# AnthonyDickson/HIVE

Hardware: AMD Instinct MI355X
Metric: frames/sec (depth+TSDF integrate) @640x480, 512^3 vol (higher is better)
Workload: dtype bf16; 1 GPU; synthetic 640x480x150 RGB (seeded room trajectory), host-resident uint8 frames uploaded in the timed region, DPT-Hybrid depth (seeded random weights: depth 1-7 m, bf16, hip engine) + 512x512x512 TSDF integrate, 107 frames/step; frames_total=4066, volume=512x512x512, tsdf_overlap=True, scaling_mode=weak

## Files before the change

hive_amd/csrc/conv.hip:

```cpp
#include "hive_internal.hpp"
#include "mfma_pipe.hpp"

#include <algorithm>

#ifndef HIVE_CONV_AHEAD_GN2
#define HIVE_CONV_AHEAD_GN2 4
#endif
#ifndef HIVE_CONV_ABLATE
#define HIVE_CONV_ABLATE 0
#endif
#ifndef HIVE_CONV_AHEAD
#define HIVE_CONV_AHEAD 4
#endif

using hive_mfma::f32x4;
using hive_mfma::vec;

namespace {

template <typename T>
struct ConvParams {
    const T *x;
    const T *w;
    const T *bias;
    const T *res1;
    const T *res2;
    T *out;
    T *out_relu;
    const T *zeros;
    int H, W, Cin, Cout, relu;
    int Ho, Wo;
    int S, taps;
    int stride, pad_t, pad_l;
    int M;
    float *gn_partial;
    int stats_only;
    const float *gn_stats;
    const T *gn_gamma, *gn_beta;
    int gn_G, gn_cpg;
    int split_k;
    hive_mfma::f32x4 *sk_ws;
    unsigned *sk_count;
};

__device__ __forceinline__ float gn_affine_exact(float x, float rstd, float gamma, float beta, float mean) {
#pragma clang fp contract(off)
    const float a = rstd * gamma;
    const float b = beta - mean * a;
    return x * a + b;
}

template <typename T, int MT, int GN, int NRES = 1>
__device__ __forceinline__ void conv_epilogue(const ConvParams<T> &p, f32x4 (&acc)[4][MT], int m_base, int n_base, unsigned char *stage, int lane,
                                              int boundary) {
    asm volatile("" : "+v"(lane));
    const int n = n_base + (lane & 7) * 8;
    float b[8] = {0.f, 0.f, 0.f, 0.f, 0.f, 0.f, 0.f, 0.f};
    if (p.bias) {
        const vec<T, 8> bv = *reinterpret_cast<const vec<T, 8> *>(p.bias + n);
#pragma unroll
        for (int j = 0; j < 8; ++j) b[j] = (float)bv[j];
    }
    float ggam[8], gbet[8], gmean[2] = {0.f, 0.f}, grstd[2] = {0.f, 0.f};
    if (GN == 2) {
        const vec<T, 8> gv = *reinterpret_cast<const vec<T, 8> *>(p.gn_gamma + n), bv = *reinterpret_cast<const vec<T, 8> *>(p.gn_beta + n);
#pragma unroll
        for (int j = 0; j < 8; ++j) ggam[j] = (float)gv[j], gbet[j] = (float)bv[j];
        const int hw = p.Ho * p.Wo, img0 = boundary / hw - 1, n_img = p.M / hw, g = n / p.gn_cpg;
        const float *st = p.gn_stats + ((size_t)img0 * p.gn_G + g) * 2;
        gmean[0] = st[0], grstd[0] = st[1];
        if (img0 + 1 < n_img) gmean[1] = st[2 * p.gn_G], grstd[1] = st[2 * p.gn_G + 1];
    }
    constexpr int AHEAD = GN == 2 ? HIVE_CONV_AHEAD_GN2 : (NRES == 2 ? HIVE_CONV_AHEAD / 2 : HIVE_CONV_AHEAD);
    vec<T, 8> rs1[AHEAD + 1][2], rs2[NRES == 2 ? AHEAD + 1 : 1][2];
    const int row_in_frag = lane >> 3;
    auto pre = [&](int mt, int j) {
        const int m = min(m_base + mt * 16 + 8 * j + row_in_frag, p.M - 1);
        const size_t off = (size_t)m * p.Cout + n;
        if (GN != 1 && p.res1) rs1[mt % (AHEAD + 1)][j] = *reinterpret_cast<const vec<T, 8> *>(p.res1 + off);
        if (GN == 0 && NRES == 2) rs2[mt % (AHEAD + 1)][j] = *reinterpret_cast<const vec<T, 8> *>(p.res2 + off);
    };
    hive_mfma::staged_rows<MT, AHEAD>(stage, acc, lane, pre, [&](int r, int, const f32x4 &lo, const f32x4 &hi, int mt, int jrow) {
        const int m = m_base + r;
        if (m >= p.M) return;
        const size_t o_off = (size_t)m * p.Cout + n;
        float o[8];
#pragma unroll
        for (int j = 0; j < 4; ++j) o[j] = lo[j] + b[j], o[4 + j] = hi[j] + b[4 + j];
        if (GN == 0 && p.res1) {
            const vec<T, 8> rs = rs1[mt % (AHEAD + 1)][jrow];
#pragma unroll
            for (int j = 0; j < 8; ++j) o[j] += (float)rs[j];
        }
        if (GN == 0 && NRES == 2) {
            const vec<T, 8> rs = rs2[mt % (AHEAD + 1)][jrow];
#pragma unroll
            for (int j = 0; j < 8; ++j) o[j] += (float)rs[j];
        }
        if (GN == 0 && p.relu) {
#pragma unroll
            for (int j = 0; j < 8; ++j) o[j] = fmaxf(o[j], 0.0f);
        }
        vec<T, 8> ov;
#pragma unroll
        for (int j = 0; j < 8; ++j) ov[j] = (T)o[j];
        if (GN == 2) {
            const bool second = m >= boundary;
            const float mean = second ? gmean[1] : gmean[0], rstd = second ? grstd[1] : grstd[0];
#pragma unroll
            for (int j = 0; j < 8; ++j) o[j] = gn_affine_exact((float)ov[j], rstd, ggam[j], gbet[j], mean);
            if (p.res1) {
                const vec<T, 8> rs = rs1[mt % (AHEAD + 1)][jrow];
#pragma unroll
                for (int j = 0; j < 8; ++j) o[j] = (float)(T)o[j] + (float)rs[j];
            }
            if (p.relu) {
#pragma unroll
                for (int j = 0; j < 8; ++j) o[j] = fmaxf(o[j], 0.0f);
            }
#pragma unroll
            for (int j = 0; j < 8; ++j) ov[j] = (T)o[j];
            *reinterpret_cast<vec<T, 8> *>(p.out + o_off) = ov;
            return;
        }
        if (GN != 1 || !p.stats_only) *reinterpret_cast<vec<T, 8> *>(p.out + o_off) = ov;
        if (GN == 0 && p.out_relu) {
#pragma unroll
            for (int j = 0; j < 8; ++j) ov[j] = (T)fmaxf(o[j], 0.0f);
            *reinterpret_cast<vec<T, 8> *>(p.out_relu + o_off) = ov;
        }
    });
}

__device__ __forceinline__ float dot2acc(vec<__bf16, 2> a, vec<__bf16, 2> b, float c) { return __builtin_amdgcn_fdot2_f32_bf16(a, b, c, false); }
__device__ __forceinline__ float dot2acc(vec<_Float16, 2> a, vec<_Float16, 2> b, float c) { return __builtin_amdgcn_fdot2(a, b, c, false); }
__device__ __forceinline__ float dpp_row_total(float v) {
#define HIVE_ROR_ADD(ctrl) v += __builtin_bit_cast(float, __builtin_amdgcn_update_dpp(0, __builtin_bit_cast(int, v), ctrl, 0xf, 0xf, false))
    HIVE_ROR_ADD(0x128);
    HIVE_ROR_ADD(0x124);
    HIVE_ROR_ADD(0x122);
    HIVE_ROR_ADD(0x121);
#undef HIVE_ROR_ADD
    return v;
}
template <typename T, int MT>
__device__ __forceinline__ void gn_sums_from_acc(const ConvParams<T> &p, const f32x4 (&acc)[4][MT], int m_base, int n_base, int lane, int boundary,
                                                 float *wsum) {
    asm volatile("" : "+v"(lane));
    const int fr = lane & 15, fq = lane >> 4;
    const int m_end = m_base + MT * 16;
    const bool one_image = m_end <= p.M && (m_end <= boundary || m_base >= boundary);
    const bool second = m_base >= boundary;
    vec<T, 2> ones;
    ones[0] = ones[1] = (T)1.0f;
#pragma unroll
    for (int nt = 0; nt < 4; ++nt) {
        f32x4 bias = f32x4{0.f, 0.f, 0.f, 0.f};
        if (p.bias) {
            const vec<T, 4> bv = *reinterpret_cast<const vec<T, 4> *>(p.bias + n_base + nt * 16 + fq * 4);
#pragma unroll
            for (int e = 0; e < 4; ++e) bias[e] = (float)bv[e];
        }
        f32x4 sv[2], qv[2];
        sv[0] = sv[1] = qv[0] = qv[1] = f32x4{0.f, 0.f, 0.f, 0.f};
        if (one_image) {
            f32x4 ts = f32x4{0.f, 0.f, 0.f, 0.f}, tq = ts;
#pragma unroll
            for (int mt = 0; mt < MT; mt += 2) {
                const f32x4 a0 = acc[nt][mt] + bias, a1 = acc[nt][mt + 1] + bias;
#pragma unroll
                for (int e = 0; e < 4; ++e) {
                    vec<T, 2> y;
                    y[0] = (T)a0[e], y[1] = (T)a1[e];
                    ts[e] = dot2acc(y, ones, ts[e]);
                    tq[e] = dot2acc(y, y, tq[e]);
                }
            }
            const f32x4 zero4 = f32x4{0.f, 0.f, 0.f, 0.f};
            sv[0] = second ? zero4 : ts;
            sv[1] = second ? ts : zero4;
            qv[0] = second ? zero4 : tq;
            qv[1] = second ? tq : zero4;
        } else {
#pragma unroll
            for (int mt = 0; mt < MT; mt += 2) {
                const int m0 = m_base + mt * 16 + fr, m1 = m0 + 16;
                const bool v0 = m0 < p.M, v1 = m1 < p.M, s0 = m0 >= boundary, s1 = m1 >= boundary;
                const f32x4 a0 = acc[nt][mt] + bias, a1 = acc[nt][mt + 1] + bias;
#pragma unroll
                for (int e = 0; e < 4; ++e) {
                    vec<T, 2> y, z;
                    y[0] = (T)(v0 && !s0 ? a0[e] : 0.f), y[1] = (T)(v1 && !s1 ? a1[e] : 0.f);
                    z[0] = (T)(v0 && s0 ? a0[e] : 0.f), z[1] = (T)(v1 && s1 ? a1[e] : 0.f);
                    sv[0][e] = dot2acc(y, ones, sv[0][e]);
                    qv[0][e] = dot2acc(y, y, qv[0][e]);
                    sv[1][e] = dot2acc(z, ones, sv[1][e]);
                    qv[1][e] = dot2acc(z, z, qv[1][e]);
                }
            }
        }
#pragma unroll
        for (int h = 0; h < 2; ++h) {
            f32x4 st = f32x4{0.f, 0.f, 0.f, 0.f}, qt = f32x4{0.f, 0.f, 0.f, 0.f};
            if (h == 0 || m_end > boundary) {
#pragma unroll
                for (int e = 0; e < 4; ++e) {
                    st[e] = dpp_row_total(sv[h][e]);
                    qt[e] = dpp_row_total(qv[h][e]);
                }
            }
            if (fr == 0) {
                *reinterpret_cast<f32x4 *>(wsum + (h * 2 + 0) * 64 + nt * 16 + fq * 4) = st;
                *reinterpret_cast<f32x4 *>(wsum + (h * 2 + 1) * 64 + nt * 16 + fq * 4) = qt;
            }
        }
    }
}

constexpr int BK = 64;


template <typename T, int TM, int TN, int GN>
__global__ __launch_bounds__(512, 1) void conv_kernel(ConvParams<T> p) {
    extern __shared__ __attribute__((aligned(16))) unsigned char lds[];
    constexpr int A_GROUPS = TM / 8, A_PW = A_GROUPS / 8;
    constexpr int W_GROUPS = TN / 8, GROUPS = A_GROUPS + W_GROUPS, PER_WAVE = GROUPS / 8;
    constexpr int STAGE_BYTES = GROUPS * 1024;
    constexpr int WN = TN / 64, WM = 8 / WN, RW = TM / WM, MT = RW / 16;
    const int tid = threadIdx.x;
    int lane = tid & 63;
    const int wave = __builtin_amdgcn_readfirstlane(tid >> 6);
    const int wr = wave / WN, wc = wave % WN;
    const int tiles_n = p.Cout / TN, n_tiles = ((p.M + TM - 1) / TM) * tiles_n;
    const int xcd = blockIdx.x & 7, per_xcd = gridDim.x >> 3, tq = n_tiles >> 3, tr = n_tiles & 7;
    const int run0 = xcd < tr ? xcd * (tq + 1) : tr * (tq + 1) + (xcd - tr) * tq, run_n = tq + (xcd < tr ? 1 : 0);
    int tl = blockIdx.x >> 3;
    if (tl >= run_n) return;
    const int K = p.taps * p.Cin, CPT = p.Cin / BK;

    struct Tile {
        int m0, n0;
        int py[A_PW], px[A_PW];
        const T *pbase[A_PW];
    };
    int a_chunk[A_PW];
    auto lane_constants = [&]() {
#pragma unroll
        for (int j = 0; j < A_PW; ++j) {
            const int row = (wave + 8 * j) * 8 + (lane >> 3);
            a_chunk[j] = ((lane & 7) ^ ((row >> 1) & 7)) * 8;
        }
    };
    lane_constants();
    auto setup = [&](int t, Tile &tile) {
        tile.m0 = (t / tiles_n) * TM;
        tile.n0 = (t % tiles_n) * TN;
#pragma unroll
        for (int j = 0; j < A_PW; ++j) {
            const int row = (wave + 8 * j) * 8 + (lane >> 3);
            const int m = min(tile.m0 + row, p.M - 1);
            const int img = m / (p.Ho * p.Wo), rem = m - img * (p.Ho * p.Wo);
            const int oy = rem / p.Wo, ox = rem - oy * p.Wo;
            tile.py[j] = oy * p.stride - p.pad_t;
            tile.px[j] = ox * p.stride - p.pad_l;
            tile.pbase[j] = p.x + (((long long)img * p.H + tile.py[j]) * p.W + tile.px[j]) * p.Cin + a_chunk[j];
        }
    };

    auto issue_piece = [&](const Tile &tile, int stage, int tap, int cc, int j) {
        unsigned char *st = lds + stage * STAGE_BYTES;
        if (HIVE_CONV_ABLATE & 4) return;
        if (j < A_PW) {
            const int dy = tap / p.S, dx = tap - dy * p.S;
            const long long shift = ((long long)dy * p.W + dx) * p.Cin + cc * BK;
            const bool inside = (unsigned)(tile.py[j] + dy) < (unsigned)p.H && (unsigned)(tile.px[j] + dx) < (unsigned)p.W;
            const T *g = inside ? tile.pbase[j] + shift : p.zeros + a_chunk[j];
            __builtin_amdgcn_global_load_lds((const void *)g, (__attribute__((address_space(3))) void *)(st + (wave + 8 * j) * 1024), 16, 0, 0);
        } else {
            const int grp = wave + 8 * (j - A_PW);
            const int row = grp * 8 + (lane >> 3);
            const int chunk = (lane & 7) ^ ((row >> 1) & 7);
            const T *g = p.w + (size_t)(tile.n0 + row) * K + tap * p.Cin + cc * BK + chunk * 8;
            __builtin_amdgcn_global_load_lds((const void *)g, (__attribute__((address_space(3))) void *)(st + (A_GROUPS + grp) * 1024), 16, 0, 0);
        }
    };

    const int KT = p.taps * CPT, last_tap = p.taps - 1;
    Tile tile;
    setup(run0 + tl, tile);
#pragma unroll
    for (int j = 0; j < PER_WAVE; ++j) issue_piece(tile, 0, 0, 0, j);
    int buf = 0;
    for (;;) {
        asm volatile("" : "+v"(lane));
        lane_constants();
        const int fr = lane & 15, fq = lane >> 4;
        const bool has_next = tl + per_xcd < run_n;
        const int em0 = tile.m0, en0 = tile.n0;
        f32x4 acc[4][MT];
#pragma unroll
        for (int i = 0; i < 4; ++i)
#pragma unroll
            for (int j = 0; j < MT; ++j) acc[i][j] = f32x4{0.f, 0.f, 0.f, 0.f};
        int nx_tap = 1, nx_cc = 0;
        if (nx_tap == p.taps) nx_tap = 0, nx_cc = 1;
        for (int kt = 0; kt < KT; ++kt) {
            asm volatile("s_waitcnt vmcnt(0)" ::: "memory");
            __builtin_amdgcn_s_barrier();
            int is_tap = nx_tap, is_cc = nx_cc;
            if (kt + 1 == KT) {
                if (has_next) {
                    setup(run0 + tl + per_xcd, tile);
                    is_tap = 0, is_cc = 0;
                } else {
                    is_tap = last_tap, is_cc = CPT - 1;
                }
            }
            if (++nx_tap == p.taps) nx_tap = 0, ++nx_cc;
            const unsigned char *a_t = lds + buf * STAGE_BYTES, *w_t = a_t + A_GROUPS * 1024;
            if (HIVE_CONV_ABLATE & 2) {
                for (int j = 0; j < PER_WAVE; ++j) issue_piece(tile, buf ^ 1, is_tap, is_cc, j);
            } else {
                hive_mfma::kstep64<T, MT, false>(a_t, w_t, wr * RW, wc * 64, fr, fq, acc, PER_WAVE, [&](int j) { issue_piece(tile, buf ^ 1, is_tap, is_cc, j); });
            }
            buf ^= 1;
        }
        unsigned char *stage = lds + 2 * STAGE_BYTES + wave * 4096;
        const int hw = p.Ho * p.Wo, boundary = (em0 / hw + 1) * hw;
        if (!(HIVE_CONV_ABLATE & 1) && !(GN == 1 && p.stats_only)) {
            if (GN == 0 && p.res2)
                conv_epilogue<T, MT, GN, 2>(p, acc, em0 + wr * RW, en0 + wc * 64, stage, lane, boundary);
            else
                conv_epilogue<T, MT, GN, 1>(p, acc, em0 + wr * RW, en0 + wc * 64, stage, lane, boundary);
        }
        if (GN == 1 && !(HIVE_CONV_ABLATE & 8)) {
            __builtin_amdgcn_wave_barrier();
            gn_sums_from_acc<T, MT>(p, acc, em0 + wr * RW, en0 + wc * 64, lane, boundary, reinterpret_cast<float *>(stage));
            __syncthreads();
            const int tile_m = em0 / TM;
            for (int t = tid; t < 4 * TN; t += 512) {
                const int hq = t / TN, ch = t - hq * TN, cw = ch >> 6, c = ch & 63;
                float a = 0.f;
#pragma unroll
                for (int w = 0; w < WM; ++w) a += reinterpret_cast<const float *>(lds + 2 * STAGE_BYTES + (w * WN + cw) * 4096)[hq * 64 + c];
                p.gn_partial[((size_t)tile_m * 4 + hq) * p.Cout + en0 + ch] = a;
            }
        }
        if (!has_next) break;
        tl += per_xcd;
    }
    asm volatile("s_waitcnt vmcnt(0)" ::: "memory");
}

template <typename T, int TN, int GN, int NST>
__global__ __launch_bounds__(512, 1) void conv_deep_kernel(ConvParams<T> p) {
    extern __shared__ __attribute__((aligned(16))) unsigned char lds[];
    constexpr int TM = 128, AHEAD = NST - 1;
    constexpr int A_GROUPS = TM / 8, A_PW = A_GROUPS / 8;
    constexpr int W_GROUPS = TN / 8, GROUPS = A_GROUPS + W_GROUPS, PER_WAVE = GROUPS / 8;
    constexpr int STAGE_BYTES = GROUPS * 1024;
    constexpr int WN = TN / 64, WM = 8 / WN, RW = TM / WM, MT = RW / 16;
    static_assert(AHEAD * PER_WAVE < 64, "vmcnt is a 6-bit counter");
    const int tid = threadIdx.x;
    int lane = tid & 63;
    const int wave = __builtin_amdgcn_readfirstlane(tid >> 6);
    const int wr = wave / WN, wc = wave % WN;
    const int S = p.split_k, KT = p.taps * (p.Cin / BK);
    const int tiles_n = p.Cout / TN, n_items = ((p.M + TM - 1) / TM) * tiles_n * S;
    const int xcd = blockIdx.x & 7, per_xcd = gridDim.x >> 3, tq = n_items >> 3, tr = n_items & 7;
    const int run0 = xcd < tr ? xcd * (tq + 1) : tr * (tq + 1) + (xcd - tr) * tq, run_n = tq + (xcd < tr ? 1 : 0);
    int tl = blockIdx.x >> 3;
    if (tl >= run_n) return;

    struct Tile {
        int m0, n0, kt, k1, tl;
        int py[A_PW], px[A_PW];
        const T *pbase[A_PW];
    };
    int a_chunk[A_PW];
    auto lane_constants = [&]() {
#pragma unroll
        for (int j = 0; j < A_PW; ++j) {
            const int row = (wave + 8 * j) * 8 + (lane >> 3);
            a_chunk[j] = ((lane & 7) ^ ((row >> 1) & 7)) * 8;
        }
    };
    lane_constants();
    auto coords = [&](int item, int &m0, int &n0, int &k0, int &k1) {
        const int t = item / S, s = item - t * S;
        m0 = (t / tiles_n) * TM;
        n0 = (t % tiles_n) * TN;
        k0 = s * KT / S;
        k1 = (s + 1) * KT / S;
    };
    auto setup = [&](Tile &tile) {
        coords(run0 + tile.tl, tile.m0, tile.n0, tile.kt, tile.k1);
#pragma unroll
        for (int j = 0; j < A_PW; ++j) {
            const int row = (wave + 8 * j) * 8 + (lane >> 3);
            const int m = min(tile.m0 + row, p.M - 1);
            const int img = m / (p.Ho * p.Wo), rem = m - img * (p.Ho * p.Wo);
            const int oy = rem / p.Wo, ox = rem - oy * p.Wo;
            tile.py[j] = oy * p.stride - p.pad_t;
            tile.px[j] = ox * p.stride - p.pad_l;
            tile.pbase[j] = p.x + (((long long)img * p.H + tile.py[j]) * p.W + tile.px[j]) * p.Cin + a_chunk[j];
        }
    };
    auto issue_piece = [&](const Tile &tile, int stage, int j) {
        unsigned char *st = lds + stage * STAGE_BYTES;
        const int cc = tile.kt / p.taps, tap = tile.kt - cc * p.taps;
        if (j < A_PW) {
            const int dy = tap / p.S, dx = tap - dy * p.S;
            const long long shift = ((long long)dy * p.W + dx) * p.Cin + cc * BK;
            const bool inside = (unsigned)(tile.py[j] + dy) < (unsigned)p.H && (unsigned)(tile.px[j] + dx) < (unsigned)p.W;
            const T *g = inside ? tile.pbase[j] + shift : p.zeros + a_chunk[j];
            hive_mfma::lds_dma16_untracked((const void *)g, __builtin_amdgcn_readfirstlane(hive_mfma::lds_address(st + (wave + 8 * j) * 1024)));
        } else {
            const int grp = wave + 8 * (j - A_PW);
            const int row = grp * 8 + (lane >> 3);
            const int chunk = (lane & 7) ^ ((row >> 1) & 7);
            const T *g = p.w + (size_t)(tile.n0 + row) * (p.taps * p.Cin) + tap * p.Cin + cc * BK + chunk * 8;
            hive_mfma::lds_dma16_untracked((const void *)g, __builtin_amdgcn_readfirstlane(hive_mfma::lds_address(st + (A_GROUPS + grp) * 1024)));
        }
    };
    auto advance = [&](Tile &tile) {
        if (tile.kt + 1 < tile.k1) {
            ++tile.kt;
        } else if (tile.tl + per_xcd < run_n) {
            tile.tl += per_xcd;
            setup(tile);
        }
    };
    Tile is;
    is.tl = tl;
    setup(is);
#pragma unroll
    for (int a = 0; a < AHEAD; ++a) {
#pragma unroll
        for (int j = 0; j < PER_WAVE; ++j) issue_piece(is, a, j);
        advance(is);
    }
    int buf = 0;
    for (;;) {
        asm volatile("" : "+v"(lane));
        lane_constants();
        const int fr = lane & 15, fq = lane >> 4;
        const bool has_next = tl + per_xcd < run_n;
        int em0, en0, k0, k1;
        coords(run0 + tl, em0, en0, k0, k1);
        f32x4 acc[4][MT];
#pragma unroll
        for (int i = 0; i < 4; ++i)
#pragma unroll
            for (int j = 0; j < MT; ++j) acc[i][j] = f32x4{0.f, 0.f, 0.f, 0.f};
        for (int kt = k0; kt < k1; ++kt) {
            asm volatile("s_waitcnt vmcnt(%0)" ::"n"((AHEAD - 1) * PER_WAVE) : "memory");
            __builtin_amdgcn_s_barrier();
            const int ib = buf + AHEAD >= NST ? buf + AHEAD - NST : buf + AHEAD;
            const unsigned char *a_t = lds + buf * STAGE_BYTES, *w_t = a_t + A_GROUPS * 1024;
            hive_mfma::kstep64<T, MT, false>(a_t, w_t, wr * RW, wc * 64, fr, fq, acc, PER_WAVE, [&](int j) { issue_piece(is, ib, j); });
            advance(is);
            buf = buf + 1 == NST ? 0 : buf + 1;
        }
        unsigned char *epi = lds + NST * STAGE_BYTES;
        bool store = true;
        if (S > 1) store = hive_mfma::splitk_combine<512>(S, p.sk_ws, p.sk_count, run0 + tl, acc, tid, reinterpret_cast<int *>(epi));
        if (store) {
            unsigned char *stage = epi + wave * 4096;
            const int hw = p.Ho * p.Wo, boundary = (em0 / hw + 1) * hw;
            if (!(GN == 1 && p.stats_only)) {
                if (GN == 0 && p.res2)
                    conv_epilogue<T, MT, GN, 2>(p, acc, em0 + wr * RW, en0 + wc * 64, stage, lane, boundary);
                else
                    conv_epilogue<T, MT, GN, 1>(p, acc, em0 + wr * RW, en0 + wc * 64, stage, lane, boundary);
            }
            if (GN == 1) {
                __builtin_amdgcn_wave_barrier();
                gn_sums_from_acc<T, MT>(p, acc, em0 + wr * RW, en0 + wc * 64, lane, boundary, reinterpret_cast<float *>(stage));
                __syncthreads();
                const int tile_m = em0 / TM;
                for (int t = tid; t < 4 * TN; t += 512) {
                    const int hq = t / TN, ch = t - hq * TN, cw = ch >> 6, c = ch & 63;
                    float a = 0.f;
#pragma unroll
                    for (int w = 0; w < WM; ++w) a += reinterpret_cast<const float *>(epi + (w * WN + cw) * 4096)[hq * 64 + c];
                    p.gn_partial[((size_t)tile_m * 4 + hq) * p.Cout + en0 + ch] = a;
                }
            }
        }
        if (!has_next) break;
        __builtin_amdgcn_s_waitcnt(0x0F70);
        __syncthreads();
        tl += per_xcd;
    }
    asm volatile("s_waitcnt vmcnt(0)" ::: "memory");
}

constexpr int conv_lds(int tm, int tn, int nst = 2) { return nst * (tm / 8 + tn / 8) * 1024 + hive_mfma::STAGED_ROWS_LDS; }

constexpr int CONV_DEEP_NST = 4;

template <typename T>
int ensure_conv_attrs(hive_ctx *ctx) {
    static bool set[64] = {};
    if (ctx->device < 64 && set[ctx->device]) return HIVE_OK;
#define HIVE_CONV_ATTR(TM_, TN_, GN_) \
    HIVE_CHECK_HIP(ctx, hipFuncSetAttribute((const void *)conv_kernel<T, TM_, TN_, GN_>, hipFuncAttributeMaxDynamicSharedMemorySize, conv_lds(TM_, TN_)))
    HIVE_CONV_ATTR(256, 256, 0);
    HIVE_CONV_ATTR(256, 256, 1);
    HIVE_CONV_ATTR(256, 128, 0);
    HIVE_CONV_ATTR(256, 128, 1);
    HIVE_CONV_ATTR(256, 64, 0);
    HIVE_CONV_ATTR(256, 64, 1);
    HIVE_CONV_ATTR(128, 256, 0);
    HIVE_CONV_ATTR(128, 256, 1);
    HIVE_CONV_ATTR(128, 128, 0);
    HIVE_CONV_ATTR(128, 128, 1);
    HIVE_CONV_ATTR(256, 256, 2);
    HIVE_CONV_ATTR(128, 256, 2);
#undef HIVE_CONV_ATTR
    HIVE_CHECK_HIP(ctx, hipFuncSetAttribute((const void *)conv_deep_kernel<T, 128, 0, CONV_DEEP_NST>, hipFuncAttributeMaxDynamicSharedMemorySize, conv_lds(128, 128, CONV_DEEP_NST)));
    HIVE_CHECK_HIP(ctx, hipFuncSetAttribute((const void *)conv_deep_kernel<T, 128, 1, CONV_DEEP_NST>, hipFuncAttributeMaxDynamicSharedMemorySize, conv_lds(128, 128, CONV_DEEP_NST)));
    if (ctx->device < 64) set[ctx->device] = true;
    return HIVE_OK;
}

struct GnMode {
    int stats_only = 0;
    const float *gn_stats = nullptr;
    const void *gn_gamma = nullptr, *gn_beta = nullptr;
    int gn_G = 0, gn_cpg = 0;
};

template <typename T>
int launch_conv_t(hive_ctx *ctx, const char *what, const void *d_x, int N, int H, int W, int C_in, int C_out, int R, int stride, int pad_t,
                  int pad_l, int Ho, int Wo, const void *d_w, const void *d_bias, int relu, const void *d_residual, const void *d_residual2,
                  void *d_out, void *d_out_relu, void *d_gn_partial, long long gn_partial_floats, int *gn_tile_rows, const GnMode *gn_mode) {
    HIVE_REQUIRE(ctx, d_x && d_w && d_out, "%s: NULL argument", what);
    if (gn_tile_rows) *gn_tile_rows = 0;
    HIVE_REQUIRE(ctx, N > 0 && H > 0 && W > 0 && Ho > 0 && Wo > 0 && (long long)N * H * W < (1ll << 31) && (long long)N * Ho * Wo < (1ll << 31),
                 "%s: bad sizes %d x %d x %d -> %d x %d", what, N, H, W, Ho, Wo);
    HIVE_REQUIRE(ctx, (R == 1 || R == 3) && (stride == 1 || stride == 2) && pad_t >= 0 && pad_t < R && pad_l >= 0 && pad_l < R,
                 "%s: kernel %d, stride %d, padding (%d, %d)", what, R, stride, pad_t, pad_l);
    HIVE_REQUIRE(ctx, (long long)(Ho - 1) * stride - pad_t < H && (long long)(Wo - 1) * stride - pad_l < W, "%s: output %d x %d reaches outside the %d x %d input", what, Ho,
                 Wo, H, W);
    HIVE_REQUIRE(ctx, C_in > 0 && C_in % 64 == 0 && C_out > 0 && C_out % 64 == 0, "%s: need C_in %% 64 == 0 and C_out %% 64 == 0, got %d -> %d", what, C_in, C_out);
    HIVE_REQUIRE(ctx, (R == 1 && stride == 1) || (d_out != d_x && d_out_relu != d_x), "%s: the output must not alias the input", what);
    ConvParams<T> p{};
    p.x = (const T *)d_x;
    p.w = (const T *)d_w;
    p.bias = (const T *)d_bias;
    p.res1 = (const T *)d_residual;
    p.res2 = (const T *)d_residual2;
    p.out = (T *)d_out;
    p.out_relu = (T *)d_out_relu;
    p.zeros = (const T *)ctx->d_zeros;
    p.H = H;
    p.W = W;
    p.Cin = C_in;
    p.Cout = C_out;
    p.relu = relu;
    p.Ho = Ho;
    p.Wo = Wo;
    p.S = R;
    p.taps = R * R;
    p.stride = stride;
    p.pad_t = pad_t;
    p.pad_l = pad_l;
    p.M = N * Ho * Wo;
    int rc = ensure_conv_attrs<T>(ctx);
    if (rc) return rc;
    const int tn = C_out % 256 == 0 ? 256 : (C_out % 128 == 0 ? 128 : 64);
    int tm = 256;
    if (tn >= 128) {
        const long long per = C_out / tn, t256 = (long long)((p.M + 255) / 256) * per, t128 = (long long)((p.M + 127) / 128) * per;
        const long long r256 = (t256 + ctx->num_cus - 1) / ctx->num_cus, r128 = (t128 + ctx->num_cus - 1) / ctx->num_cus;
        if (t256 < ctx->num_cus || r128 * 128 * 100 < r256 * 256 * 85) tm = 128;
    }
    if (gn_mode) {
        p.stats_only = gn_mode->stats_only;
        p.gn_stats = gn_mode->gn_stats;
        p.gn_gamma = (const T *)gn_mode->gn_gamma;
        p.gn_beta = (const T *)gn_mode->gn_beta;
        p.gn_G = gn_mode->gn_G;
        p.gn_cpg = gn_mode->gn_cpg;
    }
    if (d_gn_partial && gn_tile_rows && (long long)Ho * Wo >= tm && !relu && !d_residual && !d_residual2 && !d_out_relu) {
        HIVE_REQUIRE(ctx, (long long)((p.M + tm - 1) / tm) * 4 * C_out <= gn_partial_floats, "%s: gn_partial holds %lld floats, %lld needed", what,
                     gn_partial_floats, (long long)((p.M + tm - 1) / tm) * 4 * C_out);
        p.gn_partial = (float *)d_gn_partial;
        *gn_tile_rows = tm;
    }
    {
        const long long tiles128 = (long long)((p.M + 127) / 128) * (C_out / 128);
        const char *deep_env = getenv("HIVE_CONV_DEEP");
        const bool allowed = !(deep_env && deep_env[0] == '0');
        if (allowed && !p.gn_stats && C_out % 128 == 0 && tiles128 <= ctx->num_cus && tiles128 <= HIVE_SPLITK_TILES) {
            const int KT = p.taps * (C_in / BK);
            const char *sk_env = getenv("HIVE_SPLITK");
            p.split_k = sk_env ? std::max(1, std::min(atoi(sk_env), KT)) : hive_mfma::splitk_ways(tiles128, KT, ctx->num_cus);
            p.split_k = (int)std::max<long long>(1, std::min<long long>(p.split_k, ctx->num_cus / tiles128));
            if (ctx->deterministic) p.split_k = 1;
            ++ctx->n_deep_ring_launches;
            if (p.split_k > 1) {
                ++ctx->n_splitk_launches;
                void *ws = nullptr;
                rc = hive_splitk_workspace(ctx, (size_t)tiles128 * p.split_k * 128 * 128 * sizeof(float), &ws, &p.sk_count);
                if (rc) return rc;
                p.sk_ws = reinterpret_cast<hive_mfma::f32x4 *>(ws);
            }
            const bool stats = d_gn_partial && gn_tile_rows && (long long)Ho * Wo >= 128 && !relu && !d_residual && !d_residual2 && !d_out_relu;
            if (stats) {
                HIVE_REQUIRE(ctx, (long long)((p.M + 127) / 128) * 4 * C_out <= gn_partial_floats, "%s: gn_partial holds %lld floats, %lld needed", what,
                             gn_partial_floats, (long long)((p.M + 127) / 128) * 4 * C_out);
                p.gn_partial = (float *)d_gn_partial;
                *gn_tile_rows = 128;
            }
            const long long items = tiles128 * p.split_k;
            const dim3 dgrid((unsigned)std::min<long long>((items + 7) / 8 * 8, (long long)ctx->num_cus / 8 * 8));
            if (stats)
                hipLaunchKernelGGL((conv_deep_kernel<T, 128, 1, CONV_DEEP_NST>), dgrid, dim3(512), (size_t)conv_lds(128, 128, CONV_DEEP_NST), ctx->stream, p);
            else
                hipLaunchKernelGGL((conv_deep_kernel<T, 128, 0, CONV_DEEP_NST>), dgrid, dim3(512), (size_t)conv_lds(128, 128, CONV_DEEP_NST), ctx->stream, p);
            HIVE_CHECK_HIP(ctx, hipGetLastError());
            return HIVE_OK;
        }
    }
    const long long tiles = (long long)((p.M + tm - 1) / tm) * (C_out / tn);
    const dim3 grid((unsigned)std::min<long long>((tiles + 7) / 8 * 8, (long long)ctx->num_cus / 8 * 8));
    const size_t lds = (size_t)conv_lds(tm, tn);
#define HIVE_CONV_LAUNCH(TM_, TN_)                                                                                   \
    do {                                                                                                             \
        if (p.gn_partial)                                                                                            \
            hipLaunchKernelGGL((conv_kernel<T, TM_, TN_, 1>), grid, dim3(512), lds, ctx->stream, p);                    \
        else                                                                                                         \
            hipLaunchKernelGGL((conv_kernel<T, TM_, TN_, 0>), grid, dim3(512), lds, ctx->stream, p);                    \
    } while (0)
    if (p.gn_stats) {
        if (tm == 256)
            hipLaunchKernelGGL((conv_kernel<T, 256, 256, 2>), grid, dim3(512), lds, ctx->stream, p);
        else
            hipLaunchKernelGGL((conv_kernel<T, 128, 256, 2>), grid, dim3(512), lds, ctx->stream, p);
    } else if (tm == 256 && tn == 256)
        HIVE_CONV_LAUNCH(256, 256);
    else if (tm == 256 && tn == 128)
        HIVE_CONV_LAUNCH(256, 128);
    else if (tm == 256)
        HIVE_CONV_LAUNCH(256, 64);
    else if (tn == 256)
        HIVE_CONV_LAUNCH(128, 256);
    else
        HIVE_CONV_LAUNCH(128, 128);
#undef HIVE_CONV_LAUNCH
    HIVE_CHECK_HIP(ctx, hipGetLastError());
    return HIVE_OK;
}

int launch_conv(hive_ctx *ctx, const char *what, const void *d_x, int dtype, int N, int H, int W, int C_in, int C_out, int R, int stride, int pad_t,
                int pad_l, int Ho, int Wo, const void *d_w, const void *d_bias, int relu, const void *d_residual, const void *d_residual2,
                void *d_out, void *d_out_relu, void *d_gn_partial = nullptr, long long gn_partial_floats = 0, int *gn_tile_rows = nullptr,
                const GnMode *gn_mode = nullptr) {
    if (dtype == HIVE_BF16)
        return launch_conv_t<__bf16>(ctx, what, d_x, N, H, W, C_in, C_out, R, stride, pad_t, pad_l, Ho, Wo, d_w, d_bias, relu, d_residual, d_residual2, d_out, d_out_relu,
                                     d_gn_partial, gn_partial_floats, gn_tile_rows, gn_mode);
    if (dtype == HIVE_F16)
        return launch_conv_t<_Float16>(ctx, what, d_x, N, H, W, C_in, C_out, R, stride, pad_t, pad_l, Ho, Wo, d_w, d_bias, relu, d_residual, d_residual2, d_out,
                                       d_out_relu, d_gn_partial, gn_partial_floats, gn_tile_rows, gn_mode);
    if (gn_tile_rows) *gn_tile_rows = 0;
    return hive_fail(ctx, HIVE_ERR_INVALID, "%s: dtype must be HIVE_F16 or HIVE_BF16", what);
}

}

extern "C" int hive_nhwc_conv3x3(hive_ctx *ctx, const void *d_x, int dtype, int N, int H, int W, int C_in, int C_out, const void *d_w,
                                 const void *d_bias, int relu, const void *d_residual, const void *d_residual2, void *d_out,
                                 void *d_out_relu) {
    HIVE_ENTER(ctx);
    if (!ctx) return hive_fail(nullptr, HIVE_ERR_INVALID, "ctx is NULL");
    HIVE_REQUIRE(ctx, C_out % 128 == 0, "nhwc_conv3x3: need C_out %% 128 == 0, got %d", C_out);
    HIVE_REQUIRE(ctx, d_out != d_x && d_out_relu != d_x, "nhwc_conv3x3: the output must not alias the input (3 x 3 halo)");
    return launch_conv(ctx, "nhwc_conv3x3", d_x, dtype, N, H, W, C_in, C_out, 3, 1, 1, 1, H, W, d_w, d_bias, relu, d_residual, d_residual2, d_out, d_out_relu);
}

extern "C" int64_t hive_nhwc_conv_gn_partial_floats(int64_t n_px, int C_out) { return (n_px / 128 + 1) * 4 * (int64_t)C_out; }

extern "C" int hive_nhwc_conv_gn(hive_ctx *ctx, const void *d_x, int dtype, int N, int H, int W, int C_in, int C_out, int kernel, int stride, int pad_top,
                                 int pad_left, int H_out, int W_out, const void *d_w, const void *d_bias, int relu, const void *d_residual,
                                 const void *d_residual2, void *d_out, void *d_out_relu, void *d_gn_partial, int64_t gn_partial_floats, int *gn_tile_rows) {
    HIVE_ENTER(ctx);
    if (!ctx) return hive_fail(nullptr, HIVE_ERR_INVALID, "ctx is NULL");
    HIVE_REQUIRE(ctx, d_gn_partial && gn_tile_rows, "nhwc_conv_gn: NULL argument");
    return launch_conv(ctx, "nhwc_conv_gn", d_x, dtype, N, H, W, C_in, C_out, kernel, stride, pad_top, pad_left, H_out, W_out, d_w, d_bias, relu, d_residual,
                       d_residual2, d_out, d_out_relu, d_gn_partial, gn_partial_floats, gn_tile_rows);
}

extern "C" int hive_nhwc_conv_gn_apply(hive_ctx *ctx, const void *d_x, int dtype, int N, int H, int W, int C_in, int C_out, int kernel, int stride,
                                       int pad_top, int pad_left, int H_out, int W_out, const void *d_w, int G, const void *d_gamma, const void *d_beta,
                                       float eps, const void *d_residual, int relu, void *d_out, void *d_scratch, int64_t scratch_floats, int *fused) {
    HIVE_ENTER(ctx);
    if (!ctx) return hive_fail(nullptr, HIVE_ERR_INVALID, "ctx is NULL");
    HIVE_REQUIRE(ctx, d_gamma && d_beta && d_scratch && fused, "nhwc_conv_gn_apply: NULL argument");
    *fused = 0;
    const long long hw = (long long)H_out * W_out;
    if (G <= 0 || C_out % 256 != 0 || C_out % G != 0 || (C_out / G) % 8 != 0 || hw < 256) return HIVE_OK;
    const int64_t partial_floats = hive_nhwc_conv_gn_partial_floats((int64_t)N * hw, C_out);
    HIVE_REQUIRE(ctx, scratch_floats >= partial_floats + 2ll * N * G, "nhwc_conv_gn_apply: scratch holds %lld floats, %lld needed", (long long)scratch_floats,
                 (long long)(partial_floats + 2ll * N * G));
    float *partial = (float *)d_scratch, *stats = partial + partial_floats;
    GnMode mode;
    mode.stats_only = 1;
    int tile_rows = 0;
    int rc = launch_conv(ctx, "nhwc_conv_gn_apply", d_x, dtype, N, H, W, C_in, C_out, kernel, stride, pad_top, pad_left, H_out, W_out, d_w, nullptr, 0, nullptr,
                         nullptr, d_out, nullptr, partial, partial_floats, &tile_rows, &mode);
    if (rc) return rc;
    HIVE_REQUIRE(ctx, tile_rows > 0, "nhwc_conv_gn_apply: no statistics from a %lld-pixel map", hw);
    rc = hive_gn_finalize_tiles(ctx, partial, N, (int)hw, C_out, G, tile_rows, eps, stats);
    if (rc) return rc;
    mode.stats_only = 0;
    mode.gn_stats = stats;
    mode.gn_gamma = d_gamma;
    mode.gn_beta = d_beta;
    mode.gn_G = G;
    mode.gn_cpg = C_out / G;
    rc = launch_conv(ctx, "nhwc_conv_gn_apply", d_x, dtype, N, H, W, C_in, C_out, kernel, stride, pad_top, pad_left, H_out, W_out, d_w, nullptr, relu, d_residual,
                     nullptr, d_out, nullptr, nullptr, 0, nullptr, &mode);
    if (rc) return rc;
    *fused = 1;
    return HIVE_OK;
}

extern "C" int hive_nhwc_conv_gn_apply_gram(hive_ctx *ctx, const void *d_x, int dtype, int N, int H, int W, int C_in, int C_out, int stride, int H_out, int W_out,
                                            const void *d_w, const float *d_tables, int G, const void *d_gamma, const void *d_beta, float eps, const void *d_residual,
                                            int relu, void *d_out, void *d_scratch, int64_t scratch_floats, int *fused) {
    HIVE_ENTER(ctx);
    if (!ctx) return hive_fail(nullptr, HIVE_ERR_INVALID, "ctx is NULL");
    HIVE_REQUIRE(ctx, d_gamma && d_beta && d_scratch && d_tables && fused, "nhwc_conv_gn_apply_gram: NULL argument");
    *fused = 0;
    const long long hw = (long long)H_out * W_out;
    if (G < 4 || 256 % G != 0 || G > 64 || C_out % 256 != 0 || C_out % G != 0 || (C_out / G) % 8 != 0 || hw < 256 || !(C_in == 64 || C_in == 128 || C_in == 256)) return HIVE_OK;
    HIVE_REQUIRE(ctx, scratch_floats >= 2ll * N * G, "nhwc_conv_gn_apply_gram: scratch holds %lld floats, %lld needed", (long long)scratch_floats, 2ll * N * G);
    HIVE_REQUIRE(ctx, (long long)(H_out - 1) * stride < H && (long long)(W_out - 1) * stride < W, "nhwc_conv_gn_apply_gram: output %d x %d reaches outside the %d x %d input", H_out,
                 W_out, H, W);
    float *stats = (float *)d_scratch;
    int rc = hive_gram_gn_stats(ctx, d_x, dtype, N, H, W, C_in, C_out, stride, H_out, W_out, G, d_tables, eps, stats, nullptr, nullptr);
    if (rc) return rc;
    GnMode mode;
    mode.gn_stats = stats;
    mode.gn_gamma = d_gamma;
    mode.gn_beta = d_beta;
    mode.gn_G = G;
    mode.gn_cpg = C_out / G;
    rc = launch_conv(ctx, "nhwc_conv_gn_apply_gram", d_x, dtype, N, H, W, C_in, C_out, 1, stride, 0, 0, H_out, W_out, d_w, nullptr, relu, d_residual, nullptr, d_out, nullptr,
                     nullptr, 0, nullptr, &mode);
    if (rc) return rc;
    *fused = 1;
    return HIVE_OK;
}

extern "C" int hive_nhwc_conv(hive_ctx *ctx, const void *d_x, int dtype, int N, int H, int W, int C_in, int C_out, int kernel, int stride, int pad_top,
                              int pad_left, int H_out, int W_out, const void *d_w, const void *d_bias, int relu, const void *d_residual,
                              const void *d_residual2, void *d_out, void *d_out_relu) {
    HIVE_ENTER(ctx);
    if (!ctx) return hive_fail(nullptr, HIVE_ERR_INVALID, "ctx is NULL");
    return launch_conv(ctx, "nhwc_conv", d_x, dtype, N, H, W, C_in, C_out, kernel, stride, pad_top, pad_left, H_out, W_out, d_w, d_bias, relu, d_residual,
                       d_residual2, d_out, d_out_relu);
}
```

hive_amd/csrc/dpt_net.hip:

```cpp
#include "hive_internal.hpp"

#include <algorithm>
#include <map>
#include <string>
#include <vector>

typedef unsigned short half_t;

namespace {

template <typename T>
__global__ __launch_bounds__(256) void assemble_tokens_kernel(const T *__restrict__ patch, const T *__restrict__ cls, const T *__restrict__ pos,
                                                              T *__restrict__ tokens, int B, int n_patch, int D) {
    const int dv = D / 8;
    const long long total = (long long)B * (n_patch + 1) * dv;
    for (long long i = (long long)blockIdx.x * 256 + threadIdx.x; i < total; i += (long long)gridDim.x * 256) {
        const int c = (int)(i % dv) * 8;
        const long long row = i / dv;
        const int t = (int)(row % (n_patch + 1)), b = (int)(row / (n_patch + 1));
        const T *src = t == 0 ? cls + c : patch + ((size_t)b * n_patch + (t - 1)) * D + c;
        const uint4 ra = *reinterpret_cast<const uint4 *>(src), rp = *reinterpret_cast<const uint4 *>(pos + (size_t)t * D + c);
        const T *a = reinterpret_cast<const T *>(&ra), *p = reinterpret_cast<const T *>(&rp);
        T o[8];
#pragma unroll
        for (int j = 0; j < 8; ++j) o[j] = (T)((float)a[j] + (float)p[j]);
        *reinterpret_cast<uint4 *>(tokens + (size_t)row * D + c) = *reinterpret_cast<const uint4 *>(o);
    }
}

__global__ __launch_bounds__(256) void readout_concat_kernel(const half_t *__restrict__ tokens, half_t *__restrict__ out, int B, int n_patch, int D) {
    const int dv = D / 8;
    const long long total = (long long)B * n_patch * 2 * dv;
    for (long long i = (long long)blockIdx.x * 256 + threadIdx.x; i < total; i += (long long)gridDim.x * 256) {
        const int c = (int)(i % (2 * dv));
        const long long row = i / (2 * dv);
        const int b = (int)(row / n_patch), t = (int)(row % n_patch);
        const half_t *src = c < dv ? tokens + ((size_t)b * (n_patch + 1) + 1 + t) * D + c * 8 : tokens + (size_t)b * (n_patch + 1) * D + (c - dv) * 8;
        *reinterpret_cast<uint4 *>(out + (size_t)row * 2 * D + c * 8) = *reinterpret_cast<const uint4 *>(src);
    }
}

void launch_assemble_tokens(hive_ctx *ctx, int dtype, int blocks, const void *patch, const void *cls, const void *pos, void *tokens, int B, int n_patch, int D) {
    if (dtype == HIVE_BF16)
        hipLaunchKernelGGL(assemble_tokens_kernel<__bf16>, dim3(blocks), dim3(256), 0, ctx->stream, (const __bf16 *)patch, (const __bf16 *)cls, (const __bf16 *)pos,
                           (__bf16 *)tokens, B, n_patch, D);
    else
        hipLaunchKernelGGL(assemble_tokens_kernel<_Float16>, dim3(blocks), dim3(256), 0, ctx->stream, (const _Float16 *)patch, (const _Float16 *)cls,
                           (const _Float16 *)pos, (_Float16 *)tokens, B, n_patch, D);
}

}

struct hive_dpt {
    hive_ctx *ctx = nullptr;
    hive_dpt_config cfg{};
    std::map<std::string, const void *> w;
    hive_vit *vit = nullptr;
    std::map<std::string, float *> gram_tables;
    void *arena = nullptr;
    size_t arena_bytes = 0, arena_used = 0;

    const void *get(const std::string &name) const {
        auto it = w.find(name);
        return it == w.end() ? nullptr : it->second;
    }
    struct Block {
        size_t off, bytes;
    };
    std::vector<Block> free_blocks;
    std::map<const void *, Block> live;
    char *base() const { return arena ? (char *)arena : (char *)(uintptr_t)4096; }
    void reset_arena() {
        free_blocks.clear();
        live.clear();
        arena_used = 0;
    }
    half_t *alloc(size_t elems) {
        const size_t bytes = (elems * sizeof(half_t) + 255) & ~(size_t)255;
        size_t off = arena_used;
        bool found = false;
        for (size_t i = 0; i < free_blocks.size(); ++i)
            if (free_blocks[i].bytes >= bytes) {
                off = free_blocks[i].off;
                if (free_blocks[i].bytes == bytes)
                    free_blocks.erase(free_blocks.begin() + i);
                else
                    free_blocks[i] = Block{off + bytes, free_blocks[i].bytes - bytes};
                found = true;
                break;
            }
        if (!found) {
            if (!free_blocks.empty() && free_blocks.back().off + free_blocks.back().bytes == arena_used) {
                off = free_blocks.back().off;
                free_blocks.pop_back();
            }
            arena_used = off + bytes;
        }
        half_t *p = (half_t *)(base() + off);
        live[p] = Block{off, bytes};
        return p;
    }
    void release(const void *p) {
        if (!p) return;
        auto it = live.find(p);
        if (it == live.end()) return;
        Block b = it->second;
        live.erase(it);
        size_t i = 0;
        while (i < free_blocks.size() && free_blocks[i].off < b.off) ++i;
        free_blocks.insert(free_blocks.begin() + i, b);
        if (i + 1 < free_blocks.size() && free_blocks[i].off + free_blocks[i].bytes == free_blocks[i + 1].off) {
            free_blocks[i].bytes += free_blocks[i + 1].bytes;
            free_blocks.erase(free_blocks.begin() + i + 1);
        }
        if (i > 0 && free_blocks[i - 1].off + free_blocks[i - 1].bytes == free_blocks[i].off) {
            free_blocks[i - 1].bytes += free_blocks[i].bytes;
            free_blocks.erase(free_blocks.begin() + i);
        }
    }
};

namespace {

struct Map {
    half_t *p;
    int H, W, C;
    float *gn = nullptr;
    int gn_tm = 0;
};

#define DPT_TRY(expr)              \
    do {                           \
        int _rc = (expr);          \
        if (_rc) return _rc;       \
    } while (0)

int run_forward(hive_dpt *d, bool dry, const uint8_t *d_rgb, int B, int FH, int FW, int H, int W, const void *d_pos, float *d_depth, float max_depth,
                uint16_t *d_mm, float *d_m) {
    hive_ctx *ctx = d->ctx;
    const bool resized = FH != H || FW != W;
    auto preprocess = [&](half_t *xin) -> int {
        if (resized) return hive_dpt_resize_preprocess(ctx, d_rgb, B, FH, FW, H, W, 0.5f, 0.5f, d->cfg.dtype, xin);
        return hive_dpt_preprocess(ctx, d_rgb, (int64_t)B * H * W * 3, 0.5f, 0.5f, d->cfg.dtype, xin);
    };
    const int dt = d->cfg.dtype;
    const std::string bb = "pretrained.model.patch_embed.backbone.";
    auto need = [&](const std::string &n, const void **out) -> int {
        *out = d->get(n);
        if (!*out) return hive_fail(ctx, HIVE_ERR_INVALID, "hive_dpt: tensor '%s' missing from the table", n.c_str());
        return HIVE_OK;
    };
    auto same_out = [](int i, int s) { return (i + s - 1) / s; };
    auto drop = [&](Map &m) {
        d->release(m.p);
        d->release(m.gn);
        m.p = nullptr;
        m.gn = nullptr;
    };
    auto conv = [&](const Map &x, const std::string &wname, const char *bias_name, int cout, int k, int stride, bool same_pad, int relu, const half_t *res1,
                    const half_t *res2, bool want_relu_copy, Map *out, Map *out_relu, bool gn_stats = false) -> int {
        int pt, pl, oh, ow;
        if (same_pad) {
            oh = same_out(x.H, stride);
            ow = same_out(x.W, stride);
            pt = std::max((oh - 1) * stride + k - x.H, 0) / 2;
            pl = std::max((ow - 1) * stride + k - x.W, 0) / 2;
        } else {
            pt = pl = k / 2;
            oh = (x.H + 2 * pt - k) / stride + 1;
            ow = (x.W + 2 * pl - k) / stride + 1;
        }
        *out = Map{d->alloc((size_t)B * oh * ow * cout), oh, ow, cout};
        if (out_relu) *out_relu = Map{want_relu_copy ? d->alloc((size_t)B * oh * ow * cout) : nullptr, oh, ow, cout};
        const int64_t gn_floats = gn_stats ? hive_nhwc_conv_gn_partial_floats((int64_t)B * oh * ow, cout) : 0;
        if (gn_stats) out->gn = (float *)d->alloc((size_t)gn_floats * 2);
        if (dry) return HIVE_OK;
        const void *wp, *bp = nullptr;
        DPT_TRY(need(wname, &wp));
        if (bias_name) DPT_TRY(need(bias_name, &bp));
        if (gn_stats)
            return hive_nhwc_conv_gn(ctx, x.p, dt, B, x.H, x.W, x.C, cout, k, stride, pt, pl, oh, ow, wp, bp, relu, res1, res2, out->p,
                                     out_relu ? out_relu->p : nullptr, out->gn, gn_floats, &out->gn_tm);
        return hive_nhwc_conv(ctx, x.p, dt, B, x.H, x.W, x.C, cout, k, stride, pt, pl, oh, ow, wp, bp, relu, res1, res2, out->p,
                              out_relu ? out_relu->p : nullptr);
    };
    auto conv_norm = [&](const Map &x, const std::string &wname, const std::string &norm_prefix, int cout, int stride, const half_t *residual, int relu,
                         Map *out) -> int {
        const int oh = same_out(x.H, stride), ow = same_out(x.W, stride);
        const int64_t scratch_floats = hive_nhwc_conv_gn_partial_floats((int64_t)B * oh * ow, cout) + 2ll * B * 32;
        float *scratch = (float *)d->alloc((size_t)scratch_floats * 2);
        *out = Map{d->alloc((size_t)B * oh * ow * cout), oh, ow, cout};
        const bool eligible = cout % 256 == 0 && (cout / 32) % 8 == 0 && (long long)oh * ow >= 256;
        Map t{eligible ? nullptr : d->alloc((size_t)B * oh * ow * cout), oh, ow, cout};
        auto done = [&](int rc) {
            d->release(scratch);
            d->release(t.p);
            return rc;
        };
        if (dry) return done(HIVE_OK);
        const void *wp, *g, *b;
        DPT_TRY(need(wname, &wp));
        DPT_TRY(need(norm_prefix + ".weight", &g));
        DPT_TRY(need(norm_prefix + ".bias", &b));
        int fused = 0;
        const char *gram_env = getenv("HIVE_GN_GRAM");
        const long long out_elems = (long long)B * oh * ow * cout;
        const bool gram = !(gram_env && gram_env[0] == '0') && !ctx->deterministic && eligible &&
                          (((x.C == 64 || x.C == 128) && out_elems >= 150000000ll) || (x.C == 256 && stride == 2 && out_elems >= 250000000ll));
        if (gram) {
            float *&tables = d->gram_tables[wname];
            if (!tables) {
                HIVE_CHECK_HIP(ctx, hipMalloc((void **)&tables, (size_t)hive_gn_gram_table_floats(x.C, 32) * sizeof(float)));
                DPT_TRY(hive_gn_gram_prepare(ctx, wp, dt, x.C, cout, 32, tables));
            }
            DPT_TRY(hive_nhwc_conv_gn_apply_gram(ctx, x.p, dt, B, x.H, x.W, x.C, cout, stride, oh, ow, wp, tables, 32, g, b, d->cfg.gn_eps, residual, relu, out->p, scratch,
                                                 scratch_floats, &fused));
            if (fused) return done(HIVE_OK);
        }
        DPT_TRY(hive_nhwc_conv_gn_apply(ctx, x.p, dt, B, x.H, x.W, x.C, cout, 1, stride, 0, 0, oh, ow, wp, 32, g, b, d->cfg.gn_eps, residual, relu, out->p,
                                        scratch, scratch_floats, &fused));
        if (fused) return done(HIVE_OK);
        if (eligible) return hive_fail(ctx, HIVE_ERR_INVALID, "hive_dpt: conv + GroupNorm of '%s' was not fused", wname.c_str());
        DPT_TRY(hive_nhwc_conv_gn(ctx, x.p, dt, B, x.H, x.W, x.C, cout, 1, stride, 0, 0, oh, ow, wp, nullptr, 0, nullptr, nullptr, t.p, nullptr, scratch,
                                  scratch_floats, &t.gn_tm));
        return done(hive_nhwc_group_norm_stats(ctx, t.p, dt, B, oh * ow, cout, 32, g, b, d->cfg.gn_eps, residual, relu, out->p, scratch, t.gn_tm));
    };
    auto group_norm = [&](const Map &x, const std::string &prefix, const half_t *residual, int relu, Map *out) -> int {
        *out = Map{d->alloc((size_t)B * x.H * x.W * x.C), x.H, x.W, x.C};
        if (dry) return HIVE_OK;
        const void *g, *b;
        DPT_TRY(need(prefix + ".weight", &g));
        DPT_TRY(need(prefix + ".bias", &b));
        return hive_nhwc_group_norm_stats(ctx, x.p, dt, B, x.H * x.W, x.C, 32, g, b, d->cfg.gn_eps, residual, relu, out->p, x.gn, x.gn_tm);
    };

    Map layer_1, layer_2, layer_3, layer_4;
    auto hybrid_backbone = [&]() -> int {
        half_t *xin = d->alloc((size_t)B * H * W * 3);
        Map s0{d->alloc((size_t)B * same_out(H, 2) * same_out(W, 2) * 64), same_out(H, 2), same_out(W, 2), 64};
        const int64_t stem_floats = hive_nhwc_conv_gn_partial_floats((int64_t)B * s0.H * s0.W, 64);
        s0.gn = (float *)d->alloc((size_t)stem_floats * 2);
        if (!dry) {
            DPT_TRY(preprocess(xin));
            const void *sw;
            DPT_TRY(need(bb + "stem.conv.weight", &sw));
            DPT_TRY(hive_resnet_stem_conv_gn(ctx, xin, dt, B, H, W, sw, s0.p, s0.gn, stem_floats, &s0.gn_tm));
        }
        d->release(xin);
        Map feat{d->alloc((size_t)B * same_out(s0.H, 2) * same_out(s0.W, 2) * 64), same_out(s0.H, 2), same_out(s0.W, 2), 64};
        if (!dry) {
            const void *g, *b;
            DPT_TRY(need(bb + "stem.norm.weight", &g));
            DPT_TRY(need(bb + "stem.norm.bias", &b));
            DPT_TRY(hive_nhwc_group_norm_relu_maxpool(ctx, s0.p, dt, B, s0.H, s0.W, 64, 32, g, b, d->cfg.gn_eps, feat.p, s0.gn_tm ? s0.gn : nullptr, s0.gn_tm));
        }
        drop(s0);
        const int depths[3] = {3, 4, 9}, chans[3] = {256, 512, 1024};
        Map hook[2] = {Map{nullptr, 0, 0, 0}, Map{nullptr, 0, 0, 0}};
        for (int s = 0; s < 3; ++s) {
            for (int blk = 0; blk < depths[s]; ++blk) {
                const std::string pre = bb + "stages." + std::to_string(s) + ".blocks." + std::to_string(blk) + ".";
                const int cout = chans[s], mid = cout / 4, stride = (blk == 0 && s > 0) ? 2 : 1;
                Map in = feat, shortcut = feat, t, u, t2, u2;
                if (blk == 0) DPT_TRY(conv_norm(in, pre + "downsample.conv.weight", pre + "downsample.norm", cout, stride, nullptr, 0, &shortcut));
                DPT_TRY(conv(in, pre + "conv1.weight", nullptr, mid, 1, 1, true, 0, nullptr, nullptr, false, &t, nullptr, true));
                int bneck = 0;
                if (mid == 64 && stride == 1 && (long long)t.H * t.W >= 256) {
                    t2 = Map{d->alloc((size_t)B * t.H * t.W * 64), t.H, t.W, 64};
                    const int64_t floats = hive_nhwc_conv_gn_partial_floats((int64_t)B * t.H * t.W, 64);
                    t2.gn = (float *)d->alloc((size_t)floats * 2);
                    if (dry) {
                        bneck = 1;
                    } else {
                        const void *g, *b, *w2;
                        DPT_TRY(need(pre + "norm1.weight", &g));
                        DPT_TRY(need(pre + "norm1.bias", &b));
                        DPT_TRY(need(pre + "conv2.weight", &w2));
                        DPT_TRY(hive_bneck_gn_conv3x3(ctx, t.p, dt, B, t.H, t.W, 64, t.gn, t.gn_tm, g, b, d->cfg.gn_eps, w2, t2.p, t2.gn, floats, &t2.gn_tm, &bneck));
                        if (!bneck) return hive_fail(ctx, HIVE_ERR_INVALID, "hive_dpt: the 64-channel bottleneck convolution of '%s' was not fused", pre.c_str());
                    }
                    drop(t);
                }
                if (!bneck) {
                    DPT_TRY(group_norm(t, pre + "norm1", nullptr, 1, &u));
                    drop(t);
                    DPT_TRY(conv(u, pre + "conv2.weight", nullptr, mid, 3, stride, true, 0, nullptr, nullptr, false, &t2, nullptr, true));
                    drop(u);
                }
                DPT_TRY(group_norm(t2, pre + "norm2", nullptr, 1, &u2));
                drop(t2);
                DPT_TRY(conv_norm(u2, pre + "conv3.weight", pre + "norm3", cout, 1, shortcut.p, 1, &feat));
                drop(u2);
                if (blk == 0) drop(shortcut);
                if (in.p != hook[0].p && in.p != hook[1].p) drop(in);
            }
            if (s < 2) hook[s] = feat;
        }
        layer_1 = hook[0];
        layer_2 = hook[1];

        const int gh = feat.H, gw = feat.W, n_patch = gh * gw, N = n_patch + 1, D = 768;
        Map pe;
        DPT_TRY(conv(feat, "pretrained.model.patch_embed.proj.weight", "pretrained.model.patch_embed.proj.bias", D, 1, 1, false, 0, nullptr, nullptr, false, &pe,
                     nullptr));
        half_t *tokens = d->alloc((size_t)B * N * D), *tap3 = d->alloc((size_t)B * N * D), *tap4 = d->alloc((size_t)B * N * D);
        half_t *cat = d->alloc((size_t)B * n_patch * 2 * D);
        Map map3{d->alloc((size_t)B * n_patch * D), gh, gw, D}, map4{d->alloc((size_t)B * n_patch * D), gh, gw, D};
        if (!dry) {
            const void *cls;
            DPT_TRY(need("pretrained.model.cls_token", &cls));
            const int blocks = (int)std::min<long long>(((long long)B * N * D / 8 + 255) / 256, (long long)ctx->num_cus * 16);
            launch_assemble_tokens(ctx, dt, blocks, pe.p, cls, d_pos, tokens, B, n_patch, D);
            HIVE_CHECK_HIP(ctx, hipGetLastError());
            const int taps[2] = {8, 11};
            void *tap_out[2] = {tap3, tap4};
            DPT_TRY(hive_vit_forward(d->vit, tokens, B, N, taps, 2, tap_out));
            const half_t *tap[2] = {tap3, tap4};
            Map *maps[2] = {&map3, &map4};
            for (int r = 0; r < 2; ++r) {
                hipLaunchKernelGGL(readout_concat_kernel, dim3(blocks), dim3(256), 0, ctx->stream, tap[r], cat, B, n_patch, D);
                HIVE_CHECK_HIP(ctx, hipGetLastError());
                const std::string pre = std::string("pretrained.act_postprocess") + (r == 0 ? "3" : "4") + ".0.project.0.";
                const void *rw, *rb;
                DPT_TRY(need(pre + "weight", &rw));
                DPT_TRY(need(pre + "bias", &rb));
                DPT_TRY(hive_vit_linear(ctx, cat, dt, rw, (const float *)rb, nullptr, maps[r]->p, B * n_patch, D, 2 * D, 1 ));
            }
        }
        drop(feat);
        drop(pe);
        d->release(tokens);
        d->release(tap3);
        d->release(tap4);
        d->release(cat);
        Map t4;
        DPT_TRY(conv(map3, "pretrained.act_postprocess3.3.weight", "pretrained.act_postprocess3.3.bias", D, 1, 1, false, 0, nullptr, nullptr, false, &layer_3, nullptr));
        drop(map3);
        DPT_TRY(conv(map4, "pretrained.act_postprocess4.3.weight", "pretrained.act_postprocess4.3.bias", D, 1, 1, false, 0, nullptr, nullptr, false, &t4, nullptr));
        drop(map4);
        DPT_TRY(conv(t4, "pretrained.act_postprocess4.4.weight", "pretrained.act_postprocess4.4.bias", D, 3, 2, false, 0, nullptr, nullptr, false, &layer_4, nullptr));
        drop(t4);
        return HIVE_OK;
    };
    auto large_backbone = [&]() -> int {
        const int D = 1024, gh = H / 16, gw = W / 16, n_patch = gh * gw, N = n_patch + 1;
        half_t *xin = d->alloc((size_t)B * H * W * 3), *cols = d->alloc((size_t)B * n_patch * 768), *pe = d->alloc((size_t)B * n_patch * D);
        half_t *tokens = d->alloc((size_t)B * N * D), *cat = d->alloc((size_t)B * n_patch * 2 * D);
        half_t *tapb[4];
        Map maps[4];
        for (int r = 0; r < 4; ++r) {
            tapb[r] = d->alloc((size_t)B * N * D);
            maps[r] = Map{d->alloc((size_t)B * n_patch * D), gh, gw, D};
        }
        if (!dry) {
            DPT_TRY(preprocess(xin));
            DPT_TRY(hive_patch_rows(ctx, xin, dt, B, H, W, 3, 16, cols));
            const void *pw, *pb, *cls;
            DPT_TRY(need("pretrained.model.patch_embed.proj.weight", &pw));
            DPT_TRY(need("pretrained.model.patch_embed.proj.bias.f32", &pb));
            DPT_TRY(need("pretrained.model.cls_token", &cls));
            DPT_TRY(hive_vit_linear(ctx, cols, dt, pw, (const float *)pb, nullptr, pe, B * n_patch, D, 768, 0));
            const int blocks = (int)std::min<long long>(((long long)B * N * D / 8 + 255) / 256, (long long)ctx->num_cus * 16);
            launch_assemble_tokens(ctx, dt, blocks, pe, cls, d_pos, tokens, B, n_patch, D);
            HIVE_CHECK_HIP(ctx, hipGetLastError());
            const int taps[4] = {5, 11, 17, 23};
            void *tap_out[4] = {tapb[0], tapb[1], tapb[2], tapb[3]};
            DPT_TRY(hive_vit_forward(d->vit, tokens, B, N, taps, 4, tap_out));
            for (int r = 0; r < 4; ++r) {
                hipLaunchKernelGGL(readout_concat_kernel, dim3(blocks), dim3(256), 0, ctx->stream, (const half_t *)tapb[r], cat, B, n_patch, D);
                HIVE_CHECK_HIP(ctx, hipGetLastError());
                const std::string pre = "pretrained.act_postprocess" + std::to_string(r + 1) + ".0.project.0.";
                const void *rw, *rb;
                DPT_TRY(need(pre + "weight", &rw));
                DPT_TRY(need(pre + "bias", &rb));
                DPT_TRY(hive_vit_linear(ctx, cat, dt, rw, (const float *)rb, nullptr, maps[r].p, B * n_patch, D, 2 * D, 1 ));
            }
        }
        d->release(xin);
        d->release(cols);
        d->release(pe);
        d->release(tokens);
        d->release(cat);
        for (int r = 0; r < 4; ++r) d->release(tapb[r]);
        auto conv_transpose = [&](const Map &x, const std::string &prefix, int s_, Map *out) -> int {
            Map tmp{d->alloc((size_t)B * x.H * x.W * s_ * s_ * x.C), x.H, x.W, s_ * s_ * x.C};
            *out = Map{d->alloc((size_t)B * x.H * x.W * s_ * s_ * x.C), s_ * x.H, s_ * x.W, x.C};
            if (dry) {
                drop(tmp);
                return HIVE_OK;
            }
            const void *wr, *bias;
            DPT_TRY(need(prefix + ".weight.rows", &wr));
            DPT_TRY(need(prefix + ".bias", &bias));
            DPT_TRY(hive_nhwc_conv(ctx, x.p, dt, B, x.H, x.W, x.C, s_ * s_ * x.C, 1, 1, 0, 0, x.H, x.W, wr, nullptr, 0, nullptr, nullptr, tmp.p, nullptr));
            const int rc = hive_nhwc_pixel_shuffle_bias(ctx, tmp.p, bias, dt, B, x.H, x.W, x.C, s_, out->p);
            drop(tmp);
            return rc;
        };
        const std::string pp = "pretrained.act_postprocess";
        Map t;
        DPT_TRY(conv(maps[0], pp + "1.3.weight", (pp + "1.3.bias").c_str(), 256, 1, 1, false, 0, nullptr, nullptr, false, &t, nullptr));
        drop(maps[0]);
        DPT_TRY(conv_transpose(t, pp + "1.4", 4, &layer_1));
        drop(t);
        DPT_TRY(conv(maps[1], pp + "2.3.weight", (pp + "2.3.bias").c_str(), 512, 1, 1, false, 0, nullptr, nullptr, false, &t, nullptr));
        drop(maps[1]);
        DPT_TRY(conv_transpose(t, pp + "2.4", 2, &layer_2));
        drop(t);
        DPT_TRY(conv(maps[2], pp + "3.3.weight", (pp + "3.3.bias").c_str(), 1024, 1, 1, false, 0, nullptr, nullptr, false, &layer_3, nullptr));
        drop(maps[2]);
        DPT_TRY(conv(maps[3], pp + "4.3.weight", (pp + "4.3.bias").c_str(), 1024, 1, 1, false, 0, nullptr, nullptr, false, &t, nullptr));
        drop(maps[3]);
        DPT_TRY(conv(t, pp + "4.4.weight", (pp + "4.4.bias").c_str(), 1024, 3, 2, false, 0, nullptr, nullptr, false, &layer_4, nullptr));
        drop(t);
        return HIVE_OK;
    };

    DPT_TRY(d->cfg.backbone == 0 ? hybrid_backbone() : large_backbone());

    auto refinenet = [&](int n, const Map *path, const Map &lrn, const Map &lrn_relu, Map *out) -> int {
        const std::string pre = "scratch.refinenet" + std::to_string(n) + ".";
        Map o = lrn, o_relu = lrn_relu, t;
        if (path) {
            DPT_TRY(conv(lrn_relu, pre + "resConfUnit1.conv1.weight", (pre + "resConfUnit1.conv1.bias").c_str(), 256, 3, 1, false, 1, nullptr, nullptr, false, &t,
                         nullptr));
            DPT_TRY(conv(t, pre + "resConfUnit1.conv2.weight", (pre + "resConfUnit1.conv2.bias").c_str(), 256, 3, 1, false, 0, lrn.p, path->p, true, &o, &o_relu));
            drop(t);
        }
        Map u, low, t2;
        DPT_TRY(conv(o_relu, pre + "resConfUnit2.conv1.weight", (pre + "resConfUnit2.conv1.bias").c_str(), 256, 3, 1, false, 1, nullptr, nullptr, false, &t2, nullptr));
        DPT_TRY(conv(t2, pre + "resConfUnit2.conv2.weight", (pre + "resConfUnit2.conv2.bias").c_str(), 256, 3, 1, false, 0, o.p, nullptr, false, &u, nullptr));
        drop(t2);
        if (o.p != lrn.p) drop(o);
        if (o_relu.p != lrn_relu.p) drop(o_relu);
        DPT_TRY(conv(u, pre + "out_conv.weight", nullptr, 256, 1, 1, false, 0, nullptr, nullptr, false, &low, nullptr));
        drop(u);
        *out = Map{d->alloc((size_t)B * 4 * low.H * low.W * 256), 2 * low.H, 2 * low.W, 256};
        int rc = HIVE_OK;
        if (!dry) {
            const void *ob;
            DPT_TRY(need(pre + "out_conv.bias", &ob));
            rc = hive_nhwc_upsample2x(ctx, low.p, ob, dt, B, low.H, low.W, 256, out->p);
        }
        drop(low);
        return rc;
    };
    const Map *layers[4] = {&layer_1, &layer_2, &layer_3, &layer_4};
    Map path{}, prev{};
    for (int n = 4; n >= 1; --n) {
        Map lrn, lrn_relu;
        DPT_TRY(conv(*layers[n - 1], "scratch.layer" + std::to_string(n) + "_rn.weight", nullptr, 256, 3, 1, false, 0, nullptr, nullptr, true, &lrn, &lrn_relu));
        d->release(layers[n - 1]->p);
        DPT_TRY(refinenet(n, n == 4 ? nullptr : &prev, lrn, lrn_relu, &path));
        drop(lrn);
        drop(lrn_relu);
        if (n != 4) drop(prev);
        prev = path;
    }

    Map lo;
    DPT_TRY(conv(path, "scratch.output_conv.0.weight", "scratch.output_conv.0.bias", 128, 3, 1, false, 0, nullptr, nullptr, false, &lo, nullptr));
    drop(path);
    float *net_depth = resized ? (float *)d->alloc((size_t)B * H * W * 2) : nullptr;
    if (dry) return HIVE_OK;
    const void *w3;
    DPT_TRY(need("scratch.output_conv.2.weight", &w3));
    HIVE_REQUIRE(ctx, 2 * lo.H == H && 2 * lo.W == W, "hive_dpt: network size %d x %d must be a multiple of 32", H, W);
    if (!resized)
        return hive_dpt_head_fused(ctx, lo.p, nullptr, dt, B, lo.H, lo.W, 128, 32, w3, d->cfg.head_b3, d->cfg.head_w1, d->cfg.head_b1,
                                   d->cfg.non_negative, d->cfg.invert, d->cfg.scale, d->cfg.shift, d_depth, 1.0f / 1000.0f, max_depth, d_mm, d_m);
    DPT_TRY(hive_dpt_head_fused(ctx, lo.p, nullptr, dt, B, lo.H, lo.W, 128, 32, w3, d->cfg.head_b3, d->cfg.head_w1, d->cfg.head_b1, d->cfg.non_negative, d->cfg.invert,
                                d->cfg.scale, d->cfg.shift, net_depth, 1.0f / 1000.0f, max_depth, nullptr, nullptr));
    return hive_depth_resize_nearest(ctx, net_depth, B, H, W, FH, FW, 1.0f / 1000.0f, max_depth, d_depth, d_mm, d_m);
}

}

extern "C" {

int hive_dpt_create(hive_ctx *ctx, const hive_dpt_config *config, const hive_dpt_tensor *tensors, int n_tensors, hive_dpt **out) {
    HIVE_ENTER(ctx);
    if (!ctx) return hive_fail(nullptr, HIVE_ERR_INVALID, "ctx is NULL");
    HIVE_REQUIRE(ctx, config && tensors && n_tensors > 0 && out, "hive_dpt_create: NULL argument");
    HIVE_REQUIRE(ctx, config->backbone == 0 || config->backbone == 1, "hive_dpt_create: backbone %d (0 = vitb_rn50_384, 1 = vitl16_384)", config->backbone);
    HIVE_REQUIRE(ctx, config->dtype == HIVE_BF16 || config->dtype == HIVE_F16, "hive_dpt_create: dtype %d (HIVE_F16 = %d or HIVE_BF16 = %d)", config->dtype, (int)HIVE_F16,
                 (int)HIVE_BF16);
    const int vit_depth = config->backbone == 0 ? 12 : 24, vit_dim = config->backbone == 0 ? 768 : 1024, vit_heads = vit_dim / 64;
    *out = nullptr;
    hive_dpt *d = new hive_dpt();
    d->ctx = ctx;
    d->cfg = *config;
    for (int i = 0; i < n_tensors; ++i)
        if (tensors[i].name && tensors[i].data) d->w[tensors[i].name] = tensors[i].data;
    std::vector<hive_vit_block_weights> blocks(vit_depth);
    const char *fields[12] = {"norm1.weight", "norm1.bias", "attn.qkv.weight", "attn.qkv.bias", "attn.proj.weight", "attn.proj.bias",
                              "norm2.weight", "norm2.bias", "mlp.fc1.weight", "mlp.fc1.bias", "mlp.fc2.weight", "mlp.fc2.bias"};
    for (int i = 0; i < vit_depth; ++i) {
        const void **dst = reinterpret_cast<const void **>(&blocks[i]);
        for (int f = 0; f < 12; ++f) {
            const std::string name = "pretrained.model.blocks." + std::to_string(i) + "." + fields[f];
            dst[f] = d->get(name);
            if (!dst[f]) {
                int rc = hive_fail(ctx, HIVE_ERR_INVALID, "hive_dpt_create: tensor '%s' missing from the table", name.c_str());
                delete d;
                return rc;
            }
        }
    }
    int rc = hive_vit_create(ctx, config->dtype, vit_depth, vit_dim, vit_heads, 4 * vit_dim, config->ln_eps, blocks.data(), &d->vit);
    if (rc) {
        hive_dpt_destroy(d);
        return rc;
    }
    *out = d;
    return HIVE_OK;
}

int hive_dpt_forward_frames(hive_dpt *d, const uint8_t *d_rgb, int B, int frame_h, int frame_w, int net_h, int net_w, const void *d_pos_embed, float *d_depth,
                            float max_depth, uint16_t *d_out_mm, float *d_out_m) {
    HIVE_ENTER(d ? d->ctx : nullptr);
    if (!d) return hive_fail(nullptr, HIVE_ERR_INVALID, "dpt is NULL");
    hive_ctx *ctx = d->ctx;
    const int H = net_h, W = net_w;
    HIVE_REQUIRE(ctx, d_rgb && d_pos_embed && (d_depth || d_out_mm || d_out_m), "hive_dpt_forward: NULL argument");
    HIVE_REQUIRE(ctx, B > 0 && frame_h > 0 && frame_w > 0, "hive_dpt_forward: bad frame batch %d x %d x %d", B, frame_h, frame_w);
    HIVE_REQUIRE(ctx, H >= 32 && W >= 32 && H % 32 == 0 && W % 32 == 0, "hive_dpt_forward: the network's input size must be a multiple of 32 (%d x %d)", H, W);
    void *arena = d->arena;
    d->arena = nullptr;
    d->reset_arena();
    int rc = run_forward(d, true, d_rgb, B, frame_h, frame_w, H, W, d_pos_embed, d_depth, max_depth, d_out_mm, d_out_m);
    d->arena = arena;
    if (rc) return rc;
    const size_t need = d->arena_used;
    if ((rc = hive_reserve_device(ctx, &d->arena, &d->arena_bytes, need))) return rc;
    d->reset_arena();
    return run_forward(d, false, d_rgb, B, frame_h, frame_w, H, W, d_pos_embed, d_depth, max_depth, d_out_mm, d_out_m);
}

int hive_dpt_forward(hive_dpt *d, const uint8_t *d_rgb, int B, int H, int W, const void *d_pos_embed, float *d_depth, float max_depth,
                     uint16_t *d_out_mm, float *d_out_m) {
    return hive_dpt_forward_frames(d, d_rgb, B, H, W, H, W, d_pos_embed, d_depth, max_depth, d_out_mm, d_out_m);
}

int hive_dpt_weights_modified(hive_dpt *d) {
    HIVE_ENTER(d ? d->ctx : nullptr);
    if (!d) return hive_fail(nullptr, HIVE_ERR_INVALID, "dpt is NULL");
    HIVE_CHECK_HIP(d->ctx, hipStreamSynchronize(d->ctx->stream));
    for (auto &kv : d->gram_tables)
        if (kv.second) (void)hipFree(kv.second);
    d->gram_tables.clear();
    return hive_vit_weights_modified(d->vit);
}

int hive_dpt_arena_bytes(hive_dpt *d, int64_t *bytes) {
    if (!d || !bytes) return hive_fail(d ? d->ctx : nullptr, HIVE_ERR_INVALID, "hive_dpt_arena_bytes: NULL argument");
    *bytes = (int64_t)d->arena_bytes;
    return HIVE_OK;
}

int hive_dpt_destroy(hive_dpt *d) {
    if (!d) return HIVE_OK;
    {
        HIVE_ENTER(d->ctx);
        (void)hipStreamSynchronize(d->ctx->stream);
        if (d->vit) hive_vit_destroy(d->vit);
        if (d->arena) (void)hipFree(d->arena);
        for (auto &kv : d->gram_tables)
            if (kv.second) (void)hipFree(kv.second);
    }
    delete d;
    return HIVE_OK;
}

}
```

hive_amd/csrc/hive_internal.hpp:

```cpp
#pragma once
#include <hip/hip_runtime.h>

#include <cstdarg>
#include <cstdint>
#include <cstdio>
#include <cstring>
#include <string>
#include <vector>

#include "../../include/hive_mi355x.h"

#define HIVE_WAVE 64

struct hive_staging_slot {
    void *pinned = nullptr;
    size_t bytes = 0;
    hipEvent_t done = nullptr;
    bool in_flight = false;
};

struct hive_ctx {
    int device = 0;
    int num_cus = 256;
    hipStream_t stream = nullptr;
    bool owns_stream = false;
    int round_mode = HIVE_ROUND_HALF_EVEN;
    std::string last_error;

    static constexpr int kSlots = 4;
    hive_staging_slot slots[kSlots];
    int next_slot = 0;

    void *d_scratch = nullptr;
    size_t scratch_bytes = 0;
    void *d_frame = nullptr;
    size_t frame_bytes = 0;
    void *d_batch = nullptr;
    size_t batch_bytes = 0;
    void *d_in = nullptr;
    size_t in_bytes = 0;
    int tsdf_scalars = 0;
    int tsdf_multi_scalars = 0;
    unsigned *d_scalars = nullptr;
    void *h_pinned_small = nullptr;
    void *d_zeros = nullptr;
    void *d_splitk = nullptr;
    size_t splitk_bytes = 0;
    unsigned *d_splitk_count = nullptr;
    void *d_gram = nullptr;
    size_t gram_bytes = 0;

    bool deterministic = false;
    int64_t n_splitk_launches = 0, n_deep_ring_launches = 0;

    bool timing = false;
    std::vector<hipEvent_t> ev_pool;
    size_t ev_used = 0;
    hipEvent_t last_start = nullptr, last_stop = nullptr;
};

int hive_fail(hive_ctx *ctx, int code, const char *fmt, ...);

struct hive_device_guard {
    int prev = -1;
    bool switched = false;
    explicit hive_device_guard(const hive_ctx *ctx) {
        if (!ctx) return;
        if (hipGetDevice(&prev) == hipSuccess && prev != ctx->device) switched = hipSetDevice(ctx->device) == hipSuccess;
    }
    ~hive_device_guard() {
        if (switched) (void)hipSetDevice(prev);
    }
    hive_device_guard(const hive_device_guard &) = delete;
    hive_device_guard &operator=(const hive_device_guard &) = delete;
};
#define HIVE_ENTER(ctx) hive_device_guard _hive_device_guard(ctx)
void hive_set_global_error(const char *msg);

#define HIVE_CHECK_HIP(ctx, expr)                                                                        \
    do {                                                                                                 \
        hipError_t _e = (expr);                                                                          \
        if (_e != hipSuccess)                                                                            \
            return hive_fail((ctx), _e == hipErrorOutOfMemory ? HIVE_ERR_NOMEM : HIVE_ERR_DEVICE,        \
                             "%s failed: %s (%s:%d)", #expr, hipGetErrorString(_e), __FILE__, __LINE__); \
    } while (0)

#define HIVE_REQUIRE(ctx, cond, ...)                                   \
    do {                                                               \
        if (!(cond)) return hive_fail((ctx), HIVE_ERR_INVALID, __VA_ARGS__); \
    } while (0)

int hive_reserve_device(hive_ctx *ctx, void **ptr, size_t *cur, size_t bytes);
int hive_upload(hive_ctx *ctx, void *dst, const void *src, size_t bytes);
int hive_gn_finalize_tiles(hive_ctx *ctx, const float *d_partial, int N, int HW, int C, int G, int tile_rows, float eps, float *d_stats);
constexpr int HIVE_SPLITK_TILES = 4096;
int hive_splitk_workspace(hive_ctx *ctx, size_t bytes, void **ws, unsigned **count);
int hive_gram_gn_stats(hive_ctx *ctx, const void *d_x, int dtype, int N, int H, int W, int C_in, int C_out, int stride, int Ho, int Wo, int G, const float *d_tables,
                       float eps, float *d_stats, float *d_S_out, float *d_s_out);
__device__ __forceinline__ unsigned block_exclusive(unsigned c, unsigned *lds) {
    const int lane = threadIdx.x & 63, wave = threadIdx.x >> 6;
    unsigned inc = c;
    for (int off = 1; off < 64; off <<= 1) {
        const unsigned o = (unsigned)__shfl_up((int)inc, off);
        if (lane >= off) inc += o;
    }
    if (lane == 63) lds[wave] = inc;
    __syncthreads();
    unsigned before = 0;
    for (int w = 0; w < wave; ++w) before += lds[w];
    __syncthreads();
    return before + inc - c;
}
void hive_launch_scan_blocks2(hive_ctx *ctx, unsigned *a, unsigned *b, int nb, unsigned *totals, int *bbox);
struct hive_dec_job {
    const double *pos;
    const int32_t *faces;
    const unsigned *counts;
    long long vert_cap = 0, face_cap = 0;
    long long budget = 0;
    double max_error = 0.0;
    int32_t *out_faces = nullptr;
    long long out_face_cap = 0;
    int32_t *out_vertex_index = nullptr;
    unsigned *out_counts = nullptr;
};
size_t hive_decimate_scratch_bytes(long long vert_cap, long long face_cap);
int32_t *hive_decimate_vmap(void *scratch, long long vert_cap, long long face_cap);
int hive_decimate_run(hive_ctx *ctx, const hive_dec_job &job, void *scratch, int64_t stats[3]);
int hive_time_begin(hive_ctx *ctx);
int hive_time_end(hive_ctx *ctx);

struct hive_tsdf {
    hive_ctx *ctx = nullptr;
    int64_t dim[3] = {0, 0, 0};
    int64_t n = 0;
    int64_t x_off = 0;
    int64_t grid_dim0 = 0;
    double bnds[6] = {0, 0, 0, 0, 0, 0};
    float origin[3] = {0, 0, 0};
    float voxel_size = 0.f;
    float trunc = 0.f;
    float *d_tsdf = nullptr, *d_weight = nullptr, *d_color = nullptr;
    bool owns = false;
    int round_mode = HIVE_ROUND_HALF_EVEN;
    std::vector<int> last_groups;
    bool unit_weights = true;
    int64_t unit_frames = 0;
    int64_t frames_seen = 0, launches_seen = 0;
    const unsigned *last_n_items = nullptr;
    int64_t n_verts = -1, n_faces = -1;
    int64_t cap_verts = 0, cap_faces = 0;
    float *d_verts = nullptr, *d_norms = nullptr, *d_verts_vox = nullptr;
    int32_t *d_faces = nullptr;
    uint8_t *d_vcolors = nullptr;
    uint32_t *d_vbase = nullptr;
    size_t vbase_bytes = 0;
    uint32_t *d_blk = nullptr;
    size_t blk_bytes = 0;
};

void hive_tsdf_free_mesh(hive_tsdf *vol);

template <int RM>
__device__ __forceinline__ float hive_round(float x) {
    if (RM == 0) return rintf(x);
    return roundf(x);
}
```

hive_amd/csrc/vit.hip:

```cpp
#include "hive_internal.hpp"
#include "mfma_pipe.hpp"

#include <algorithm>
#include <cstdlib>
#include <cmath>

using hive_mfma::f32x4;
using hive_mfma::f32x16;
using hive_mfma::vec;

#ifndef HIVE_GEMM_AHEAD
#define HIVE_GEMM_AHEAD 3
#endif
enum { EPI_BIAS = 0, EPI_BIAS_GELU = 1, EPI_BIAS_RESIDUAL = 2, EPI_QKV = 3, EPI_QKV_ALL = 4 };

__device__ __forceinline__ int vt_slot(int tok) { return (tok & ~12) | ((tok & 4) << 1) | ((tok & 8) >> 1); }

using hive_mfma::swz;

template <typename T, int CH>
__global__ __launch_bounds__(256) void layernorm_kernel(const T *__restrict__ x, const float *__restrict__ gamma,
                                                        const float *__restrict__ beta, T *__restrict__ out, int M, float eps) {
    constexpr int D = 256 * CH;
    const int row = blockIdx.x * 4 + (threadIdx.x >> 6);
    const int lane = threadIdx.x & 63;
    if (row >= M) return;
    const T *xr = x + (size_t)row * D;
    float v[4 * CH];
    constexpr int n_chunks = CH;
    float sum = 0.f;
#pragma unroll
    for (int i = 0; i < n_chunks; ++i) {
        const vec<T, 4> t = *reinterpret_cast<const vec<T, 4> *>(xr + i * 256 + lane * 4);
        for (int j = 0; j < 4; ++j) {
            v[4 * i + j] = (float)t[j];
            sum += v[4 * i + j];
        }
    }
    for (int off = 32; off > 0; off >>= 1) sum += __shfl_xor(sum, off);
    const float mean = sum / (float)D;
    float var = 0.f;
#pragma unroll
    for (int i = 0; i < 4 * n_chunks; ++i) {
        const float d = v[i] - mean;
        var += d * d;
    }
    for (int off = 32; off > 0; off >>= 1) var += __shfl_xor(var, off);
    const float rstd = rsqrtf(var / (float)D + eps);
    T *orow = out + (size_t)row * D;
#pragma unroll
    for (int i = 0; i < n_chunks; ++i) {
        const int c = i * 256 + lane * 4;
        const float4 g = *reinterpret_cast<const float4 *>(gamma + c);
        const float4 b = *reinterpret_cast<const float4 *>(beta + c);
        vec<T, 4> o;
        o[0] = (T)((v[4 * i + 0] - mean) * rstd * g.x + b.x);
        o[1] = (T)((v[4 * i + 1] - mean) * rstd * g.y + b.y);
        o[2] = (T)((v[4 * i + 2] - mean) * rstd * g.z + b.z);
        o[3] = (T)((v[4 * i + 3] - mean) * rstd * g.w + b.w);
        *reinterpret_cast<vec<T, 4> *>(orow + c) = o;
    }
}

template <typename T>
struct GemmParams {
    const T *A;
    const T *W;
    const float *bias;
    const T *residual;
    T *C;
    T *vT;
    int M, N, K, ldc;
    int Np, H;
    int n_split;
    int q_cols;
    float q_scale;
    const float *ln_stats;
    const float *ln_c1;
    float *ln_partial;
    int split_k = 1;
    hive_mfma::f32x4 *sk_ws = nullptr;
    unsigned *sk_count = nullptr;
};

constexpr int BN = 128, BK = 64;

#ifndef HIVE_GEMM_ABLATE
#define HIVE_GEMM_ABLATE 0
#endif

typedef float f32x2 __attribute__((ext_vector_type(2)));

#ifndef HIVE_GELU_AS
#define HIVE_GELU_AS 0
#endif
#if HIVE_GELU_AS
__device__ __forceinline__ f32x2 gelu_exact2(f32x2 x) {
    const f32x2 ax = f32x2{fabsf(x.x), fabsf(x.y)};
    const f32x2 z = ax * 0.70710678118654752440f;
    const f32x2 d = 1.0f + 0.3275911f * z;
    const f32x2 t = f32x2{__builtin_amdgcn_rcpf(d.x), __builtin_amdgcn_rcpf(d.y)};
    const f32x2 poly = ((((1.061405429f * t - 1.453152027f) * t + 1.421413741f) * t - 0.284496736f) * t + 0.254829592f) * t;
    const f32x2 a = -z * z * 1.44269504088896340736f;
    const f32x2 e = f32x2{__builtin_amdgcn_exp2f(a.x), __builtin_amdgcn_exp2f(a.y)};
    const f32x2 erf_abs = 1.0f - poly * e;
    const f32x2 s = f32x2{copysignf(erf_abs.x, x.x), copysignf(erf_abs.y, x.y)};
    return 0.5f * x * (1.0f + s);
}
#else
__device__ __forceinline__ f32x2 gelu_exact2(f32x2 x) {
    const f32x2 ax = f32x2{fabsf(x.x), fabsf(x.y)};
    f32x2 q = 4.88117491e-04f * ax - 7.19880622e-03f;
    q = q * ax + 5.21468023e-02f;
    q = q * ax + 4.59595714e-01f;
    q = q * ax + 1.15100057e+00f;
    const f32x2 P = ax * q + 1.0f;
    const f32x2 e = f32x2{__builtin_amdgcn_exp2f(-P.x), __builtin_amdgcn_exp2f(-P.y)};
    return (x + ax) * 0.5f - ax * e;
}
#endif


template <typename T, bool UNTRACKED = false>
__device__ __forceinline__ void stage_group(const T *__restrict__ src, int ld, int row0, int row_max, int k0,
                                            unsigned char *tile, int grp, int lane) {
    const int row = grp * 8 + (lane >> 3);
    const int chunk = (lane & 7) ^ ((row >> 1) & 7);
    const int grow = min(row0 + row, row_max);
    const T *g = src + (size_t)grow * ld + k0 + chunk * 8;
    if constexpr (UNTRACKED)
        hive_mfma::lds_dma16_untracked((const void *)g, __builtin_amdgcn_readfirstlane(hive_mfma::lds_address(tile + grp * 1024)));
    else
        __builtin_amdgcn_global_load_lds((const void *)g, (__attribute__((address_space(3))) void *)(tile + grp * 1024), 16, 0, 0);
}

__device__ __forceinline__ float dpp_oct_total(float v) {
#define HIVE_DPP_ADD(ctrl) v += __builtin_bit_cast(float, __builtin_amdgcn_update_dpp(0, __builtin_bit_cast(int, v), ctrl, 0xf, 0xf, false))
    HIVE_DPP_ADD(0xB1);
    HIVE_DPP_ADD(0x4E);
    HIVE_DPP_ADD(0x141);
#undef HIVE_DPP_ADD
    return v;
}

template <typename T, int EPI, int MT>
__device__ __forceinline__ void gemm_store_rows(const GemmParams<T> &p, const f32x4 (&acc)[4][MT], int m_base, int n_base, unsigned char *stage, int lane) {
    const int n = n_base + (lane & 7) * 8, rr = lane >> 3;
    const float4 b0 = *reinterpret_cast<const float4 *>(p.bias + n), b1 = *reinterpret_cast<const float4 *>(p.bias + n + 4);
    const bool ln_in = EPI != EPI_BIAS_RESIDUAL && p.ln_stats != nullptr;
    const bool ln_out = EPI == EPI_BIAS_RESIDUAL && p.ln_partial != nullptr;
    float4 c0 = float4{0.f, 0.f, 0.f, 0.f}, c1 = c0;
    if (ln_in) {
        c0 = *reinterpret_cast<const float4 *>(p.ln_c1 + n);
        c1 = *reinterpret_cast<const float4 *>(p.ln_c1 + n + 4);
    }
    constexpr int AHEAD = HIVE_GEMM_AHEAD;
    vec<T, 8> rs[AHEAD + 1][2];
    float2 st_in[2] = {float2{0.f, 0.f}, float2{0.f, 0.f}}, st_out[2] = {float2{0.f, 0.f}, float2{0.f, 0.f}};
    const int pc = lane & 7;
    auto pair_row = [&](int q) { return m_base + (q >> 1) * 16 + 8 * (q & 1) + rr; };
    if (ln_in) {
        st_in[0] = *reinterpret_cast<const float2 *>(p.ln_stats + 2 * (size_t)min(pair_row(pc), p.M - 1));
        if (MT > 4) st_in[1] = *reinterpret_cast<const float2 *>(p.ln_stats + 2 * (size_t)min(pair_row(pc + 8), p.M - 1));
    }
    auto pre = [&](int mt, int j) {
        const int m = min(m_base + mt * 16 + 8 * j + rr, p.M - 1);
        if (EPI == EPI_BIAS_RESIDUAL) rs[mt % (AHEAD + 1)][j] = *reinterpret_cast<const vec<T, 8> *>(p.residual + (size_t)m * p.ldc + n);
    };
#define HIVE_BCAST8(v, k) __builtin_bit_cast(float, __builtin_amdgcn_ds_swizzle(__builtin_bit_cast(int, (v)), 0x18 | ((k) << 5)))
    hive_mfma::staged_rows<MT, AHEAD>(stage, acc, lane, pre, [&](int r, int, const f32x4 &lo, const f32x4 &hi, int mt, int j) {
        const int m = m_base + r;
        if (m >= p.M) return;
        float o[8];
        if (ln_in) {
            float2 st;
            {
                const int q = 2 * mt + j;
                const float2 src = st_in[q >> 3];
                switch (q & 7) {
                    case 0: st = float2{HIVE_BCAST8(src.x, 0), HIVE_BCAST8(src.y, 0)}; break;
                    case 1: st = float2{HIVE_BCAST8(src.x, 1), HIVE_BCAST8(src.y, 1)}; break;
                    case 2: st = float2{HIVE_BCAST8(src.x, 2), HIVE_BCAST8(src.y, 2)}; break;
                    case 3: st = float2{HIVE_BCAST8(src.x, 3), HIVE_BCAST8(src.y, 3)}; break;
                    case 4: st = float2{HIVE_BCAST8(src.x, 4), HIVE_BCAST8(src.y, 4)}; break;
                    case 5: st = float2{HIVE_BCAST8(src.x, 5), HIVE_BCAST8(src.y, 5)}; break;
                    case 6: st = float2{HIVE_BCAST8(src.x, 6), HIVE_BCAST8(src.y, 6)}; break;
                    default: st = float2{HIVE_BCAST8(src.x, 7), HIVE_BCAST8(src.y, 7)}; break;
                }
            }
            o[0] = st.y * (lo[0] - st.x * c0.x) + b0.x, o[1] = st.y * (lo[1] - st.x * c0.y) + b0.y;
            o[2] = st.y * (lo[2] - st.x * c0.z) + b0.z, o[3] = st.y * (lo[3] - st.x * c0.w) + b0.w;
            o[4] = st.y * (hi[0] - st.x * c1.x) + b1.x, o[5] = st.y * (hi[1] - st.x * c1.y) + b1.y;
            o[6] = st.y * (hi[2] - st.x * c1.z) + b1.z, o[7] = st.y * (hi[3] - st.x * c1.w) + b1.w;
        } else {
            o[0] = lo[0] + b0.x, o[1] = lo[1] + b0.y, o[2] = lo[2] + b0.z, o[3] = lo[3] + b0.w;
            o[4] = hi[0] + b1.x, o[5] = hi[1] + b1.y, o[6] = hi[2] + b1.z, o[7] = hi[3] + b1.w;
        }
        if (EPI == EPI_BIAS && n < p.q_cols) {
#pragma unroll
            for (int k = 0; k < 8; ++k) o[k] *= p.q_scale;
        }
        if (EPI == EPI_BIAS_GELU) {
#pragma unroll
            for (int k = 0; k < 8; k += 2) {
                const f32x2 g = gelu_exact2(f32x2{o[k], o[k + 1]});
                o[k] = g.x;
                o[k + 1] = g.y;
            }
        }
        if (EPI == EPI_BIAS_RESIDUAL) {
#pragma unroll
            for (int k = 0; k < 8; ++k) o[k] += (float)rs[mt % (AHEAD + 1)][j][k];
        }
        vec<T, 8> ov;
#pragma unroll
        for (int k = 0; k < 8; ++k) ov[k] = (T)o[k];
        if constexpr (HIVE_GEMM_ABLATE & 2)
            asm volatile("" ::"v"(ov));
        else
            *reinterpret_cast<vec<T, 8> *>(p.C + (size_t)m * p.ldc + n) = ov;
        if (ln_out) {
            float v[8], sum = 0.f;
#pragma unroll
            for (int k = 0; k < 8; ++k) {
                v[k] = (float)ov[k];
                sum += v[k];
            }
            sum = dpp_oct_total(sum);
            const float mean = sum * (1.0f / 64.0f);
            float m2 = 0.f;
#pragma unroll
            for (int k = 0; k < 8; ++k) m2 += (v[k] - mean) * (v[k] - mean);
            m2 = dpp_oct_total(m2);
            {
                const int q = 2 * mt + j;
                if (pc == (q & 7)) st_out[q >> 3] = float2{sum, m2};
            }
        }
    });
    if (ln_out) {
#pragma unroll
        for (int h = 0; h < (MT > 4 ? 2 : 1); ++h) {
            const int m = pair_row(pc + 8 * h);
            if (m < p.M) *reinterpret_cast<float2 *>(p.ln_partial + 2 * ((size_t)m * (p.N >> 6) + (n_base >> 6))) = st_out[h];
        }
    }
#undef HIVE_BCAST8
}

template <typename T, int CH>
__global__ __launch_bounds__(256) void ln_row_stats_kernel(const T *__restrict__ x, float *__restrict__ stats, int M, float eps) {
    constexpr int D = 256 * CH;
    const int row = blockIdx.x * 4 + (threadIdx.x >> 6);
    const int lane = threadIdx.x & 63;
    if (row >= M) return;
    const T *xr = x + (size_t)row * D;
    float v[4 * CH];
    float sum = 0.f;
#pragma unroll
    for (int i = 0; i < CH; ++i) {
        const vec<T, 4> t = *reinterpret_cast<const vec<T, 4> *>(xr + i * 256 + lane * 4);
        for (int j = 0; j < 4; ++j) {
            v[4 * i + j] = (float)t[j];
            sum += v[4 * i + j];
        }
    }
    for (int off = 32; off > 0; off >>= 1) sum += __shfl_xor(sum, off);
    const float mean = sum / (float)D;
    float var = 0.f;
#pragma unroll
    for (int i = 0; i < 4 * CH; ++i) {
        const float d = v[i] - mean;
        var += d * d;
    }
    for (int off = 32; off > 0; off >>= 1) var += __shfl_xor(var, off);
    if (lane == 0) *reinterpret_cast<float2 *>(stats + 2 * (size_t)row) = float2{mean, rsqrtf(var / (float)D + eps)};
}

__device__ __forceinline__ float dpp_row16_total(float v) {
#define HIVE_DPP_ADD(ctrl) v += __builtin_bit_cast(float, __builtin_amdgcn_update_dpp(0, __builtin_bit_cast(int, v), ctrl, 0xf, 0xf, false))
    HIVE_DPP_ADD(0x128);
    HIVE_DPP_ADD(0x124);
    HIVE_DPP_ADD(0x122);
    HIVE_DPP_ADD(0x121);
#undef HIVE_DPP_ADD
    return v;
}
__global__ __launch_bounds__(256) void ln_finalize_kernel(const float *__restrict__ partial, int M, int groups, float eps, float *__restrict__ stats) {
    const int row = blockIdx.x * 16 + (threadIdx.x >> 4), g = threadIdx.x & 15;
    float2 pg = float2{0.f, 0.f};
    if (row < M && g < groups) pg = reinterpret_cast<const float2 *>(partial)[(size_t)row * groups + g];
    const float mean = dpp_row16_total(pg.x) / (float)(64 * groups);
    const float d = pg.x * (1.0f / 64.0f) - mean;
    const float m2 = dpp_row16_total(g < groups ? pg.y + 64.0f * d * d : 0.f);
    if (row < M && g == 0) *reinterpret_cast<float2 *>(stats + 2 * (size_t)row) = float2{mean, rsqrtf(m2 / (float)(64 * groups) + eps)};
}

template <typename T>
__global__ __launch_bounds__(256) void ln_fold_weights_kernel(const T *__restrict__ W, const float *__restrict__ bias, const float *__restrict__ gamma,
                                                              const float *__restrict__ beta, int K, T *__restrict__ Wf, float *__restrict__ c1, float *__restrict__ c2) {
    __shared__ double red[2][256];
    const int n = blockIdx.x;
    double s1 = 0.0, s2 = 0.0;
    for (int k = threadIdx.x; k < K; k += 256) {
        const float w = (float)W[(size_t)n * K + k];
        const T wf = (T)(gamma[k] * w);
        Wf[(size_t)n * K + k] = wf;
        s1 += (double)(float)wf;
        s2 += (double)beta[k] * (double)w;
    }
    red[0][threadIdx.x] = s1;
    red[1][threadIdx.x] = s2;
    __syncthreads();
    for (int off = 128; off > 0; off >>= 1) {
        if ((int)threadIdx.x < off) {
            red[0][threadIdx.x] += red[0][threadIdx.x + off];
            red[1][threadIdx.x] += red[1][threadIdx.x + off];
        }
        __syncthreads();
    }
    if (threadIdx.x == 0) {
        c1[n] = (float)red[0][0];
        c2[n] = (float)(red[1][0] + (double)bias[n]);
    }
}

template <typename T, int EPI, int TM, int NST>
__global__ __launch_bounds__(TM * 2, 1) void gemm_kernel(GemmParams<T> p) {
    extern __shared__ __attribute__((aligned(16))) unsigned char lds[];
    constexpr int NWAVES = TM / 32;
    constexpr int A_GROUPS = TM / 8, GROUPS = A_GROUPS + 16, PER_WAVE = GROUPS / NWAVES;
    constexpr int STAGE_BYTES = GROUPS * 1024;
    constexpr bool VT = (EPI == EPI_QKV);
    constexpr bool ALL = (EPI == EPI_QKV_ALL);
    const int tid = threadIdx.x, lane = tid & 63;
    const int wave = __builtin_amdgcn_readfirstlane(tid >> 6);
    const int wr = wave >> 1, wc = wave & 1;
    const int S = p.split_k, KT = p.K / BK;
    const int tiles_n = p.N / BN, n_tiles = ((p.M + TM - 1) / TM) * tiles_n * S;
    const int xcd = blockIdx.x & 7, per_xcd = gridDim.x >> 3, tq = n_tiles >> 3, tr = n_tiles & 7;
    const int run0 = xcd < tr ? xcd * (tq + 1) : tr * (tq + 1) + (xcd - tr) * tq, run_n = tq + (xcd < tr ? 1 : 0);
    int tl = blockIdx.x >> 3;
    if (tl >= run_n) return;
    auto coords = [&](int item, int &m, int &n, int &ka, int &kb) {
        const int t = item / S, s = item - t * S;
        m = (t / tiles_n) * TM;
        n = (t % tiles_n) * BN;
        ka = s * KT / S;
        kb = (s + 1) * KT / S;
    };
    int m0, n0, k0, k1;
    coords(run0 + tl, m0, n0, k0, k1);

    auto issue_piece = [&](int tm0, int tn0, int kt, int buf, int j) {
        unsigned char *st = lds + buf * STAGE_BYTES;
        const int g = wave + j * NWAVES;
        if (g < A_GROUPS)
            stage_group<T, (NST > 2)>(p.A, p.K, tm0, p.M - 1, kt * BK, st, g, lane);
        else
            stage_group<T, (NST > 2)>(p.W, p.K, tn0, p.N - 1, kt * BK, st + A_GROUPS * 1024, g - A_GROUPS, lane);
    };
    constexpr int AHEAD = NST - 1;
    struct Cursor {
        int m0, n0, kt, k1, tl;
    } is = {m0, n0, k0, k1, tl};
    auto advance = [&](Cursor &c) {
        if (c.kt + 1 < c.k1) {
            ++c.kt;
        } else if (c.tl + per_xcd < run_n) {
            c.tl += per_xcd;
            coords(run0 + c.tl, c.m0, c.n0, c.kt, c.k1);
        }
    };
#pragma unroll
    for (int a = 0; a < AHEAD; ++a) {
#pragma unroll
        for (int j = 0; j < PER_WAVE; ++j) issue_piece(is.m0, is.n0, is.kt, a, j);
        advance(is);
    }
    const int fr = lane & 15, fq = lane >> 4;
    int buf = 0;
    for (;;) {
    const bool has_next = tl + per_xcd < run_n;
    f32x4 acc[4][4];
#pragma unroll
    for (int i = 0; i < 4; ++i)
#pragma unroll
        for (int j = 0; j < 4; ++j) acc[i][j] = f32x4{0.f, 0.f, 0.f, 0.f};
    for (int kt = k0; kt < k1; ++kt) {
        asm volatile("s_waitcnt vmcnt(%0)" ::"n"((AHEAD - 1) * PER_WAVE) : "memory");
        __builtin_amdgcn_s_barrier();
        const int ib = buf + AHEAD >= NST ? buf + AHEAD - NST : buf + AHEAD;
        const unsigned char *a_t = lds + buf * STAGE_BYTES, *w_t = a_t + A_GROUPS * 1024;
        if (ALL && n0 >= p.n_split)
            hive_mfma::kstep64<T, 4, true>(a_t, w_t, wr * 64, wc * 64, fr, fq, acc, PER_WAVE, [&](int j) { issue_piece(is.m0, is.n0, is.kt, ib, j); });
        else
            hive_mfma::kstep64<T, 4, VT>(a_t, w_t, wr * 64, wc * 64, fr, fq, acc, PER_WAVE, [&](int j) { issue_piece(is.m0, is.n0, is.kt, ib, j); });
        advance(is);
        buf = buf + 1 == NST ? 0 : buf + 1;
    }

    bool store = true;
    if (S > 1) store = hive_mfma::splitk_combine<TM * 2>(S, p.sk_ws, p.sk_count, run0 + tl, acc, tid, reinterpret_cast<int *>(lds + NST * STAGE_BYTES));
    if (store) {
    if (!VT && !(ALL && n0 >= p.n_split)) {
        if constexpr (!VT) gemm_store_rows<T, ALL ? EPI_BIAS : EPI, 4>(p, acc, m0 + wr * 64, n0 + wc * 64, lds + NST * STAGE_BYTES + wave * 4096, lane);
    } else if constexpr (VT || ALL) {
        unsigned char *ot = lds + NST * STAGE_BYTES + wave * 4096;
        const int mw = m0 + wr * 64;
        const int fqs = ((fq & 1) << 1) | (fq >> 1);
        float4 ls[4][2];
        if (p.ln_stats) {
#pragma unroll
            for (int mt = 0; mt < 4; ++mt) {
                const float *st = p.ln_stats + 2 * (size_t)min(mw + mt * 16 + fq * 4, p.M - 4);
                ls[mt][0] = *reinterpret_cast<const float4 *>(st), ls[mt][1] = *reinterpret_cast<const float4 *>(st + 4);
            }
        }
#pragma unroll
        for (int half = 0; half < 2; ++half) {
#pragma unroll
            for (int ntl = 0; ntl < 2; ++ntl) {
                const int nt = half * 2 + ntl, row = ntl * 16 + fr;
                const float b = p.bias[n0 + wc * 64 + nt * 16 + fr];
                const float c1v = p.ln_stats ? p.ln_c1[n0 + wc * 64 + nt * 16 + fr] : 0.f;
#pragma unroll
                for (int mt = 0; mt < 4; ++mt) {
                    vec<T, 4> ov;
                    if (p.ln_stats) {
                        const float4 s0 = ls[mt][0], s1 = ls[mt][1];
                        ov[0] = (T)(s0.y * (acc[mt][nt][0] - s0.x * c1v) + b);
                        ov[1] = (T)(s0.w * (acc[mt][nt][1] - s0.z * c1v) + b);
                        ov[2] = (T)(s1.y * (acc[mt][nt][2] - s1.x * c1v) + b);
                        ov[3] = (T)(s1.w * (acc[mt][nt][3] - s1.z * c1v) + b);
                    } else {
#pragma unroll
                        for (int j = 0; j < 4; ++j) ov[j] = (T)(acc[mt][nt][j] + b);
                    }
                    *reinterpret_cast<vec<T, 4> *>(ot + row * 128 + (((mt * 2 + (fqs >> 1)) ^ (row & 7)) << 4) + (fqs & 1) * 8) = ov;
                }
            }
            __builtin_amdgcn_fence(__ATOMIC_RELEASE, "wavefront");
            __builtin_amdgcn_wave_barrier();
            __builtin_amdgcn_fence(__ATOMIC_ACQUIRE, "wavefront");
            if (mw < p.M) {
                const int img = mw / p.Np, tok0 = mw - img * p.Np, head = (n0 - (ALL ? p.n_split : 0) + wc * 64) >> 6;
#pragma unroll
                for (int i = 0; i < 4; ++i) {
                    const int row = 8 * i + (lane >> 3), c = lane & 7;
                    const vec<T, 8> o8 = *reinterpret_cast<const vec<T, 8> *>(ot + row * 128 + ((c ^ (row & 7)) << 4));
                    *reinterpret_cast<vec<T, 8> *>(p.vT + (((size_t)img * p.H + head) * 64 + half * 32 + row) * p.Np + tok0 + 8 * c) = o8;
                }
            }
            __builtin_amdgcn_wave_barrier();
        }
    }
    }
    if (!has_next) break;
    if constexpr (NST > 2) __builtin_amdgcn_s_waitcnt(0x0F70);
    tl += per_xcd;
    coords(run0 + tl, m0, n0, k0, k1);
    }
    asm volatile("s_waitcnt vmcnt(0)" ::: "memory");
}

constexpr int T256 = 256, T256_STAGE = 2 * T256 / 8 * 1024;

#ifdef HIVE_GEMM_STAMPS
__device__ unsigned long long g_stamps[8 * 8192];
extern "C" int hive_debug_read_stamps(void *host, size_t bytes) {
    return hipMemcpyFromSymbol(host, HIP_SYMBOL(g_stamps), bytes, 0, hipMemcpyDeviceToHost) == hipSuccess ? 0 : 1;
}
#define HIVE_STAMP(i) do { if (tid == 0 && blockIdx.x < 8192) g_stamps[blockIdx.x * 8 + (i)] = clock64(); } while (0)
#define HIVE_STAMP_ADD(i, v) do { if (tid == 0 && blockIdx.x < 8192) g_stamps[blockIdx.x * 8 + (i)] = (v); } while (0)
#else
#define HIVE_STAMP(i) do { } while (0)
#define HIVE_STAMP_ADD(i, v) do { } while (0)
#endif

template <typename T, int EPI>
__global__ __launch_bounds__(512, 1) void gemm256_kernel(GemmParams<T> p) {
    extern __shared__ __attribute__((aligned(16))) unsigned char lds[];
    constexpr int A_GROUPS = T256 / 8, GROUPS = 2 * A_GROUPS, PER_WAVE = GROUPS / 8;
    static_assert(EPI != EPI_QKV, "the transposed v^T store stays with the 128-row kernel (N = 768)");
    const int tid = threadIdx.x, lane = tid & 63;
    const int wave = __builtin_amdgcn_readfirstlane(tid >> 6);
    const int wr = wave >> 2, wc = wave & 3;
    const int nwg = gridDim.x, xcd = blockIdx.x & 7, q = nwg >> 3, r = nwg & 7;
    const int tile = (xcd < r ? xcd * (q + 1) : r * (q + 1) + (xcd - r) * q) + (blockIdx.x >> 3);
    const int tiles_n = p.N / T256;
    const int m0 = (tile / tiles_n) * T256, n0 = (tile % tiles_n) * T256;

    unsigned piece_off[PER_WAVE];
#pragma unroll
    for (int j = 0; j < PER_WAVE; ++j) {
        const int g = wave + j * 8, row = (g & (A_GROUPS - 1)) * 8 + (lane >> 3), chunk = (lane & 7) ^ ((row >> 1) & 7);
        const int rel = j < PER_WAVE / 2 ? min(row, p.M - 1 - m0) : min(row, p.N - 1 - n0);
        piece_off[j] = (unsigned)rel * (unsigned)p.K * 2u + (unsigned)chunk * 16u;
    }
    const char *a_panel = reinterpret_cast<const char *>(p.A + (size_t)m0 * p.K), *w_panel = reinterpret_cast<const char *>(p.W + (size_t)n0 * p.K);
    auto issue_piece = [&](int kt, int stage, int j) {
        const char *g = (j < PER_WAVE / 2 ? a_panel : w_panel) + (size_t)kt * (BK * 2) + piece_off[j];
        __builtin_amdgcn_global_load_lds((const void *)g, (__attribute__((address_space(3))) void *)(lds + stage * T256_STAGE + (wave + j * 8) * 1024), 16, 0, 0);
    };

    f32x4 acc[4][8];
#pragma unroll
    for (int i = 0; i < 4; ++i)
#pragma unroll
        for (int j = 0; j < 8; ++j) acc[i][j] = f32x4{0.f, 0.f, 0.f, 0.f};

    const int KT = p.K / BK;
    HIVE_STAMP(0);
#pragma unroll
    for (int j = 0; j < PER_WAVE; ++j) issue_piece(0, 0, j);
    const int fr = lane & 15, fq = lane >> 4;
#ifdef HIVE_GEMM_STAMPS
    unsigned long long waited = 0, waited_vm = 0;
#endif
    hive_mfma::KPipe<T, 8, false> pipe;
    pipe.a_row0 = wr * 128, pipe.w_row0 = wc * 64, pipe.fr = fr, pipe.fq = fq;
    for (int kt = 0; kt < KT; ++kt) {
#ifdef HIVE_GEMM_STAMPS
        const unsigned long long w0 = clock64();
#endif
        asm volatile("s_waitcnt vmcnt(0) lgkmcnt(0)" ::: "memory");
#ifdef HIVE_GEMM_STAMPS
        const unsigned long long w1 = clock64();
#endif
        __builtin_amdgcn_s_barrier();
#ifdef HIVE_GEMM_STAMPS
        if (kt == 0) HIVE_STAMP(1); else waited += clock64() - w0, waited_vm += w1 - w0;
#endif
        const int nk = min(kt + 1, KT - 1);
        const unsigned char *a_t = lds + (kt & 1) * T256_STAGE, *w_t = a_t + A_GROUPS * 1024;
        pipe.begin(a_t, w_t);
        if (kt > 0) pipe.flush(acc);
        pipe.body(acc, PER_WAVE, [&](int j) { issue_piece(nk, (kt + 1) & 1, j); });
    }
    pipe.flush(acc);
    HIVE_STAMP(2);
    asm volatile("s_waitcnt vmcnt(0)" ::: "memory");
    HIVE_STAMP(3);
    HIVE_STAMP_ADD(6, waited);
    HIVE_STAMP_ADD(7, waited_vm);

    gemm_store_rows<T, EPI, 8>(p, acc, m0 + wr * 128, n0 + wc * 64, lds + 2 * T256_STAGE + wave * 4096, lane);
    HIVE_STAMP(4);
#ifdef HIVE_GEMM_STAMPS
    asm volatile("s_waitcnt vmcnt(0)" ::: "memory");
    HIVE_STAMP(5);
#endif
}

template <typename T, int EPI>
__global__ __launch_bounds__(512, 1) void gemm256p_kernel(GemmParams<T> p) {
    extern __shared__ __attribute__((aligned(16))) unsigned char lds[];
    constexpr int A_GROUPS = T256 / 8, GROUPS = 2 * A_GROUPS, PER_WAVE = GROUPS / 8;
    constexpr bool VT = (EPI == EPI_QKV);
    const int tid = threadIdx.x, lane = tid & 63;
    const int wave = __builtin_amdgcn_readfirstlane(tid >> 6);
    const int wr = wave >> 2, wc = wave & 3;
    const int tiles_n = p.N / T256, n_tiles = ((p.M + T256 - 1) / T256) * tiles_n;
    const int xcd = blockIdx.x & 7, per_xcd = gridDim.x >> 3, tq = n_tiles >> 3, tr = n_tiles & 7;
    const int run0 = xcd < tr ? xcd * (tq + 1) : tr * (tq + 1) + (xcd - tr) * tq, run_n = tq + (xcd < tr ? 1 : 0);
    int tl = blockIdx.x >> 3;
    if (tl >= run_n) return;
    int m0, n0;
    unsigned piece_off[PER_WAVE];
    const char *a_panel, *w_panel;
    auto setup = [&](int tile) {
        m0 = (tile / tiles_n) * T256;
        n0 = (tile % tiles_n) * T256;
#pragma unroll
        for (int j = 0; j < PER_WAVE; ++j) {
            const int g = wave + j * 8, row = (g & (A_GROUPS - 1)) * 8 + (lane >> 3), chunk = (lane & 7) ^ ((row >> 1) & 7);
            const int rel = j < PER_WAVE / 2 ? min(row, p.M - 1 - m0) : min(row, p.N - 1 - n0);
            piece_off[j] = (unsigned)rel * (unsigned)p.K * 2u + (unsigned)chunk * 16u;
        }
        a_panel = reinterpret_cast<const char *>(p.A + (size_t)m0 * p.K);
        w_panel = reinterpret_cast<const char *>(p.W + (size_t)n0 * p.K);
    };
    auto issue_piece = [&](int kt, int stage, int j) {
        const char *g = (j < PER_WAVE / 2 ? a_panel : w_panel) + (size_t)kt * (BK * 2) + piece_off[j];
        __builtin_amdgcn_global_load_lds((const void *)g, (__attribute__((address_space(3))) void *)(lds + stage * T256_STAGE + (wave + j * 8) * 1024), 16, 0, 0);
    };
    const int KT = p.K / BK;
    setup(run0 + tl);
#pragma unroll
    for (int j = 0; j < PER_WAVE; ++j) issue_piece(0, 0, j);
    hive_mfma::KPipe<T, 8, VT> pipe;
    pipe.a_row0 = wr * 128, pipe.w_row0 = wc * 64, pipe.fr = lane & 15, pipe.fq = lane >> 4;
    int buf = 0;
    for (;;) {
        const bool has_next = tl + per_xcd < run_n;
        const int em0 = m0, en0 = n0;
        f32x4 acc[VT ? 8 : 4][VT ? 4 : 8];
#pragma unroll
        for (int i = 0; i < (VT ? 8 : 4); ++i)
#pragma unroll
            for (int j = 0; j < (VT ? 4 : 8); ++j) acc[i][j] = f32x4{0.f, 0.f, 0.f, 0.f};
        for (int kt = 0; kt < KT; ++kt) {
            asm volatile("s_waitcnt vmcnt(0) lgkmcnt(0)" ::: "memory");
            __builtin_amdgcn_s_barrier();
            int nk = kt + 1;
            if (nk == KT) {
                if (has_next) {
                    setup(run0 + tl + per_xcd);
                    nk = 0;
                } else {
                    nk = KT - 1;
                }
            }
            const unsigned char *a_t = lds + buf * T256_STAGE, *w_t = a_t + A_GROUPS * 1024;
            pipe.begin(a_t, w_t);
            if (kt > 0) pipe.flush(acc);
            pipe.body(acc, PER_WAVE, [&](int j) { issue_piece(nk, buf ^ 1, j); });
            buf ^= 1;
        }
        pipe.flush(acc);
        if constexpr (HIVE_GEMM_ABLATE & 1) {
#pragma unroll
            for (int i = 0; i < (VT ? 8 : 4); ++i)
#pragma unroll
                for (int j = 0; j < (VT ? 4 : 8); ++j) asm volatile("" ::"v"(acc[i][j]));
        } else if constexpr (!VT) {
            gemm_store_rows<T, EPI, 8>(p, acc, em0 + wr * 128, en0 + wc * 64, lds + 2 * T256_STAGE + wave * 4096, lane);
        } else {
            unsigned char *ot = lds + 2 * T256_STAGE + wave * 4096;
            const int fr = lane & 15, fq = lane >> 4, fqs = ((fq & 1) << 1) | (fq >> 1);
#pragma unroll
            for (int blk = 0; blk < 2; ++blk) {
                const int mw = em0 + wr * 128 + blk * 64;
#pragma unroll
                for (int half = 0; half < 2; ++half) {
#pragma unroll
                    for (int ntl = 0; ntl < 2; ++ntl) {
                        const int nt = half * 2 + ntl, row = ntl * 16 + fr;
                        const float bv = p.bias[en0 + wc * 64 + nt * 16 + fr];
                        const float c1v = p.ln_stats ? p.ln_c1[en0 + wc * 64 + nt * 16 + fr] : 0.f;
#pragma unroll
                        for (int mtl = 0; mtl < 4; ++mtl) {
                            vec<T, 4> ov;
                            if (p.ln_stats) {
                                const float *st = p.ln_stats + 2 * (size_t)min(mw + mtl * 16 + fq * 4, p.M - 4);
                                const float4 s0 = *reinterpret_cast<const float4 *>(st), s1 = *reinterpret_cast<const float4 *>(st + 4);
                                ov[0] = (T)(s0.y * (acc[blk * 4 + mtl][nt][0] - s0.x * c1v) + bv);
                                ov[1] = (T)(s0.w * (acc[blk * 4 + mtl][nt][1] - s0.z * c1v) + bv);
                                ov[2] = (T)(s1.y * (acc[blk * 4 + mtl][nt][2] - s1.x * c1v) + bv);
                                ov[3] = (T)(s1.w * (acc[blk * 4 + mtl][nt][3] - s1.z * c1v) + bv);
                            } else
#pragma unroll
                            for (int j = 0; j < 4; ++j) ov[j] = (T)(acc[blk * 4 + mtl][nt][j] + bv);
                            *reinterpret_cast<vec<T, 4> *>(ot + row * 128 + (((mtl * 2 + (fqs >> 1)) ^ (row & 7)) << 4) + (fqs & 1) * 8) = ov;
                        }
                    }
                    __builtin_amdgcn_fence(__ATOMIC_RELEASE, "wavefront");
                    __builtin_amdgcn_wave_barrier();
                    __builtin_amdgcn_fence(__ATOMIC_ACQUIRE, "wavefront");
                    if (mw < p.M) {
                        const int img = mw / p.Np, tok0 = mw - img * p.Np, head = (en0 + wc * 64) >> 6;
#pragma unroll
                        for (int i = 0; i < 4; ++i) {
                            const int row = 8 * i + (lane >> 3), c = lane & 7;
                            const vec<T, 8> o8 = *reinterpret_cast<const vec<T, 8> *>(ot + row * 128 + ((c ^ (row & 7)) << 4));
                            *reinterpret_cast<vec<T, 8> *>(p.vT + (((size_t)img * p.H + head) * 64 + half * 32 + row) * p.Np + tok0 + 8 * c) = o8;
                        }
                    }
                    __builtin_amdgcn_wave_barrier();
                }
            }
        }
        if (!has_next) break;
        tl += per_xcd;
    }
    asm volatile("s_waitcnt vmcnt(0)" ::: "memory");
}

template <typename T>
struct AttnParams {
    const T *qk;
    const T *vT;
    T *out;
    int B, H, N, Np, D;
};

constexpr int ATT_KV = 64;
constexpr float ATT_DEFER = 8.0f;

__device__ __forceinline__ float max3_raw(float a, float b, float c) {
    float r;
    asm("v_max3_f32 %0, %1, %2, %3" : "=v"(r) : "v"(a), "v"(b), "v"(c));
    return r;
}

template <typename T, int KS>
__global__ __launch_bounds__(256 * KS) void attention_kernel(AttnParams<T> p) {
    __shared__ __attribute__((aligned(16))) unsigned char lds_all[KS * 2 * 2 * ATT_KV * 128];
    const int tid = threadIdx.x, lane = tid & 63;
    const int wave_all = __builtin_amdgcn_readfirstlane(tid >> 6);
    const int wave = wave_all & 3, kh = KS > 1 ? wave_all >> 2 : 0;
    unsigned char *lds = lds_all + kh * (2 * 2 * ATT_KV * 128);
    const int q_blocks = (p.Np + 127) / 128;
    const int qb = blockIdx.x % q_blocks;
    const int head = (blockIdx.x / q_blocks) % p.H;
    const int img = blockIdx.x / (q_blocks * p.H);
    const int lq = lane & 31, hh = lane >> 5;
    const int q_row = qb * 128 + wave * 32 + lq;
    const int q_tok = min(q_row, p.Np - 1);
    const size_t row0 = (size_t)img * p.Np;
    const int ld = 2 * p.D;

    vec<T, 8> qf[4];
    for (int ks = 0; ks < 4; ++ks)
        qf[ks] = *reinterpret_cast<const vec<T, 8> *>(p.qk + (row0 + q_tok) * ld + head * 64 + ks * 16 + hh * 8);

    const char *k_base = reinterpret_cast<const char *>(p.qk + row0 * ld + p.D + head * 64);
    const char *v_base = reinterpret_cast<const char *>(p.vT + ((size_t)img * p.H + head) * 64 * p.Np);
    unsigned k_off[2], v_off[2];
#pragma unroll
    for (int j = 0; j < 2; ++j) {
        const int row = (wave + 4 * j) * 8 + (lane >> 3), chunk = (lane & 7) ^ ((row >> 1) & 7);
        k_off[j] = (unsigned)row * (unsigned)ld * 2u + (unsigned)chunk * 16u;
        v_off[j] = (unsigned)row * (unsigned)p.Np * 2u + (unsigned)chunk * 16u;
    }
    auto issue_tile = [&](int t, int stage) {
        unsigned char *k_t = lds + stage * 2 * ATT_KV * 128 + wave * 1024, *v_t = k_t + ATT_KV * 128;
        const char *kp = k_base + (size_t)t * ((size_t)ATT_KV * ld * 2), *vp = v_base + (size_t)t * (ATT_KV * 2);
#pragma unroll
        for (int j = 0; j < 2; ++j)
            __builtin_amdgcn_global_load_lds((const void *)(kp + k_off[j]), (__attribute__((address_space(3))) void *)(k_t + j * 4096), 16, 0, 0);
#pragma unroll
        for (int j = 0; j < 2; ++j)
            __builtin_amdgcn_global_load_lds((const void *)(vp + v_off[j]), (__attribute__((address_space(3))) void *)(v_t + j * 4096), 16, 0, 0);
    };

    f32x16 oacc[2];
    for (int i = 0; i < 16; ++i) oacc[0][i] = oacc[1][i] = 0.f;
    float m_run = -INFINITY, l_run = 0.f;
    f32x16 neg_m;
    for (int i = 0; i < 16; ++i) neg_m[i] = 0.f;

    const int n_tiles = p.Np / ATT_KV;
    const int per_half = (n_tiles + KS - 1) / KS;
    const int t_begin = kh * per_half, t_end = min(n_tiles, t_begin + per_half);
    if (KS == 1 || t_begin < t_end) issue_tile(t_begin, 0);
    asm volatile("s_waitcnt vmcnt(0)" ::: "memory");
    __syncthreads();
    for (int it = 0; it < per_half; ++it) {
        const int t = t_begin + it;
        const int stage = it & 1;
        if (t + 1 < t_end) issue_tile(t + 1, stage ^ 1);
        if (KS == 1 || t < t_end) {
            const unsigned char *k_t = lds + stage * 2 * ATT_KV * 128, *v_t = k_t + ATT_KV * 128;
            const float m_used = it == 0 ? 0.f : m_run;
            f32x16 sacc[2];
#pragma unroll
            for (int ks = 0; ks < 4; ++ks)
#pragma unroll
                for (int kb = 0; kb < 2; ++kb) {
                    const vec<T, 8> kf = *reinterpret_cast<const vec<T, 8> *>(k_t + swz(kb * 32 + lq, ks * 2 + hh));
                    sacc[kb] = hive_mfma::mfma32(kf, qf[ks], ks == 0 ? neg_m : sacc[kb]);
                }
            if (t == n_tiles - 1) {
                asm volatile("; pad keys: last tile only" ::: "memory");
                const int key0 = t * ATT_KV + 4 * hh;
#pragma unroll
                for (int kb = 0; kb < 2; ++kb)
#pragma unroll
                    for (int i = 0; i < 16; ++i)
                        if (key0 + kb * 32 + (i & 3) + 8 * (i >> 2) >= p.N) sacc[kb][i] = -INFINITY;
            }
            float m_tile = max3_raw(sacc[0][0], sacc[1][0], sacc[0][1]);
            m_tile = max3_raw(m_tile, sacc[1][1], sacc[0][2]);
#pragma unroll
            for (int i = 2; i < 16; i += 2) {
                m_tile = max3_raw(m_tile, sacc[1][i], sacc[0][i + 1]);
                if (i + 2 < 16)
                    m_tile = max3_raw(m_tile, sacc[1][i + 1], sacc[0][i + 2]);
                else
                    m_tile = max3_raw(m_tile, sacc[1][i + 1], sacc[1][i + 1]);
            }
            m_tile = fmaxf(m_tile, __shfl_xor(m_tile, 32));
            if (it == 0 || __any(m_tile > ATT_DEFER)) {
                const float m_new = it == 0 ? m_tile : fmaxf(m_run, m_used + m_tile);
                const float delta = m_new - m_used;
                const float alpha = it == 0 ? 0.f : __builtin_amdgcn_exp2f(m_run - m_new);
                m_run = m_new;
                l_run *= alpha;
#pragma unroll
                for (int i = 0; i < 16; ++i) {
                    oacc[0][i] *= alpha;
                    oacc[1][i] *= alpha;
                    sacc[0][i] -= delta;
                    sacc[1][i] -= delta;
                    neg_m[i] = -m_new;
                }
            }
            vec<T, 8> pf[2][2];
            float l_tile = 0.f;
#pragma unroll
            for (int kb = 0; kb < 2; ++kb)
#pragma unroll
                for (int i = 0; i < 16; ++i) {
                    const float e = __builtin_amdgcn_exp2f(sacc[kb][i]);
                    l_tile += e;
                    pf[kb][i >> 3][i & 7] = (T)e;
                }
            l_run += l_tile;
#pragma unroll
            for (int kb = 0; kb < 2; ++kb)
#pragma unroll
                for (int s = 0; s < 2; ++s)
#pragma unroll
                    for (int db = 0; db < 2; ++db) {
                        const vec<T, 8> vf = *reinterpret_cast<const vec<T, 8> *>(v_t + swz(db * 32 + lq, 4 * kb + 2 * s + hh));
                        oacc[db] = hive_mfma::mfma32(vf, pf[kb][s], oacc[db]);
                    }
        }
        asm volatile("s_waitcnt vmcnt(0)" ::: "memory");
        __syncthreads();
    }
    float l_tot = l_run + __shfl_xor(l_run, 32);
    if constexpr (KS > 1) {
        float *xch = reinterpret_cast<float *>(lds_all + 4 * 4096) + wave * (34 * 64) + lane;
        if (kh == 1) {
#pragma unroll
            for (int i = 0; i < 16; ++i) {
                xch[i * 64] = oacc[0][i];
                xch[(16 + i) * 64] = oacc[1][i];
            }
            xch[32 * 64] = m_run;
            xch[33 * 64] = l_tot;
        }
        __syncthreads();
        if (kh == 1) return;
        const float m1 = xch[32 * 64], l1 = xch[33 * 64];
        const float m = fmaxf(m_run, m1);
        const float a0 = __builtin_amdgcn_exp2f(m_run - m), a1 = __builtin_amdgcn_exp2f(m1 - m);
        l_tot = l_tot * a0 + l1 * a1;
#pragma unroll
        for (int i = 0; i < 16; ++i) {
            oacc[0][i] = oacc[0][i] * a0 + xch[i * 64] * a1;
            oacc[1][i] = oacc[1][i] * a0 + xch[(16 + i) * 64] * a1;
        }
    }
    const float inv = 1.0f / l_tot;
    unsigned char *ot = lds_all + wave * 4096;
#pragma unroll
    for (int db = 0; db < 2; ++db)
#pragma unroll
        for (int g = 0; g < 4; ++g) {
            vec<T, 4> ov;
            for (int j = 0; j < 4; ++j) ov[j] = (T)(oacc[db][4 * g + j] * inv);
            *reinterpret_cast<vec<T, 4> *>(ot + lq * 128 + (((4 * db + g) ^ (lq & 7)) << 4) + 8 * hh) = ov;
        }
    __builtin_amdgcn_fence(__ATOMIC_RELEASE, "wavefront");
    __builtin_amdgcn_wave_barrier();
    __builtin_amdgcn_fence(__ATOMIC_ACQUIRE, "wavefront");
#pragma unroll
    for (int j = 0; j < 4; ++j) {
        const int r = 8 * j + (lane >> 3), c = lane & 7;
        const vec<T, 8> row = *reinterpret_cast<const vec<T, 8> *>(ot + r * 128 + ((c ^ (r & 7)) << 4));
        const int q = qb * 128 + wave * 32 + r;
        if (q < p.Np) *reinterpret_cast<vec<T, 8> *>(p.out + (row0 + q) * p.D + head * 64 + 8 * c) = row;
    }
}

typedef unsigned short half_bits;
__global__ __launch_bounds__(256) void pad_tokens_kernel(const half_bits *__restrict__ src, half_bits *__restrict__ dst, int B, int N, int Np,
                                                         int D, int to_padded) {
    const size_t chunks_per_row = D / 8;
    const size_t total = (size_t)B * Np * chunks_per_row;
    for (size_t i = (size_t)blockIdx.x * 256 + threadIdx.x; i < total; i += (size_t)gridDim.x * 256) {
        const size_t row = i / chunks_per_row, c = i % chunks_per_row;
        const int img = (int)(row / Np), tok = (int)(row % Np);
        if (to_padded) {
            uint4 v = make_uint4(0, 0, 0, 0);
            if (tok < N) v = *reinterpret_cast<const uint4 *>(src + ((size_t)img * N + tok) * D + c * 8);
            *reinterpret_cast<uint4 *>(dst + row * D + c * 8) = v;
        } else if (tok < N) {
            *reinterpret_cast<uint4 *>(dst + ((size_t)img * N + tok) * D + c * 8) = *reinterpret_cast<const uint4 *>(src + row * D + c * 8);
        }
    }
}

struct HeadTailParams {
    float w[64];
    float pre_bias[64];
    int pre_relu;
    float bias, scale, shift;
    int C, non_negative, invert;
    long long n_px;
    float depth_scale, max_depth;
};

template <typename T>
__global__ __launch_bounds__(256) void head_tail_kernel(const T *__restrict__ feat, HeadTailParams p, float *__restrict__ out_depth,
                                                        uint16_t *__restrict__ out_mm, float *__restrict__ out_m) {
    const long long i = (long long)blockIdx.x * 256 + threadIdx.x;
    if (i >= p.n_px) return;
    const T *f = feat + i * p.C;
    float acc = p.bias;
    for (int c = 0; c < p.C; c += 8) {
        const uint4 raw = *reinterpret_cast<const uint4 *>(f + c);
        const T *v = reinterpret_cast<const T *>(&raw);
#pragma unroll
        for (int j = 0; j < 8; ++j) {
            float x = (float)v[j] + p.pre_bias[c + j];
            if (p.pre_relu) x = fmaxf(x, 0.0f);
            acc += x * p.w[c + j];
        }
    }
    if (p.non_negative) acc = fmaxf(acc, 0.0f);
    float depth = acc;
    if (p.invert) depth = 1.0f / fmaxf(p.scale * acc + p.shift, 1e-8f);
    if (out_depth) out_depth[i] = depth;
    if (out_mm || out_m) {
        const uint16_t mm = (uint16_t)(int)fminf(fmaxf(depth * 1000.0f, 0.0f), 65535.0f);
        float m = p.depth_scale * (float)mm;
        if (m > p.max_depth) m = 0.0f;
        if (out_mm) out_mm[i] = mm;
        if (out_m) out_m[i] = m;
    }
}

struct PreprocessLut {
    float v[256];
};

template <typename T>
__global__ __launch_bounds__(256) void preprocess_kernel(const uint8_t *__restrict__ rgb, long long n, PreprocessLut lut,
                                                         T *__restrict__ out) {
    __shared__ float tab[256];
    tab[threadIdx.x] = lut.v[threadIdx.x];
    __syncthreads();
    const long long i = ((long long)blockIdx.x * 256 + threadIdx.x) * 4;
    if (i >= n) return;
    if (i + 4 <= n) {
        const uchar4 v = *reinterpret_cast<const uchar4 *>(rgb + i);
        T o[4] = {(T)tab[v.x], (T)tab[v.y], (T)tab[v.z], (T)tab[v.w]};
        *reinterpret_cast<uint2 *>(out + i) = *reinterpret_cast<const uint2 *>(o);
    } else {
        for (long long j = i; j < n; ++j) out[j] = (T)tab[rgb[j]];
    }
}

struct hive_vit {
    hive_ctx *ctx = nullptr;
    int dtype = HIVE_BF16;
    int depth = 0, dim = 0, heads = 0, mlp = 0;
    float eps = 1e-6f;
    std::vector<hive_vit_block_weights> blocks;
    void *ws = nullptr;
    size_t ws_bytes = 0;
    struct Folded {
        const void *qkv_w = nullptr, *fc1_w = nullptr;
        const float *qkv_c1 = nullptr, *qkv_c2 = nullptr, *fc1_c1 = nullptr, *fc1_c2 = nullptr;
    };
    std::vector<Folded> folded;
    void *fold_mem = nullptr;
};

template <typename T>
static int launch_layernorm(hive_ctx *ctx, const void *x, const float *g, const float *b, void *out, int M, int D, float eps) {
    const dim3 grid((M + 3) / 4), block(256);
    const T *xi = (const T *)x;
    T *xo = (T *)out;
    switch (D / 256) {
        case 1: hipLaunchKernelGGL((layernorm_kernel<T, 1>), grid, block, 0, ctx->stream, xi, g, b, xo, M, eps); break;
        case 2: hipLaunchKernelGGL((layernorm_kernel<T, 2>), grid, block, 0, ctx->stream, xi, g, b, xo, M, eps); break;
        case 3: hipLaunchKernelGGL((layernorm_kernel<T, 3>), grid, block, 0, ctx->stream, xi, g, b, xo, M, eps); break;
        case 4: hipLaunchKernelGGL((layernorm_kernel<T, 4>), grid, block, 0, ctx->stream, xi, g, b, xo, M, eps); break;
        default: return hive_fail(ctx, HIVE_ERR_INVALID, "layernorm: unsupported D %d", D);
    }
    HIVE_CHECK_HIP(ctx, hipGetLastError());
    return HIVE_OK;
}

constexpr int GEMM_TM = 128, GEMM_NST = 2, GEMM_NST_DEEP = 4;
constexpr size_t gemm_lds(int nst) { return (size_t)nst * (GEMM_TM / 8 + 16) * 1024 + (GEMM_TM / 32) * 4096; }
constexpr size_t GEMM_LDS = gemm_lds(GEMM_NST), GEMM_LDS_DEEP = gemm_lds(GEMM_NST_DEEP);
constexpr int GEMM256_LDS = 2 * T256_STAGE + hive_mfma::STAGED_ROWS_LDS;

template <typename T>
static int launch_gemm256(hive_ctx *ctx, int epi, const GemmParams<T> &p) {
    const dim3 grid((unsigned)(((p.M + T256 - 1) / T256) * (p.N / T256))), block(512);
    const size_t lds_bytes = GEMM256_LDS;
    static const char *persist = getenv("HIVE_GEMM_PERSIST");
    if (!(persist && persist[0] == '0')) {
        const dim3 pgrid((unsigned)std::min<long long>(((long long)grid.x + 7) / 8 * 8, (long long)ctx->num_cus / 8 * 8));
        switch (epi) {
            case EPI_BIAS: hipLaunchKernelGGL((gemm256p_kernel<T, EPI_BIAS>), pgrid, block, lds_bytes, ctx->stream, p); break;
            case EPI_BIAS_GELU: hipLaunchKernelGGL((gemm256p_kernel<T, EPI_BIAS_GELU>), pgrid, block, lds_bytes, ctx->stream, p); break;
            case EPI_BIAS_RESIDUAL: hipLaunchKernelGGL((gemm256p_kernel<T, EPI_BIAS_RESIDUAL>), pgrid, block, lds_bytes, ctx->stream, p); break;
            case EPI_QKV: hipLaunchKernelGGL((gemm256p_kernel<T, EPI_QKV>), pgrid, block, lds_bytes, ctx->stream, p); break;
            default: return hive_fail(ctx, HIVE_ERR_INVALID, "gemm: unknown epilogue %d", epi);
        }
        HIVE_CHECK_HIP(ctx, hipGetLastError());
        return HIVE_OK;
    }
    switch (epi) {
        case EPI_BIAS: hipLaunchKernelGGL((gemm256_kernel<T, EPI_BIAS>), grid, block, lds_bytes, ctx->stream, p); break;
        case EPI_BIAS_GELU: hipLaunchKernelGGL((gemm256_kernel<T, EPI_BIAS_GELU>), grid, block, lds_bytes, ctx->stream, p); break;
        case EPI_BIAS_RESIDUAL: hipLaunchKernelGGL((gemm256_kernel<T, EPI_BIAS_RESIDUAL>), grid, block, lds_bytes, ctx->stream, p); break;
        default: return hive_fail(ctx, HIVE_ERR_INVALID, "gemm: unknown epilogue %d", epi);
    }
    HIVE_CHECK_HIP(ctx, hipGetLastError());
    return HIVE_OK;
}

template <typename T>
static int launch_gemm(hive_ctx *ctx, int epi, const GemmParams<T> &p) {
    const char *force = getenv("HIVE_GEMM_TILE");
    const long long tiles256 = (long long)((p.M + T256 - 1) / T256) * (p.N / T256);
    const long long rounds = (tiles256 + ctx->num_cus - 1) / ctx->num_cus;
    const bool fills = tiles256 * 5 >= rounds * ctx->num_cus * 3;
    static const char *persist_env = getenv("HIVE_GEMM_PERSIST");
    const bool one_tile_kernel = persist_env && persist_env[0] == '0';
    if ((epi != EPI_QKV || !one_tile_kernel) && p.N % T256 == 0 && ((force && force[0] == '2') || (!force && fills))) return launch_gemm256<T>(ctx, epi, p);
    const long long tiles = (long long)((p.M + GEMM_TM - 1) / GEMM_TM) * (p.N / BN);
    GemmParams<T> q = p;
    const long long slots = (long long)(2 * ctx->num_cus) / 8 * 8;
    const char *sk_env = getenv("HIVE_SPLITK");
    q.split_k = sk_env ? std::max(1, std::min(atoi(sk_env), p.K / BK)) : hive_mfma::splitk_ways(tiles, p.K / BK, ctx->num_cus);
    if (tiles > HIVE_SPLITK_TILES || ctx->deterministic) q.split_k = 1;
    if (q.split_k > 1) {
        ++ctx->n_splitk_launches;
        void *ws = nullptr;
        int rc = hive_splitk_workspace(ctx, (size_t)tiles * q.split_k * GEMM_TM * BN * sizeof(float), &ws, &q.sk_count);
        if (rc) return rc;
        q.sk_ws = reinterpret_cast<hive_mfma::f32x4 *>(ws);
    }
    const long long items = tiles * q.split_k;
    const char *ring_env = getenv("HIVE_GEMM_RING");
    const bool deep = ring_env ? ring_env[0] == '4' : items <= ctx->num_cus;
    if (deep) ++ctx->n_deep_ring_launches;
    const dim3 grid((unsigned)std::min<long long>((items + 7) / 8 * 8, deep ? (long long)ctx->num_cus / 8 * 8 : slots)), block(GEMM_TM * 2);
#define HIVE_GEMM_CASE(EPI_)                                                                                                          \
    case EPI_:                                                                                                                        \
        if (deep)                                                                                                                     \
            hipLaunchKernelGGL((gemm_kernel<T, EPI_, GEMM_TM, GEMM_NST_DEEP>), grid, block, GEMM_LDS_DEEP, ctx->stream, q);            \
        else                                                                                                                          \
            hipLaunchKernelGGL((gemm_kernel<T, EPI_, GEMM_TM, GEMM_NST>), grid, block, GEMM_LDS, ctx->stream, q);                      \
        break
    switch (epi) {
        HIVE_GEMM_CASE(EPI_BIAS);
        HIVE_GEMM_CASE(EPI_BIAS_GELU);
        HIVE_GEMM_CASE(EPI_BIAS_RESIDUAL);
        HIVE_GEMM_CASE(EPI_QKV);
#undef HIVE_GEMM_CASE
        default: return hive_fail(ctx, HIVE_ERR_INVALID, "gemm: unknown epilogue %d", epi);
    }
    HIVE_CHECK_HIP(ctx, hipGetLastError());
    return HIVE_OK;
}

template <typename T>
static int ensure_gemm_attrs(hive_ctx *ctx) {
    static bool set[64] = {false};
    if (ctx->device < 64 && set[ctx->device]) return HIVE_OK;
#define HIVE_GEMM_ATTR(EPI_)                                                                                                                                  \
    HIVE_CHECK_HIP(ctx, hipFuncSetAttribute((const void *)gemm_kernel<T, EPI_, GEMM_TM, GEMM_NST>, hipFuncAttributeMaxDynamicSharedMemorySize, (int)GEMM_LDS)); \
    HIVE_CHECK_HIP(ctx, hipFuncSetAttribute((const void *)gemm_kernel<T, EPI_, GEMM_TM, GEMM_NST_DEEP>, hipFuncAttributeMaxDynamicSharedMemorySize, (int)GEMM_LDS_DEEP)); \
    HIVE_CHECK_HIP(ctx, hipFuncSetAttribute((const void *)gemm256p_kernel<T, EPI_>, hipFuncAttributeMaxDynamicSharedMemorySize, GEMM256_LDS))
    HIVE_GEMM_ATTR(EPI_BIAS);
    HIVE_GEMM_ATTR(EPI_BIAS_GELU);
    HIVE_GEMM_ATTR(EPI_BIAS_RESIDUAL);
    HIVE_GEMM_ATTR(EPI_QKV);
#undef HIVE_GEMM_ATTR
    HIVE_CHECK_HIP(ctx, hipFuncSetAttribute((const void *)gemm_kernel<T, EPI_QKV_ALL, GEMM_TM, GEMM_NST_DEEP>, hipFuncAttributeMaxDynamicSharedMemorySize, (int)GEMM_LDS_DEEP));
    HIVE_CHECK_HIP(ctx, hipFuncSetAttribute((const void *)gemm_kernel<T, EPI_QKV_ALL, GEMM_TM, GEMM_NST>, hipFuncAttributeMaxDynamicSharedMemorySize, (int)GEMM_LDS));
    HIVE_CHECK_HIP(ctx, hipFuncSetAttribute((const void *)gemm256_kernel<T, EPI_BIAS>, hipFuncAttributeMaxDynamicSharedMemorySize, GEMM256_LDS));
    HIVE_CHECK_HIP(ctx, hipFuncSetAttribute((const void *)gemm256_kernel<T, EPI_BIAS_GELU>, hipFuncAttributeMaxDynamicSharedMemorySize, GEMM256_LDS));
    HIVE_CHECK_HIP(ctx, hipFuncSetAttribute((const void *)gemm256_kernel<T, EPI_BIAS_RESIDUAL>, hipFuncAttributeMaxDynamicSharedMemorySize, GEMM256_LDS));
    if (ctx->device < 64) set[ctx->device] = true;
    return HIVE_OK;
}

static inline int pad64(int n) { return (n + 63) / 64 * 64; }

struct LnFold {
    const float *stats = nullptr, *c1 = nullptr;
    float *partial = nullptr;
};

template <typename T>
static int linear_t(hive_ctx *ctx, const void *A, const void *W, const float *bias, const void *residual, void *C, int M, int N, int K, int epilogue,
                    const LnFold &ln = LnFold()) {
    int rc = ensure_gemm_attrs<T>(ctx);
    if (rc) return rc;
    GemmParams<T> p{};
    p.A = (const T *)A;
    p.W = (const T *)W;
    p.bias = bias;
    p.residual = (const T *)residual;
    p.C = (T *)C;
    p.M = M;
    p.N = N;
    p.K = K;
    p.ldc = N;
    p.ln_stats = ln.stats;
    p.ln_c1 = ln.c1;
    p.ln_partial = ln.partial;
    return launch_gemm<T>(ctx, epilogue, p);
}

template <typename T>
static int qkv_t(hive_ctx *ctx, const void *x, const void *W, const float *bias, void *qk, void *vT, int B, int Np, int D, int H, const LnFold &ln = LnFold()) {
    int rc = ensure_gemm_attrs<T>(ctx);
    if (rc) return rc;
    GemmParams<T> p{};
    p.A = (const T *)x;
    p.W = (const T *)W;
    p.bias = bias;
    p.C = (T *)qk;
    p.M = B * Np;
    p.N = 2 * D;
    p.K = D;
    p.ldc = 2 * D;
    p.q_cols = D;
    p.q_scale = 0.125f * 1.44269504088896340736f;
    p.ln_stats = ln.stats;
    p.ln_c1 = ln.c1;
    {
        const long long tiles_all = (long long)((p.M + GEMM_TM - 1) / GEMM_TM) * (3 * D / BN);
        const char *merge_env = getenv("HIVE_QKV_MERGE");
        const long long merge_max = merge_env && merge_env[0] == '2' ? (long long)(2 * ctx->num_cus) / 8 * 8 : ctx->num_cus;
        if (!(merge_env && merge_env[0] == '0') && tiles_all <= merge_max && !getenv("HIVE_GEMM_TILE") && !getenv("HIVE_GEMM_RING")) {
            GemmParams<T> q = p;
            q.N = 3 * D;
            q.n_split = 2 * D;
            q.vT = (T *)vT;
            q.Np = Np;
            q.H = H;
            const bool deep = tiles_all <= ctx->num_cus;
            if (deep) ++ctx->n_deep_ring_launches;
            const dim3 grid((unsigned)((tiles_all + 7) / 8 * 8)), block(GEMM_TM * 2);
            if (deep)
                hipLaunchKernelGGL((gemm_kernel<T, EPI_QKV_ALL, GEMM_TM, GEMM_NST_DEEP>), grid, block, GEMM_LDS_DEEP, ctx->stream, q);
            else
                hipLaunchKernelGGL((gemm_kernel<T, EPI_QKV_ALL, GEMM_TM, GEMM_NST>), grid, block, GEMM_LDS, ctx->stream, q);
            HIVE_CHECK_HIP(ctx, hipGetLastError());
            return HIVE_OK;
        }
    }
    if ((rc = launch_gemm<T>(ctx, EPI_BIAS, p))) return rc;
    GemmParams<T> pv{};
    pv.A = (const T *)x;
    pv.W = (const T *)W + (size_t)2 * D * D;
    pv.bias = bias + 2 * D;
    pv.vT = (T *)vT;
    pv.M = B * Np;
    pv.N = D;
    pv.K = D;
    pv.ldc = D;
    pv.Np = Np;
    pv.H = H;
    pv.ln_stats = ln.stats;
    pv.ln_c1 = ln.c1 ? ln.c1 + 2 * D : nullptr;
    return launch_gemm<T>(ctx, EPI_QKV, pv);
}

template <typename T>
static int attention_t(hive_ctx *ctx, const void *qk, const void *vT, void *out, int B, int N, int Np, int D, int H) {
    AttnParams<T> p{};
    p.qk = (const T *)qk;
    p.vT = (const T *)vT;
    p.out = (T *)out;
    p.B = B;
    p.H = H;
    p.N = N;
    p.Np = Np;
    p.D = D;
    const int q_blocks = (p.Np + 127) / 128;
    const long long grid = (long long)p.B * p.H * q_blocks;
    const char *ks_env = getenv("HIVE_ATT_KSPLIT");
    const bool split = p.Np / ATT_KV >= 4 && (ks_env ? ks_env[0] == '1' : (grid <= ctx->num_cus && !ctx->deterministic));
    if (split)
        hipLaunchKernelGGL((attention_kernel<T, 2>), dim3((unsigned)grid), dim3(512), 0, ctx->stream, p);
    else
        hipLaunchKernelGGL((attention_kernel<T, 1>), dim3((unsigned)grid), dim3(256), 0, ctx->stream, p);
    HIVE_CHECK_HIP(ctx, hipGetLastError());
    return HIVE_OK;
}

#define HIVE_REQUIRE_16BIT(ctx, dtype, what) HIVE_REQUIRE(ctx, (dtype) == HIVE_BF16 || (dtype) == HIVE_F16, what ": dtype must be HIVE_F16 or HIVE_BF16, got %d", (int)(dtype))

static void fold_layernorm_weights(hive_vit *v) {
    hive_ctx *ctx = v->ctx;
    const int dim = v->dim, mlp_dim = v->mlp, depth = v->depth;
    const size_t esz = sizeof(half_bits), rows = (size_t)3 * dim + mlp_dim;
    const size_t w_bytes = (rows * dim * esz + 255) & ~(size_t)255, c_bytes = (2 * rows * sizeof(float) + 255) & ~(size_t)255;
    for (int i = 0; i < depth; ++i) {
        char *base = (char *)v->fold_mem + (size_t)i * (w_bytes + c_bytes);
        float *c = (float *)(base + w_bytes);
        hive_vit::Folded &f = v->folded[i];
        f.qkv_w = base;
        f.fc1_w = base + (size_t)3 * dim * dim * esz;
        f.qkv_c1 = c, f.qkv_c2 = c + 3 * dim, f.fc1_c1 = c + 6 * dim, f.fc1_c2 = c + 6 * dim + mlp_dim;
        const hive_vit_block_weights &b = v->blocks[i];
#define HIVE_FOLD(T_)                                                                                                                                   \
    hipLaunchKernelGGL(ln_fold_weights_kernel<T_>, dim3(3 * dim), dim3(256), 0, ctx->stream, (const T_ *)b.qkv_w, (const float *)b.qkv_b, (const float *)b.ln1_g, \
                       (const float *)b.ln1_b, dim, (T_ *)f.qkv_w, (float *)f.qkv_c1, (float *)f.qkv_c2);                                                \
    hipLaunchKernelGGL(ln_fold_weights_kernel<T_>, dim3(mlp_dim), dim3(256), 0, ctx->stream, (const T_ *)b.fc1_w, (const float *)b.fc1_b, (const float *)b.ln2_g, \
                       (const float *)b.ln2_b, dim, (T_ *)f.fc1_w, (float *)f.fc1_c1, (float *)f.fc1_c2)
        if (v->dtype == HIVE_BF16) {
            HIVE_FOLD(__bf16);
        } else {
            HIVE_FOLD(_Float16);
        }
#undef HIVE_FOLD
    }
}

extern "C" {

int hive_vit_layernorm(hive_ctx *ctx, const void *x, int dtype, const float *gamma, const float *beta, void *out, int M, int D, float eps) {
    HIVE_ENTER(ctx);
    if (!ctx) return hive_fail(nullptr, HIVE_ERR_INVALID, "ctx is NULL");
    HIVE_REQUIRE(ctx, x && gamma && beta && out, "layernorm: NULL argument");
    HIVE_REQUIRE_16BIT(ctx, dtype, "layernorm");
    HIVE_REQUIRE(ctx, M > 0 && D > 0 && D % 256 == 0 && D <= 1024, "layernorm: D must be a multiple of 256 and <= 1024, got %d", D);
    return dtype == HIVE_BF16 ? launch_layernorm<__bf16>(ctx, x, gamma, beta, out, M, D, eps) : launch_layernorm<_Float16>(ctx, x, gamma, beta, out, M, D, eps);
}

int hive_vit_linear(hive_ctx *ctx, const void *A, int dtype, const void *W, const float *bias, const void *residual, void *C, int M, int N,
                    int K, int epilogue) {
    HIVE_ENTER(ctx);
    if (!ctx) return hive_fail(nullptr, HIVE_ERR_INVALID, "ctx is NULL");
    HIVE_REQUIRE(ctx, A && W && bias && C, "linear: NULL argument");
    HIVE_REQUIRE_16BIT(ctx, dtype, "linear");
    HIVE_REQUIRE(ctx, M > 0 && N > 0 && K > 0 && N % BN == 0 && K % BK == 0, "linear: need N %% 128 == 0 and K %% 64 == 0 (M=%d N=%d K=%d)", M, N, K);
    HIVE_REQUIRE(ctx, epilogue == EPI_BIAS || epilogue == EPI_BIAS_GELU || (epilogue == EPI_BIAS_RESIDUAL && residual),
                 "linear: bad epilogue %d", epilogue);
    return dtype == HIVE_BF16 ? linear_t<__bf16>(ctx, A, W, bias, residual, C, M, N, K, epilogue) : linear_t<_Float16>(ctx, A, W, bias, residual, C, M, N, K, epilogue);
}

int hive_vit_qkv(hive_ctx *ctx, const void *x, int dtype, const void *W, const float *bias, void *qk, void *vT, int B, int Np, int D, int H) {
    HIVE_ENTER(ctx);
    if (!ctx) return hive_fail(nullptr, HIVE_ERR_INVALID, "ctx is NULL");
    HIVE_REQUIRE(ctx, x && W && bias && qk && vT, "qkv: NULL argument");
    HIVE_REQUIRE_16BIT(ctx, dtype, "qkv");
    HIVE_REQUIRE(ctx, B > 0 && Np > 0 && Np % 64 == 0 && D == H * 64 && D % 128 == 0, "qkv: need Np %% 64 == 0, D == 64 H, D %% 128 == 0");
    return dtype == HIVE_BF16 ? qkv_t<__bf16>(ctx, x, W, bias, qk, vT, B, Np, D, H) : qkv_t<_Float16>(ctx, x, W, bias, qk, vT, B, Np, D, H);
}

int hive_vit_attention(hive_ctx *ctx, const void *qk, int dtype, const void *vT, void *out, int B, int N, int Np, int D, int H) {
    HIVE_ENTER(ctx);
    if (!ctx) return hive_fail(nullptr, HIVE_ERR_INVALID, "ctx is NULL");
    HIVE_REQUIRE(ctx, qk && vT && out, "attention: NULL argument");
    HIVE_REQUIRE_16BIT(ctx, dtype, "attention");
    HIVE_REQUIRE(ctx, B > 0 && N > 0 && N <= Np && Np % 64 == 0 && Np - N < 64 && D == H * 64, "attention: need Np - 64 < N <= Np, Np %% 64 == 0, head dim 64");
    HIVE_REQUIRE(ctx, Np - N < 64, "attention: Np (%d) must be N (%d) rounded up to a multiple of 64", Np, N);
    return dtype == HIVE_BF16 ? attention_t<__bf16>(ctx, qk, vT, out, B, N, Np, D, H) : attention_t<_Float16>(ctx, qk, vT, out, B, N, Np, D, H);
}

int hive_dpt_preprocess(hive_ctx *ctx, const uint8_t *d_rgb, int64_t n_values, float mean, float std, int dtype, void *d_out) {
    HIVE_ENTER(ctx);
    if (!ctx) return hive_fail(nullptr, HIVE_ERR_INVALID, "ctx is NULL");
    HIVE_REQUIRE(ctx, d_rgb && d_out && n_values > 0 && std != 0.f, "dpt_preprocess: bad arguments");
    HIVE_REQUIRE(ctx, ((uintptr_t)d_rgb % 4 == 0) && ((uintptr_t)d_out % 8 == 0), "dpt_preprocess: unaligned buffers");
    const dim3 grid((unsigned)((n_values / 4 + 256) / 256));
    PreprocessLut lut;
    for (int i = 0; i < 256; ++i) lut.v[i] = (float)(((double)i / 255.0 - (double)mean) / (double)std);
    if (dtype == HIVE_BF16)
        hipLaunchKernelGGL(preprocess_kernel<__bf16>, grid, dim3(256), 0, ctx->stream, d_rgb, (long long)n_values, lut, (__bf16 *)d_out);
    else if (dtype == HIVE_F16)
        hipLaunchKernelGGL(preprocess_kernel<_Float16>, grid, dim3(256), 0, ctx->stream, d_rgb, (long long)n_values, lut, (_Float16 *)d_out);
    else
        return hive_fail(ctx, HIVE_ERR_INVALID, "dpt_preprocess: dtype must be HIVE_F16 or HIVE_BF16");
    HIVE_CHECK_HIP(ctx, hipGetLastError());
    return HIVE_OK;
}

int hive_dpt_head_tail(hive_ctx *ctx, const void *d_feat, int dtype, int64_t n_px, int C, const float *h_pre_bias, int pre_relu,
                       const float *h_weight, float bias, int non_negative, int invert, float scale, float shift, float *d_depth,
                       float depth_scale, float max_depth, uint16_t *d_out_mm, float *d_out_m) {
    HIVE_ENTER(ctx);
    if (!ctx) return hive_fail(nullptr, HIVE_ERR_INVALID, "ctx is NULL");
    HIVE_REQUIRE(ctx, d_feat && h_weight && n_px > 0, "dpt_head_tail: bad arguments");
    HIVE_REQUIRE(ctx, C > 0 && C <= 64 && C % 8 == 0, "dpt_head_tail: C must be a multiple of 8 and <= 64, got %d", C);
    HIVE_REQUIRE(ctx, d_depth || d_out_mm || d_out_m, "dpt_head_tail: no output requested");
    HeadTailParams p{};
    memcpy(p.w, h_weight, sizeof(float) * C);
    if (h_pre_bias) memcpy(p.pre_bias, h_pre_bias, sizeof(float) * C);
    p.pre_relu = pre_relu;
    p.bias = bias;
    p.scale = scale;
    p.shift = shift;
    p.C = C;
    p.non_negative = non_negative;
    p.invert = invert;
    p.n_px = n_px;
    p.depth_scale = depth_scale;
    p.max_depth = max_depth;
    const dim3 grid((unsigned)((n_px + 255) / 256));
    if (dtype == HIVE_BF16)
        hipLaunchKernelGGL(head_tail_kernel<__bf16>, grid, dim3(256), 0, ctx->stream, (const __bf16 *)d_feat, p, d_depth, d_out_mm, d_out_m);
    else if (dtype == HIVE_F16)
        hipLaunchKernelGGL(head_tail_kernel<_Float16>, grid, dim3(256), 0, ctx->stream, (const _Float16 *)d_feat, p, d_depth, d_out_mm, d_out_m);
    else
        return hive_fail(ctx, HIVE_ERR_INVALID, "dpt_head_tail: dtype must be HIVE_F16 or HIVE_BF16");
    HIVE_CHECK_HIP(ctx, hipGetLastError());
    return HIVE_OK;
}

int hive_vit_create(hive_ctx *ctx, int dtype, int depth, int dim, int heads, int mlp_dim, float ln_eps, const hive_vit_block_weights *blocks,
                    hive_vit **out) {
    HIVE_ENTER(ctx);
    if (!ctx) return hive_fail(nullptr, HIVE_ERR_INVALID, "ctx is NULL");
    HIVE_REQUIRE(ctx, out && blocks && depth > 0, "vit_create: NULL argument");
    HIVE_REQUIRE_16BIT(ctx, dtype, "vit_create");
    HIVE_REQUIRE(ctx, dim == heads * 64 && dim % 256 == 0 && dim <= 1024 && mlp_dim % 128 == 0,
                 "vit_create: need head dim 64, dim %% 256 == 0, dim <= 1024, mlp %% 128 == 0 (dim=%d heads=%d mlp=%d)", dim, heads, mlp_dim);
    for (int i = 0; i < depth; ++i) {
        const hive_vit_block_weights &b = blocks[i];
        HIVE_REQUIRE(ctx, b.ln1_g && b.ln1_b && b.qkv_w && b.qkv_b && b.proj_w && b.proj_b && b.ln2_g && b.ln2_b && b.fc1_w && b.fc1_b &&
                              b.fc2_w && b.fc2_b, "vit_create: block %d has a NULL weight pointer", i);
    }
    hive_vit *v = new hive_vit();
    v->ctx = ctx;
    v->dtype = dtype;
    v->depth = depth;
    v->dim = dim;
    v->heads = heads;
    v->mlp = mlp_dim;
    v->eps = ln_eps;
    v->blocks.assign(blocks, blocks + depth);
    {
        const size_t esz = sizeof(half_bits), rows = (size_t)3 * dim + mlp_dim;
        const size_t w_bytes = (rows * dim * esz + 255) & ~(size_t)255, c_bytes = (2 * rows * sizeof(float) + 255) & ~(size_t)255;
        hipError_t e = hipMalloc(&v->fold_mem, (size_t)depth * (w_bytes + c_bytes));
        if (e != hipSuccess) {
            int rc = hive_fail(ctx, HIVE_ERR_NOMEM, "vit_create: allocating the folded LayerNorm weights failed: %s", hipGetErrorString(e));
            delete v;
            return rc;
        }
        v->folded.resize(depth);
        fold_layernorm_weights(v);
        e = hipGetLastError();
        if (e == hipSuccess) e = hipStreamSynchronize(ctx->stream);
        if (e != hipSuccess) {
            int rc = hive_fail(ctx, HIVE_ERR_DEVICE, "vit_create: folding the LayerNorm weights failed: %s", hipGetErrorString(e));
            (void)hipFree(v->fold_mem);
            delete v;
            return rc;
        }
    }
    *out = v;
    return HIVE_OK;
}

int hive_vit_weights_modified(hive_vit *v) {
    HIVE_ENTER(v ? v->ctx : nullptr);
    if (!v) return hive_fail(nullptr, HIVE_ERR_INVALID, "vit is NULL");
    fold_layernorm_weights(v);
    HIVE_CHECK_HIP(v->ctx, hipGetLastError());
    return HIVE_OK;
}

int hive_vit_destroy(hive_vit *v) {
    HIVE_ENTER(v ? v->ctx : nullptr);
    if (!v) return HIVE_OK;
    (void)hipStreamSynchronize(v->ctx->stream);
    if (v->ws) (void)hipFree(v->ws);
    if (v->fold_mem) (void)hipFree(v->fold_mem);
    delete v;
    return HIVE_OK;
}

int hive_vit_forward(hive_vit *v, const void *x, int B, int N, const int *tap_blocks, int n_taps, void *const *tap_out) {
    HIVE_ENTER(v ? v->ctx : nullptr);
    if (!v) return hive_fail(nullptr, HIVE_ERR_INVALID, "vit is NULL");
    hive_ctx *ctx = v->ctx;
    HIVE_REQUIRE(ctx, x && B > 0 && N > 0, "vit_forward: bad arguments");
    HIVE_REQUIRE(ctx, n_taps >= 0 && (n_taps == 0 || (tap_blocks && tap_out)), "vit_forward: bad taps");
    int rc;
    const int D = v->dim, H = v->heads, Np = pad64(N), M = B * Np, dt = v->dtype;
    const size_t tok = (size_t)M * D * sizeof(half_bits);
    const char *fold_env = getenv("HIVE_LN_FOLD");
    const bool fold = !(fold_env && fold_env[0] == '0');
    const int groups = D / 64;
    const size_t part_bytes = ((size_t)M * groups * 2 * sizeof(float) + 255) & ~(size_t)255, stat_bytes = ((size_t)M * 2 * sizeof(float) + 255) & ~(size_t)255;
    const size_t off_x = 0, off_ln = off_x + tok, off_qk = off_ln + tok, off_vt = off_qk + 2 * tok, off_attn = off_vt + tok,
                 off_hid = off_attn + tok, off_part = off_hid + (size_t)M * v->mlp * sizeof(half_bits), off_stat = off_part + part_bytes,
                 total = off_stat + stat_bytes;
    if ((rc = hive_reserve_device(ctx, &v->ws, &v->ws_bytes, total))) return rc;
    char *ws = (char *)v->ws;
    half_bits *xs = (half_bits *)(ws + off_x), *ln = (half_bits *)(ws + off_ln), *qk = (half_bits *)(ws + off_qk), *vt = (half_bits *)(ws + off_vt),
              *attn = (half_bits *)(ws + off_attn), *hid = (half_bits *)(ws + off_hid);
    float *part = (float *)(ws + off_part), *stats = (float *)(ws + off_stat);
    const int cp_blocks = std::min<int>((int)(((size_t)M * D / 8 + 255) / 256), ctx->num_cus * 8);
    hipLaunchKernelGGL(pad_tokens_kernel, dim3(cp_blocks), dim3(256), 0, ctx->stream, (const half_bits *)x, xs, B, N, Np, D, 1);
    HIVE_CHECK_HIP(ctx, hipGetLastError());
    auto finalize = [&]() -> int {
        hipLaunchKernelGGL(ln_finalize_kernel, dim3((unsigned)((M + 15) / 16)), dim3(256), 0, ctx->stream, (const float *)part, M, groups, v->eps, stats);
        HIVE_CHECK_HIP(ctx, hipGetLastError());
        return HIVE_OK;
    };
    auto linear = [&](const void *A, const void *W, const float *bias, const void *residual, void *C, int Mm, int Nn, int Kk, int epi, const LnFold &lf) {
        return dt == HIVE_BF16 ? linear_t<__bf16>(ctx, A, W, bias, residual, C, Mm, Nn, Kk, epi, lf) : linear_t<_Float16>(ctx, A, W, bias, residual, C, Mm, Nn, Kk, epi, lf);
    };
    for (int i = 0; i < v->depth; ++i) {
        const hive_vit_block_weights &w = v->blocks[i];
        if (!fold) {
            if ((rc = hive_vit_layernorm(ctx, xs, dt, (const float *)w.ln1_g, (const float *)w.ln1_b, ln, M, D, v->eps))) return rc;
            if ((rc = hive_vit_qkv(ctx, ln, dt, w.qkv_w, (const float *)w.qkv_b, qk, vt, B, Np, D, H))) return rc;
            if ((rc = hive_vit_attention(ctx, qk, dt, vt, attn, B, N, Np, D, H))) return rc;
            if ((rc = hive_vit_linear(ctx, attn, dt, w.proj_w, (const float *)w.proj_b, xs, xs, M, D, D, EPI_BIAS_RESIDUAL))) return rc;
            if ((rc = hive_vit_layernorm(ctx, xs, dt, (const float *)w.ln2_g, (const float *)w.ln2_b, ln, M, D, v->eps))) return rc;
            if ((rc = hive_vit_linear(ctx, ln, dt, w.fc1_w, (const float *)w.fc1_b, nullptr, hid, M, v->mlp, D, EPI_BIAS_GELU))) return rc;
            if ((rc = hive_vit_linear(ctx, hid, dt, w.fc2_w, (const float *)w.fc2_b, xs, xs, M, D, v->mlp, EPI_BIAS_RESIDUAL))) return rc;
        } else {
            const hive_vit::Folded &f = v->folded[i];
            if (i == 0) {
                const dim3 grid((M + 3) / 4), block(256);
#define HIVE_STATS(T_, CH_) hipLaunchKernelGGL((ln_row_stats_kernel<T_, CH_>), grid, block, 0, ctx->stream, (const T_ *)xs, stats, M, v->eps)
                if (dt == HIVE_BF16) {
                    switch (D / 256) { case 1: HIVE_STATS(__bf16, 1); break; case 2: HIVE_STATS(__bf16, 2); break; case 3: HIVE_STATS(__bf16, 3); break; default: HIVE_STATS(__bf16, 4); }
                } else {
                    switch (D / 256) { case 1: HIVE_STATS(_Float16, 1); break; case 2: HIVE_STATS(_Float16, 2); break; case 3: HIVE_STATS(_Float16, 3); break; default: HIVE_STATS(_Float16, 4); }
                }
#undef HIVE_STATS
                HIVE_CHECK_HIP(ctx, hipGetLastError());
            } else if ((rc = finalize())) {
                return rc;
            }
            LnFold in1, in2, out;
            in1.stats = stats, in1.c1 = f.qkv_c1;
            in2.stats = stats, in2.c1 = f.fc1_c1;
            out.partial = part;
            rc = dt == HIVE_BF16 ? qkv_t<__bf16>(ctx, xs, f.qkv_w, f.qkv_c2, qk, vt, B, Np, D, H, in1) : qkv_t<_Float16>(ctx, xs, f.qkv_w, f.qkv_c2, qk, vt, B, Np, D, H, in1);
            if (rc) return rc;
            if ((rc = hive_vit_attention(ctx, qk, dt, vt, attn, B, N, Np, D, H))) return rc;
            if ((rc = linear(attn, w.proj_w, (const float *)w.proj_b, xs, xs, M, D, D, EPI_BIAS_RESIDUAL, out))) return rc;
            if ((rc = finalize())) return rc;
            if ((rc = linear(xs, f.fc1_w, f.fc1_c2, nullptr, hid, M, v->mlp, D, EPI_BIAS_GELU, in2))) return rc;
            if ((rc = linear(hid, w.fc2_w, (const float *)w.fc2_b, xs, xs, M, D, v->mlp, EPI_BIAS_RESIDUAL, i + 1 < v->depth ? out : LnFold()))) return rc;
        }
        for (int t = 0; t < n_taps; ++t)
            if (tap_blocks[t] == i) {
                hipLaunchKernelGGL(pad_tokens_kernel, dim3(cp_blocks), dim3(256), 0, ctx->stream, (const half_bits *)xs, (half_bits *)tap_out[t], B,
                                   N, Np, D, 0);
                HIVE_CHECK_HIP(ctx, hipGetLastError());
            }
    }
    return HIVE_OK;
}

}
```

Before: 1388 frames/s.

## Write patch-embed conv straight into padded ViT tokens and fuse readout gathers

Adds a token-path mode, on by default. The patch-embedding conv epilogue adds the positional embedding and writes directly into the padded ViT token workspace, and a small kernel fills the cls token and padding rows. The ViT forward then runs the readout projection inside the tap loop, using a gathering GEMM that reads the padded tokens directly when the shape allows. This removes the separate patch-embed output, token assembly, pad copy, tap copies and readout concat passes, cutting memory traffic and kernel launches. In exchange it adds a new conv epilogue variant and kernel instantiations, plus more coupling between the DPT and ViT workspaces.

```diff
diff --git a/hive_amd/csrc/conv.hip b/hive_amd/csrc/conv.hip
--- a/hive_amd/csrc/conv.hip
+++ b/hive_amd/csrc/conv.hip
@@ -41,6 +41,8 @@
     int split_k;
     hive_mfma::f32x4 *sk_ws;
     unsigned *sk_count;
+    const T *tok_pos;
+    int tok_np;
 };
 
 __device__ __forceinline__ float gn_affine_exact(float x, float rstd, float gamma, float beta, float mean) {
@@ -77,7 +79,7 @@
     auto pre = [&](int mt, int j) {
         const int m = min(m_base + mt * 16 + 8 * j + row_in_frag, p.M - 1);
         const size_t off = (size_t)m * p.Cout + n;
-        if (GN != 1 && p.res1) rs1[mt % (AHEAD + 1)][j] = *reinterpret_cast<const vec<T, 8> *>(p.res1 + off);
+        if (GN != 1 && GN != 3 && p.res1) rs1[mt % (AHEAD + 1)][j] = *reinterpret_cast<const vec<T, 8> *>(p.res1 + off);
         if (GN == 0 && NRES == 2) rs2[mt % (AHEAD + 1)][j] = *reinterpret_cast<const vec<T, 8> *>(p.res2 + off);
     };
     hive_mfma::staged_rows<MT, AHEAD>(stage, acc, lane, pre, [&](int r, int, const f32x4 &lo, const f32x4 &hi, int mt, int jrow) {
@@ -104,6 +106,14 @@
         vec<T, 8> ov;
 #pragma unroll
         for (int j = 0; j < 8; ++j) ov[j] = (T)o[j];
+        if (GN == 3) {
+            const int hw = p.Ho * p.Wo, img = m / hw, tokn = 1 + (m - img * hw);
+            const vec<T, 8> pv = *reinterpret_cast<const vec<T, 8> *>(p.tok_pos + (size_t)tokn * p.Cout + n);
+#pragma unroll
+            for (int j = 0; j < 8; ++j) ov[j] = (T)((float)ov[j] + (float)pv[j]);
+            *reinterpret_cast<vec<T, 8> *>(p.out + ((size_t)img * p.tok_np + tokn) * p.Cout + n) = ov;
+            return;
+        }
         if (GN == 2) {
             const bool second = m >= boundary;
             const float mean = second ? gmean[1] : gmean[0], rstd = second ? grstd[1] : grstd[0];
@@ -518,7 +528,10 @@
     HIVE_CONV_ATTR(128, 128, 1);
     HIVE_CONV_ATTR(256, 256, 2);
     HIVE_CONV_ATTR(128, 256, 2);
+    HIVE_CONV_ATTR(256, 256, 3);
+    HIVE_CONV_ATTR(128, 256, 3);
 #undef HIVE_CONV_ATTR
+    HIVE_CHECK_HIP(ctx, hipFuncSetAttribute((const void *)conv_deep_kernel<T, 128, 3, CONV_DEEP_NST>, hipFuncAttributeMaxDynamicSharedMemorySize, conv_lds(128, 128, CONV_DEEP_NST)));
     HIVE_CHECK_HIP(ctx, hipFuncSetAttribute((const void *)conv_deep_kernel<T, 128, 0, CONV_DEEP_NST>, hipFuncAttributeMaxDynamicSharedMemorySize, conv_lds(128, 128, CONV_DEEP_NST)));
     HIVE_CHECK_HIP(ctx, hipFuncSetAttribute((const void *)conv_deep_kernel<T, 128, 1, CONV_DEEP_NST>, hipFuncAttributeMaxDynamicSharedMemorySize, conv_lds(128, 128, CONV_DEEP_NST)));
     if (ctx->device < 64) set[ctx->device] = true;
@@ -530,6 +543,8 @@
     const float *gn_stats = nullptr;
     const void *gn_gamma = nullptr, *gn_beta = nullptr;
     int gn_G = 0, gn_cpg = 0;
+    const void *tok_pos = nullptr;
+    int tok_np = 0;
 };
 
 template <typename T>
@@ -584,6 +599,8 @@
         p.gn_beta = (const T *)gn_mode->gn_beta;
         p.gn_G = gn_mode->gn_G;
         p.gn_cpg = gn_mode->gn_cpg;
+        p.tok_pos = (const T *)gn_mode->tok_pos;
+        p.tok_np = gn_mode->tok_np;
     }
     if (d_gn_partial && gn_tile_rows && (long long)Ho * Wo >= tm && !relu && !d_residual && !d_residual2 && !d_out_relu) {
         HIVE_REQUIRE(ctx, (long long)((p.M + tm - 1) / tm) * 4 * C_out <= gn_partial_floats, "%s: gn_partial holds %lld floats, %lld needed", what,
@@ -620,6 +637,8 @@
             const dim3 dgrid((unsigned)std::min<long long>((items + 7) / 8 * 8, (long long)ctx->num_cus / 8 * 8));
             if (stats)
                 hipLaunchKernelGGL((conv_deep_kernel<T, 128, 1, CONV_DEEP_NST>), dgrid, dim3(512), (size_t)conv_lds(128, 128, CONV_DEEP_NST), ctx->stream, p);
+            else if (p.tok_pos)
+                hipLaunchKernelGGL((conv_deep_kernel<T, 128, 3, CONV_DEEP_NST>), dgrid, dim3(512), (size_t)conv_lds(128, 128, CONV_DEEP_NST), ctx->stream, p);
             else
                 hipLaunchKernelGGL((conv_deep_kernel<T, 128, 0, CONV_DEEP_NST>), dgrid, dim3(512), (size_t)conv_lds(128, 128, CONV_DEEP_NST), ctx->stream, p);
             HIVE_CHECK_HIP(ctx, hipGetLastError());
@@ -641,6 +660,11 @@
             hipLaunchKernelGGL((conv_kernel<T, 256, 256, 2>), grid, dim3(512), lds, ctx->stream, p);
         else
             hipLaunchKernelGGL((conv_kernel<T, 128, 256, 2>), grid, dim3(512), lds, ctx->stream, p);
+    } else if (p.tok_pos) {
+        if (tm == 256)
+            hipLaunchKernelGGL((conv_kernel<T, 256, 256, 3>), grid, dim3(512), lds, ctx->stream, p);
+        else
+            hipLaunchKernelGGL((conv_kernel<T, 128, 256, 3>), grid, dim3(512), lds, ctx->stream, p);
     } else if (tm == 256 && tn == 256)
         HIVE_CONV_LAUNCH(256, 256);
     else if (tm == 256 && tn == 128)
@@ -757,6 +781,20 @@
     return HIVE_OK;
 }
 
+extern "C" int hive_nhwc_conv_tokens(hive_ctx *ctx, const void *d_x, int dtype, int N, int H, int W, int C_in, int C_out, const void *d_w, const void *d_bias,
+                                     const void *d_pos, int Np, void *d_tokens) {
+    HIVE_ENTER(ctx);
+    if (!ctx) return hive_fail(nullptr, HIVE_ERR_INVALID, "ctx is NULL");
+    HIVE_REQUIRE(ctx, d_pos && d_tokens && d_tokens != d_x, "nhwc_conv_tokens: NULL argument");
+    HIVE_REQUIRE(ctx, C_out % 256 == 0 && H > 0 && W > 0 && (long long)H * W + 1 <= Np, "nhwc_conv_tokens: need C_out %% 256 == 0 and H W + 1 <= Np (C_out=%d, %d x %d, Np=%d)", C_out,
+                 H, W, Np);
+    GnMode mode;
+    mode.tok_pos = d_pos;
+    mode.tok_np = Np;
+    return launch_conv(ctx, "nhwc_conv_tokens", d_x, dtype, N, H, W, C_in, C_out, 1, 1, 0, 0, H, W, d_w, d_bias, 0, nullptr, nullptr, d_tokens, nullptr, nullptr, 0, nullptr,
+                       &mode);
+}
+
 extern "C" int hive_nhwc_conv(hive_ctx *ctx, const void *d_x, int dtype, int N, int H, int W, int C_in, int C_out, int kernel, int stride, int pad_top,
                               int pad_left, int H_out, int W_out, const void *d_w, const void *d_bias, int relu, const void *d_residual,
                               const void *d_residual2, void *d_out, void *d_out_relu) {
diff --git a/hive_amd/csrc/dpt_net.hip b/hive_amd/csrc/dpt_net.hip
--- a/hive_amd/csrc/dpt_net.hip
+++ b/hive_amd/csrc/dpt_net.hip
@@ -40,6 +40,29 @@
     }
 }
 
+template <typename T>
+__global__ __launch_bounds__(256) void token_frame_kernel(const T *__restrict__ cls, const T *__restrict__ pos, T *__restrict__ xs, int B, int N, int Np, int D) {
+    const int dv = D / 8, rows = 1 + Np - N;
+    const long long total = (long long)B * rows * dv;
+    for (long long i = (long long)blockIdx.x * 256 + threadIdx.x; i < total; i += (long long)gridDim.x * 256) {
+        const int c = (int)(i % dv) * 8;
+        const long long rb = i / dv;
+        const int r = (int)(rb % rows), b = (int)(rb / rows);
+        T o[8];
+        if (r == 0) {
+            const uint4 ra = *reinterpret_cast<const uint4 *>(cls + c), rp = *reinterpret_cast<const uint4 *>(pos + c);
+            const T *a = reinterpret_cast<const T *>(&ra), *p = reinterpret_cast<const T *>(&rp);
+#pragma unroll
+            for (int j = 0; j < 8; ++j) o[j] = (T)((float)a[j] + (float)p[j]);
+        } else {
+#pragma unroll
+            for (int j = 0; j < 8; ++j) o[j] = (T)0.0f;
+        }
+        const int row = r == 0 ? 0 : N + r - 1;
+        *reinterpret_cast<uint4 *>(xs + ((size_t)b * Np + row) * D + c) = *reinterpret_cast<const uint4 *>(o);
+    }
+}
+
 void launch_assemble_tokens(hive_ctx *ctx, int dtype, int blocks, const void *patch, const void *cls, const void *pos, void *tokens, int B, int n_patch, int D) {
     if (dtype == HIVE_BF16)
         hipLaunchKernelGGL(assemble_tokens_kernel<__bf16>, dim3(blocks), dim3(256), 0, ctx->stream, (const __bf16 *)patch, (const __bf16 *)cls, (const __bf16 *)pos,
@@ -135,7 +158,7 @@
         if (_rc) return _rc;       \
     } while (0)
 
-int run_forward(hive_dpt *d, bool dry, const uint8_t *d_rgb, int B, int FH, int FW, int H, int W, const void *d_pos, float *d_depth, float max_depth,
+int run_forward(hive_dpt *d, bool dry, bool token_path, const uint8_t *d_rgb, int B, int FH, int FW, int H, int W, const void *d_pos, float *d_depth, float max_depth,
                 uint16_t *d_mm, float *d_m) {
     hive_ctx *ctx = d->ctx;
     const bool resized = FH != H || FW != W;
@@ -300,6 +323,42 @@
         layer_2 = hook[1];
 
         const int gh = feat.H, gw = feat.W, n_patch = gh * gw, N = n_patch + 1, D = 768;
+        if (token_path) {
+            half_t *cat = hive_vit_readout_gathers(ctx, B, N, D) ? nullptr : d->alloc((size_t)B * n_patch * 2 * D);
+            Map map3{d->alloc((size_t)B * n_patch * D), gh, gw, D}, map4{d->alloc((size_t)B * n_patch * D), gh, gw, D};
+            if (!dry) {
+                const void *pw, *pb, *cls;
+                DPT_TRY(need("pretrained.model.patch_embed.proj.weight", &pw));
+                DPT_TRY(need("pretrained.model.patch_embed.proj.bias", &pb));
+                DPT_TRY(need("pretrained.model.cls_token", &cls));
+                void *xs = nullptr;
+                DPT_TRY(hive_vit_tokens(d->vit, B, N, &xs));
+                DPT_TRY(hive_dpt_patch_tokens(ctx, feat.p, dt, B, gh, gw, feat.C, D, pw, pb, cls, d_pos, xs));
+                const int taps[2] = {8, 11};
+                hive_vit_tap ro[2];
+                Map *maps[2] = {&map3, &map4};
+                for (int r = 0; r < 2; ++r) {
+                    const std::string pre = std::string("pretrained.act_postprocess") + (r == 0 ? "3" : "4") + ".0.project.0.";
+                    const void *rb;
+                    DPT_TRY(need(pre + "weight", &ro[r].w));
+                    DPT_TRY(need(pre + "bias", &rb));
+                    ro[r].bias = (const float *)rb;
+                    ro[r].out = maps[r]->p;
+                    ro[r].cat = cat;
+                }
+                DPT_TRY(hive_vit_forward_readout(d->vit, nullptr, B, N, taps, 2, ro));
+            }
+            drop(feat);
+            d->release(cat);
+            Map t4;
+            DPT_TRY(conv(map3, "pretrained.act_postprocess3.3.weight", "pretrained.act_postprocess3.3.bias", D, 1, 1, false, 0, nullptr, nullptr, false, &layer_3, nullptr));
+            drop(map3);
+            DPT_TRY(conv(map4, "pretrained.act_postprocess4.3.weight", "pretrained.act_postprocess4.3.bias", D, 1, 1, false, 0, nullptr, nullptr, false, &t4, nullptr));
+            drop(map4);
+            DPT_TRY(conv(t4, "pretrained.act_postprocess4.4.weight", "pretrained.act_postprocess4.4.bias", D, 3, 2, false, 0, nullptr, nullptr, false, &layer_4, nullptr));
+            drop(t4);
+            return HIVE_OK;
+        }
         Map pe;
         DPT_TRY(conv(feat, "pretrained.model.patch_embed.proj.weight", "pretrained.model.patch_embed.proj.bias", D, 1, 1, false, 0, nullptr, nullptr, false, &pe,
                      nullptr));
@@ -345,11 +404,12 @@
     auto large_backbone = [&]() -> int {
         const int D = 1024, gh = H / 16, gw = W / 16, n_patch = gh * gw, N = n_patch + 1;
         half_t *xin = d->alloc((size_t)B * H * W * 3), *cols = d->alloc((size_t)B * n_patch * 768), *pe = d->alloc((size_t)B * n_patch * D);
-        half_t *tokens = d->alloc((size_t)B * N * D), *cat = d->alloc((size_t)B * n_patch * 2 * D);
+        const bool need_cat = !token_path || !hive_vit_readout_gathers(ctx, B, N, D);
+        half_t *tokens = d->alloc((size_t)B * N * D), *cat = need_cat ? d->alloc((size_t)B * n_patch * 2 * D) : nullptr;
         half_t *tapb[4];
         Map maps[4];
         for (int r = 0; r < 4; ++r) {
-            tapb[r] = d->alloc((size_t)B * N * D);
+            tapb[r] = token_path ? nullptr : d->alloc((size_t)B * N * D);
             maps[r] = Map{d->alloc((size_t)B * n_patch * D), gh, gw, D};
         }
         if (!dry) {
@@ -364,9 +424,22 @@
             launch_assemble_tokens(ctx, dt, blocks, pe, cls, d_pos, tokens, B, n_patch, D);
             HIVE_CHECK_HIP(ctx, hipGetLastError());
             const int taps[4] = {5, 11, 17, 23};
+            if (token_path) {
+                hive_vit_tap ro[4];
+                for (int r = 0; r < 4; ++r) {
+                    const std::string pre = "pretrained.act_postprocess" + std::to_string(r + 1) + ".0.project.0.";
+                    const void *rb;
+                    DPT_TRY(need(pre + "weight", &ro[r].w));
+                    DPT_TRY(need(pre + "bias", &rb));
+                    ro[r].bias = (const float *)rb;
+                    ro[r].out = maps[r].p;
+                    ro[r].cat = cat;
+                }
+                DPT_TRY(hive_vit_forward_readout(d->vit, tokens, B, N, taps, 4, ro));
+            }
             void *tap_out[4] = {tapb[0], tapb[1], tapb[2], tapb[3]};
-            DPT_TRY(hive_vit_forward(d->vit, tokens, B, N, taps, 4, tap_out));
-            for (int r = 0; r < 4; ++r) {
+            if (!token_path) DPT_TRY(hive_vit_forward(d->vit, tokens, B, N, taps, 4, tap_out));
+            for (int r = 0; r < 4 && !token_path; ++r) {
                 hipLaunchKernelGGL(readout_concat_kernel, dim3(blocks), dim3(256), 0, ctx->stream, (const half_t *)tapb[r], cat, B, n_patch, D);
                 HIVE_CHECK_HIP(ctx, hipGetLastError());
                 const std::string pre = "pretrained.act_postprocess" + std::to_string(r + 1) + ".0.project.0.";
@@ -525,16 +598,36 @@
     HIVE_REQUIRE(ctx, d_rgb && d_pos_embed && (d_depth || d_out_mm || d_out_m), "hive_dpt_forward: NULL argument");
     HIVE_REQUIRE(ctx, B > 0 && frame_h > 0 && frame_w > 0, "hive_dpt_forward: bad frame batch %d x %d x %d", B, frame_h, frame_w);
     HIVE_REQUIRE(ctx, H >= 32 && W >= 32 && H % 32 == 0 && W % 32 == 0, "hive_dpt_forward: the network's input size must be a multiple of 32 (%d x %d)", H, W);
+    const char *tp_env = getenv("HIVE_TOKEN_PATH");
+    const bool token_path = !(tp_env && tp_env[0] == '0');
     void *arena = d->arena;
     d->arena = nullptr;
     d->reset_arena();
-    int rc = run_forward(d, true, d_rgb, B, frame_h, frame_w, H, W, d_pos_embed, d_depth, max_depth, d_out_mm, d_out_m);
+    int rc = run_forward(d, true, token_path, d_rgb, B, frame_h, frame_w, H, W, d_pos_embed, d_depth, max_depth, d_out_mm, d_out_m);
     d->arena = arena;
     if (rc) return rc;
     const size_t need = d->arena_used;
     if ((rc = hive_reserve_device(ctx, &d->arena, &d->arena_bytes, need))) return rc;
     d->reset_arena();
-    return run_forward(d, false, d_rgb, B, frame_h, frame_w, H, W, d_pos_embed, d_depth, max_depth, d_out_mm, d_out_m);
+    return run_forward(d, false, token_path, d_rgb, B, frame_h, frame_w, H, W, d_pos_embed, d_depth, max_depth, d_out_mm, d_out_m);
+}
+
+int hive_dpt_patch_tokens(hive_ctx *ctx, const void *d_x, int dtype, int N, int H, int W, int C_in, int D, const void *d_w, const void *d_bias, const void *d_cls,
+                          const void *d_pos, void *d_tokens) {
+    HIVE_ENTER(ctx);
+    if (!ctx) return hive_fail(nullptr, HIVE_ERR_INVALID, "ctx is NULL");
+    HIVE_REQUIRE(ctx, d_x && d_w && d_bias && d_cls && d_pos && d_tokens, "dpt_patch_tokens: NULL argument");
+    HIVE_REQUIRE(ctx, dtype == HIVE_BF16 || dtype == HIVE_F16, "dpt_patch_tokens: dtype must be HIVE_F16 or HIVE_BF16, got %d", dtype);
+    HIVE_REQUIRE(ctx, N > 0 && H > 0 && W > 0 && D > 0 && D % 256 == 0, "dpt_patch_tokens: bad sizes %d x %d x %d, D = %d", N, H, W, D);
+    const int n_tok = H * W + 1, Np = (n_tok + 63) / 64 * 64;
+    const int blocks = (int)std::min<long long>(((long long)N * (1 + Np - n_tok) * D / 8 + 255) / 256, (long long)ctx->num_cus * 16);
+    if (dtype == HIVE_BF16)
+        hipLaunchKernelGGL(token_frame_kernel<__bf16>, dim3(blocks), dim3(256), 0, ctx->stream, (const __bf16 *)d_cls, (const __bf16 *)d_pos, (__bf16 *)d_tokens, N, n_tok, Np, D);
+    else
+        hipLaunchKernelGGL(token_frame_kernel<_Float16>, dim3(blocks), dim3(256), 0, ctx->stream, (const _Float16 *)d_cls, (const _Float16 *)d_pos, (_Float16 *)d_tokens, N, n_tok,
+                           Np, D);
+    HIVE_CHECK_HIP(ctx, hipGetLastError());
+    return hive_nhwc_conv_tokens(ctx, d_x, dtype, N, H, W, C_in, D, d_w, d_bias, d_pos, Np, d_tokens);
 }
 
 int hive_dpt_forward(hive_dpt *d, const uint8_t *d_rgb, int B, int H, int W, const void *d_pos_embed, float *d_depth, float max_depth,
diff --git a/hive_amd/csrc/hive_internal.hpp b/hive_amd/csrc/hive_internal.hpp
--- a/hive_amd/csrc/hive_internal.hpp
+++ b/hive_amd/csrc/hive_internal.hpp
@@ -97,6 +97,22 @@
 int hive_splitk_workspace(hive_ctx *ctx, size_t bytes, void **ws, unsigned **count);
 int hive_gram_gn_stats(hive_ctx *ctx, const void *d_x, int dtype, int N, int H, int W, int C_in, int C_out, int stride, int Ho, int Wo, int G, const float *d_tables,
                        float eps, float *d_stats, float *d_S_out, float *d_s_out);
+extern "C" {
+typedef struct hive_vit_tap {
+    const void *w;
+    const float *bias;
+    void *out;
+    void *cat;
+} hive_vit_tap;
+int hive_vit_tokens(hive_vit *vit, int B, int N, void **xs);
+int hive_vit_forward_readout(hive_vit *vit, const void *x, int B, int N, const int *tap_blocks, int n_taps, const hive_vit_tap *readouts);
+int hive_vit_readout(hive_ctx *ctx, const void *xs, int dtype, int B, int N, int D, const void *W, const float *bias, void *cat, void *out);
+int hive_vit_readout_gathers(hive_ctx *ctx, int B, int N, int D);
+int hive_nhwc_conv_tokens(hive_ctx *ctx, const void *d_x, int dtype, int N, int H, int W, int C_in, int C_out, const void *d_w, const void *d_bias,
+                          const void *d_pos, int Np, void *d_tokens);
+int hive_dpt_patch_tokens(hive_ctx *ctx, const void *d_x, int dtype, int N, int H, int W, int C_in, int D, const void *d_w, const void *d_bias, const void *d_cls,
+                          const void *d_pos, void *d_tokens);
+}
 __device__ __forceinline__ unsigned block_exclusive(unsigned c, unsigned *lds) {
     const int lane = threadIdx.x & 63, wave = threadIdx.x >> 6;
     unsigned inc = c;
diff --git a/hive_amd/csrc/vit.hip b/hive_amd/csrc/vit.hip
--- a/hive_amd/csrc/vit.hip
+++ b/hive_amd/csrc/vit.hip
@@ -81,6 +81,7 @@
     int split_k = 1;
     hive_mfma::f32x4 *sk_ws = nullptr;
     unsigned *sk_count = nullptr;
+    int g_np = 0, g_n = 0;
 };
 
 constexpr int BN = 128, BK = 64;
@@ -553,11 +554,12 @@
 #endif
 }
 
-template <typename T, int EPI>
+template <typename T, int EPI, bool GATHER = false>
 __global__ __launch_bounds__(512, 1) void gemm256p_kernel(GemmParams<T> p) {
     extern __shared__ __attribute__((aligned(16))) unsigned char lds[];
     constexpr int A_GROUPS = T256 / 8, GROUPS = 2 * A_GROUPS, PER_WAVE = GROUPS / 8;
     constexpr bool VT = (EPI == EPI_QKV);
+    static_assert(!GATHER || !VT, "the gathered A is the readout's: row-major output");
     const int tid = threadIdx.x, lane = tid & 63;
     const int wave = __builtin_amdgcn_readfirstlane(tid >> 6);
     const int wr = wave >> 2, wc = wave & 3;
@@ -568,7 +570,9 @@
     if (tl >= run_n) return;
     int m0, n0;
     unsigned piece_off[PER_WAVE];
+    unsigned cls_off[PER_WAVE / 2];
     const char *a_panel, *w_panel;
+    const int KT = p.K / BK, KH = KT >> 1;
     auto setup = [&](int tile) {
         m0 = (tile / tiles_n) * T256;
         n0 = (tile % tiles_n) * T256;
@@ -576,16 +580,30 @@
         for (int j = 0; j < PER_WAVE; ++j) {
             const int g = wave + j * 8, row = (g & (A_GROUPS - 1)) * 8 + (lane >> 3), chunk = (lane & 7) ^ ((row >> 1) & 7);
             const int rel = j < PER_WAVE / 2 ? min(row, p.M - 1 - m0) : min(row, p.N - 1 - n0);
+            if constexpr (GATHER) {
+                if (j < PER_WAVE / 2) {
+                    const int m = m0 + rel, img = m / p.g_n;
+                    const unsigned cls_row = (unsigned)img * (unsigned)p.g_np;
+                    piece_off[j] = (cls_row + 1u + (unsigned)(m - img * p.g_n)) * (unsigned)p.K + (unsigned)chunk * 16u;
+                    cls_off[j] = cls_row * (unsigned)p.K + (unsigned)chunk * 16u;
+                    continue;
+                }
+            }
             piece_off[j] = (unsigned)rel * (unsigned)p.K * 2u + (unsigned)chunk * 16u;
         }
-        a_panel = reinterpret_cast<const char *>(p.A + (size_t)m0 * p.K);
+        a_panel = reinterpret_cast<const char *>(GATHER ? p.A : p.A + (size_t)m0 * p.K);
         w_panel = reinterpret_cast<const char *>(p.W + (size_t)n0 * p.K);
     };
     auto issue_piece = [&](int kt, int stage, int j) {
-        const char *g = (j < PER_WAVE / 2 ? a_panel : w_panel) + (size_t)kt * (BK * 2) + piece_off[j];
+        const char *g;
+        if (GATHER && j < PER_WAVE / 2) {
+            const bool cls = kt >= KH;
+            g = a_panel + (size_t)(cls ? kt - KH : kt) * (BK * 2) + (cls ? cls_off[j] : piece_off[j]);
+        } else {
+            g = (j < PER_WAVE / 2 ? a_panel : w_panel) + (size_t)kt * (BK * 2) + piece_off[j];
+        }
         __builtin_amdgcn_global_load_lds((const void *)g, (__attribute__((address_space(3))) void *)(lds + stage * T256_STAGE + (wave + j * 8) * 1024), 16, 0, 0);
     };
-    const int KT = p.K / BK;
     setup(run0 + tl);
 #pragma unroll
     for (int j = 0; j < PER_WAVE; ++j) issue_piece(0, 0, j);
@@ -1010,15 +1028,19 @@
     return HIVE_OK;
 }
 
+static bool gemm_takes_256(hive_ctx *ctx, int M, int N) {
+    const char *force = getenv("HIVE_GEMM_TILE");
+    const long long tiles256 = (long long)((M + T256 - 1) / T256) * (N / T256);
+    const long long rounds = (tiles256 + ctx->num_cus - 1) / ctx->num_cus;
+    const bool fills = tiles256 * 5 >= rounds * ctx->num_cus * 3;
+    return N % T256 == 0 && ((force && force[0] == '2') || (!force && fills));
+}
+
 template <typename T>
 static int launch_gemm(hive_ctx *ctx, int epi, const GemmParams<T> &p) {
-    const char *force = getenv("HIVE_GEMM_TILE");
-    const long long tiles256 = (long long)((p.M + T256 - 1) / T256) * (p.N / T256);
-    const long long rounds = (tiles256 + ctx->num_cus - 1) / ctx->num_cus;
-    const bool fills = tiles256 * 5 >= rounds * ctx->num_cus * 3;
     static const char *persist_env = getenv("HIVE_GEMM_PERSIST");
     const bool one_tile_kernel = persist_env && persist_env[0] == '0';
-    if ((epi != EPI_QKV || !one_tile_kernel) && p.N % T256 == 0 && ((force && force[0] == '2') || (!force && fills))) return launch_gemm256<T>(ctx, epi, p);
+    if ((epi != EPI_QKV || !one_tile_kernel) && gemm_takes_256(ctx, p.M, p.N)) return launch_gemm256<T>(ctx, epi, p);
     const long long tiles = (long long)((p.M + GEMM_TM - 1) / GEMM_TM) * (p.N / BN);
     GemmParams<T> q = p;
     const long long slots = (long long)(2 * ctx->num_cus) / 8 * 8;
@@ -1074,6 +1096,7 @@
     HIVE_CHECK_HIP(ctx, hipFuncSetAttribute((const void *)gemm256_kernel<T, EPI_BIAS>, hipFuncAttributeMaxDynamicSharedMemorySize, GEMM256_LDS));
     HIVE_CHECK_HIP(ctx, hipFuncSetAttribute((const void *)gemm256_kernel<T, EPI_BIAS_GELU>, hipFuncAttributeMaxDynamicSharedMemorySize, GEMM256_LDS));
     HIVE_CHECK_HIP(ctx, hipFuncSetAttribute((const void *)gemm256_kernel<T, EPI_BIAS_RESIDUAL>, hipFuncAttributeMaxDynamicSharedMemorySize, GEMM256_LDS));
+    HIVE_CHECK_HIP(ctx, hipFuncSetAttribute((const void *)gemm256p_kernel<T, EPI_BIAS_GELU, true>, hipFuncAttributeMaxDynamicSharedMemorySize, GEMM256_LDS));
     if (ctx->device < 64) set[ctx->device] = true;
     return HIVE_OK;
 }
@@ -1104,6 +1127,55 @@
     p.ln_c1 = ln.c1;
     p.ln_partial = ln.partial;
     return launch_gemm<T>(ctx, epilogue, p);
+}
+
+static bool readout_gathers(hive_ctx *ctx, int B, int N, int D) {
+    static const char *persist_env = getenv("HIVE_GEMM_PERSIST");
+    if (persist_env && persist_env[0] == '0') return false;
+    if ((unsigned long long)B * (unsigned long long)pad64(N) * D * sizeof(half_bits) > 0xFFFFFFFFull) return false;
+    return gemm_takes_256(ctx, B * (N - 1), D);
+}
+
+__global__ __launch_bounds__(256) void readout_concat_padded_kernel(const half_bits *__restrict__ xs, half_bits *__restrict__ cat, int B, int n_patch, int Np, int D) {
+    const int dv = D / 8;
+    const long long total = (long long)B * n_patch * 2 * dv;
+    for (long long i = (long long)blockIdx.x * 256 + threadIdx.x; i < total; i += (long long)gridDim.x * 256) {
+        const int c = (int)(i % (2 * dv));
+        const long long row = i / (2 * dv);
+        const int b = (int)(row / n_patch), t = (int)(row % n_patch);
+        const half_bits *src = c < dv ? xs + ((size_t)b * Np + 1 + t) * D + c * 8 : xs + (size_t)b * Np * D + (c - dv) * 8;
+        *reinterpret_cast<uint4 *>(cat + (size_t)row * 2 * D + c * 8) = *reinterpret_cast<const uint4 *>(src);
+    }
+}
+
+template <typename T>
+static int readout_t(hive_ctx *ctx, const void *xs, int B, int N, int D, const void *W, const float *bias, void *cat, void *out) {
+    const int n_patch = N - 1, Np = pad64(N), M = B * n_patch;
+    if (!readout_gathers(ctx, B, N, D)) {
+        HIVE_REQUIRE(ctx, cat, "readout: this shape (B=%d N=%d D=%d) takes the concatenated matrix: cat is NULL", B, N, D);
+        const int blocks = (int)std::min<long long>(((long long)M * 2 * D / 8 + 255) / 256, (long long)ctx->num_cus * 16);
+        hipLaunchKernelGGL(readout_concat_padded_kernel, dim3(blocks), dim3(256), 0, ctx->stream, (const half_bits *)xs, (half_bits *)cat, B, n_patch, Np, D);
+        HIVE_CHECK_HIP(ctx, hipGetLastError());
+        return linear_t<T>(ctx, cat, W, bias, nullptr, out, M, D, 2 * D, EPI_BIAS_GELU);
+    }
+    int rc = ensure_gemm_attrs<T>(ctx);
+    if (rc) return rc;
+    GemmParams<T> p{};
+    p.A = (const T *)xs;
+    p.W = (const T *)W;
+    p.bias = bias;
+    p.C = (T *)out;
+    p.M = M;
+    p.N = D;
+    p.K = 2 * D;
+    p.ldc = D;
+    p.g_np = Np;
+    p.g_n = n_patch;
+    const long long tiles = (long long)((M + T256 - 1) / T256) * (D / T256);
+    const dim3 pgrid((unsigned)std::min<long long>((tiles + 7) / 8 * 8, (long long)ctx->num_cus / 8 * 8));
+    hipLaunchKernelGGL((gemm256p_kernel<T, EPI_BIAS_GELU, true>), pgrid, dim3(512), (size_t)GEMM256_LDS, ctx->stream, p);
+    HIVE_CHECK_HIP(ctx, hipGetLastError());
+    return HIVE_OK;
 }
 
 template <typename T>
@@ -1370,12 +1442,16 @@
     return HIVE_OK;
 }
 
-int hive_vit_forward(hive_vit *v, const void *x, int B, int N, const int *tap_blocks, int n_taps, void *const *tap_out) {
-    HIVE_ENTER(v ? v->ctx : nullptr);
-    if (!v) return hive_fail(nullptr, HIVE_ERR_INVALID, "vit is NULL");
+}
+
+static size_t vit_workspace_bytes(const hive_vit *v, int B, int N) {
+    const size_t M = (size_t)B * pad64(N), tok = M * v->dim * sizeof(half_bits);
+    const size_t part_bytes = (M * (v->dim / 64) * 2 * sizeof(float) + 255) & ~(size_t)255, stat_bytes = (M * 2 * sizeof(float) + 255) & ~(size_t)255;
+    return 6 * tok + M * v->mlp * sizeof(half_bits) + part_bytes + stat_bytes;
+}
+
+static int vit_forward_impl(hive_vit *v, const void *x, int B, int N, const int *tap_blocks, int n_taps, void *const *tap_out, const hive_vit_tap *readouts) {
     hive_ctx *ctx = v->ctx;
-    HIVE_REQUIRE(ctx, x && B > 0 && N > 0, "vit_forward: bad arguments");
-    HIVE_REQUIRE(ctx, n_taps >= 0 && (n_taps == 0 || (tap_blocks && tap_out)), "vit_forward: bad taps");
     int rc;
     const int D = v->dim, H = v->heads, Np = pad64(N), M = B * Np, dt = v->dtype;
     const size_t tok = (size_t)M * D * sizeof(half_bits);
@@ -1386,14 +1462,18 @@
     const size_t off_x = 0, off_ln = off_x + tok, off_qk = off_ln + tok, off_vt = off_qk + 2 * tok, off_attn = off_vt + tok,
                  off_hid = off_attn + tok, off_part = off_hid + (size_t)M * v->mlp * sizeof(half_bits), off_stat = off_part + part_bytes,
                  total = off_stat + stat_bytes;
+    HIVE_REQUIRE(ctx, total == vit_workspace_bytes(v, B, N), "vit_forward: workspace layout and vit_workspace_bytes disagree");
+    HIVE_REQUIRE(ctx, x || (v->ws && v->ws_bytes >= total), "vit_forward: no tokens (call hive_vit_tokens for this batch first)");
     if ((rc = hive_reserve_device(ctx, &v->ws, &v->ws_bytes, total))) return rc;
     char *ws = (char *)v->ws;
     half_bits *xs = (half_bits *)(ws + off_x), *ln = (half_bits *)(ws + off_ln), *qk = (half_bits *)(ws + off_qk), *vt = (half_bits *)(ws + off_vt),
               *attn = (half_bits *)(ws + off_attn), *hid = (half_bits *)(ws + off_hid);
     float *part = (float *)(ws + off_part), *stats = (float *)(ws + off_stat);
     const int cp_blocks = std::min<int>((int)(((size_t)M * D / 8 + 255) / 256), ctx->num_cus * 8);
-    hipLaunchKernelGGL(pad_tokens_kernel, dim3(cp_blocks), dim3(256), 0, ctx->stream, (const half_bits *)x, xs, B, N, Np, D, 1);
-    HIVE_CHECK_HIP(ctx, hipGetLastError());
+    if (x) {
+        hipLaunchKernelGGL(pad_tokens_kernel, dim3(cp_blocks), dim3(256), 0, ctx->stream, (const half_bits *)x, xs, B, N, Np, D, 1);
+        HIVE_CHECK_HIP(ctx, hipGetLastError());
+    }
     auto finalize = [&]() -> int {
         hipLaunchKernelGGL(ln_finalize_kernel, dim3((unsigned)((M + 15) / 16)), dim3(256), 0, ctx->stream, (const float *)part, M, groups, v->eps, stats);
         HIVE_CHECK_HIP(ctx, hipGetLastError());
@@ -1441,6 +1521,12 @@
         }
         for (int t = 0; t < n_taps; ++t)
             if (tap_blocks[t] == i) {
+                if (readouts) {
+                    const hive_vit_tap &r = readouts[t];
+                    rc = dt == HIVE_BF16 ? readout_t<__bf16>(ctx, xs, B, N, D, r.w, r.bias, r.cat, r.out) : readout_t<_Float16>(ctx, xs, B, N, D, r.w, r.bias, r.cat, r.out);
+                    if (rc) return rc;
+                    continue;
+                }
                 hipLaunchKernelGGL(pad_tokens_kernel, dim3(cp_blocks), dim3(256), 0, ctx->stream, (const half_bits *)xs, (half_bits *)tap_out[t], B,
                                    N, Np, D, 0);
                 HIVE_CHECK_HIP(ctx, hipGetLastError());
@@ -1449,4 +1535,47 @@
     return HIVE_OK;
 }
 
-}
+extern "C" {
+
+int hive_vit_forward(hive_vit *v, const void *x, int B, int N, const int *tap_blocks, int n_taps, void *const *tap_out) {
+    HIVE_ENTER(v ? v->ctx : nullptr);
+    if (!v) return hive_fail(nullptr, HIVE_ERR_INVALID, "vit is NULL");
+    hive_ctx *ctx = v->ctx;
+    HIVE_REQUIRE(ctx, x && B > 0 && N > 0, "vit_forward: bad arguments");
+    HIVE_REQUIRE(ctx, n_taps >= 0 && (n_taps == 0 || (tap_blocks && tap_out)), "vit_forward: bad taps");
+    return vit_forward_impl(v, x, B, N, tap_blocks, n_taps, tap_out, nullptr);
+}
+
+int hive_vit_tokens(hive_vit *v, int B, int N, void **xs) {
+    HIVE_ENTER(v ? v->ctx : nullptr);
+    if (!v) return hive_fail(nullptr, HIVE_ERR_INVALID, "vit is NULL");
+    HIVE_REQUIRE(v->ctx, xs && B > 0 && N > 0, "vit_tokens: bad arguments");
+    int rc = hive_reserve_device(v->ctx, &v->ws, &v->ws_bytes, vit_workspace_bytes(v, B, N));
+    if (rc) return rc;
+    *xs = v->ws;
+    return HIVE_OK;
+}
+
+int hive_vit_forward_readout(hive_vit *v, const void *x, int B, int N, const int *tap_blocks, int n_taps, const hive_vit_tap *readouts) {
+    HIVE_ENTER(v ? v->ctx : nullptr);
+    if (!v) return hive_fail(nullptr, HIVE_ERR_INVALID, "vit is NULL");
+    hive_ctx *ctx = v->ctx;
+    HIVE_REQUIRE(ctx, B > 0 && N > 1 && n_taps > 0 && tap_blocks && readouts, "vit_forward_readout: bad arguments");
+    for (int t = 0; t < n_taps; ++t) HIVE_REQUIRE(ctx, readouts[t].w && readouts[t].bias && readouts[t].out, "vit_forward_readout: readout %d has a NULL pointer", t);
+    return vit_forward_impl(v, x, B, N, tap_blocks, n_taps, nullptr, readouts);
+}
+
+int hive_vit_readout_gathers(hive_ctx *ctx, int B, int N, int D) {
+    return ctx && B > 0 && N > 1 && D > 0 && D % BN == 0 && readout_gathers(ctx, B, N, D) ? 1 : 0;
+}
+
+int hive_vit_readout(hive_ctx *ctx, const void *xs, int dtype, int B, int N, int D, const void *W, const float *bias, void *cat, void *out) {
+    HIVE_ENTER(ctx);
+    if (!ctx) return hive_fail(nullptr, HIVE_ERR_INVALID, "ctx is NULL");
+    HIVE_REQUIRE(ctx, xs && W && bias && out, "readout: NULL argument");
+    HIVE_REQUIRE_16BIT(ctx, dtype, "readout");
+    HIVE_REQUIRE(ctx, B > 0 && N > 1 && D > 0 && D % BN == 0, "readout: need N > 1 and D %% 128 == 0 (B=%d N=%d D=%d)", B, N, D);
+    return dtype == HIVE_BF16 ? readout_t<__bf16>(ctx, xs, B, N, D, W, bias, cat, out) : readout_t<_Float16>(ctx, xs, B, N, D, W, bias, cat, out);
+}
+
+}
```

Result: no change. 1401 frames/s, median of 6 (+1.0%).
